# seanrjohnson/protein_gibbs_sampler

Measured on AMD Instinct MI355X. Metric: sampled positions/sec (whole node), ESM-1b L=256 B=256 Gibbs, higher is better.
Workload: dtype bf16; 1 GPU; ESM_sampler ESM-1b (33 layers, d=1280) Gibbs: 256 chains in total, 256 per GPU x L=256 (T=258), P=25 positions per chain per iteration, mask=True top_k=0 temperature=1.0 burnin=inf; bf16 MFMA operands, fp32 accumulate + fp32 residual stream; synthetic weights N(0,0.025), embeddings N(0,0.3), LayerNorm jitter 0.1 (logit std ~10); global_batch=256, seq_len=256, parallelism=chains sharded 1-way (contiguous blocks), 1 RCCL all-gather at the end, n_layers=33

## Files before the change

### include/pgibbs.h

```cpp
#ifndef PGIBBS_H
#define PGIBBS_H

#include <stdint.h>

#ifdef __cplusplus
extern "C" {
#endif

#ifndef PG_API
#if defined(__GNUC__) || defined(__clang__)
#define PG_API __attribute__((visibility("default")))
#else
#define PG_API
#endif
#endif

#define PG_OK 0
#define PG_ERR_INVALID 1
#define PG_ERR_HIP 2
#define PG_ERR_NO_DEVICE 3
#define PG_ERR_WEIGHTS 4
#define PG_ERR_UNSUPPORTED 5
#define PG_ERR_RANGE 6

PG_API const char* pg_version(void);
PG_API const char* pg_last_error(void);
PG_API int pg_device_count(void);

typedef struct pg_pyrandom pg_pyrandom;
PG_API pg_pyrandom* pg_pyrandom_create(void);
PG_API void pg_pyrandom_destroy(pg_pyrandom*);
PG_API int pg_pyrandom_seed(pg_pyrandom*, const uint32_t* key_words, int n_words);
PG_API int pg_pyrandom_setstate(pg_pyrandom*, const uint32_t* mt624, int index);
PG_API int pg_pyrandom_getstate(const pg_pyrandom*, uint32_t* mt624, int* index);
PG_API uint32_t pg_pyrandom_getrandbits32(pg_pyrandom*, int k );
PG_API double pg_pyrandom_random(pg_pyrandom*);
PG_API int pg_pyrandom_sample(pg_pyrandom*, const int32_t* population, int n, int k, int32_t* out);
PG_API int pg_pyrandom_sample_table(pg_pyrandom*, const int32_t* population, int n, int k, int64_t n_rows, int32_t* out);
PG_API int pg_pyrandom_shuffle(pg_pyrandom*, int32_t* x, int n);
PG_API int pg_pyrandom_choices(pg_pyrandom*, int n, int k, int32_t* out);

typedef struct pg_engine pg_engine;

#define PG_ARCH_ESM1B 1
#define PG_ARCH_MSA1B 2
#define PG_ARCH_ESM1 3
#define PG_ARCH_ESM2 4

#define PG_PREC_BF16 0
#define PG_PREC_F16 2
#define PG_PREC_FP32 1

typedef struct {
  int32_t arch;
  int32_t vocab;
  int32_t d_model;
  int32_t n_layers;
  int32_t n_heads;
  int32_t d_ffn;
  int32_t max_positions;
  int32_t pad_idx, mask_idx, cls_idx, eos_idx;
  int32_t token_dropout;
  int32_t max_msa_rows;
  float layer_norm_eps;
} pg_model_config;

typedef struct {
  const char* name;
  const float* data;
  int64_t numel;
} pg_tensor;

PG_API int pg_engine_create(const pg_model_config* cfg, const pg_tensor* tensors, int n_tensors, int device_ordinal,
                     int precision, pg_engine** out);
PG_API int pg_engine_create_embedded(const pg_model_config* cfg, int head_slot, const pg_tensor* tensors, int n_tensors, int device_ordinal,
                              int precision, pg_engine** out);
PG_API void pg_engine_destroy(pg_engine*);
PG_API int pg_engine_set_stream(pg_engine*, void* hip_stream);
PG_API int pg_engine_synchronize(pg_engine*);
PG_API int pg_engine_device(const pg_engine*);
PG_API int pg_engine_set_job_items(pg_engine*, int64_t job_items);
PG_API int pg_engine_get_stat(pg_engine*, const char* name, int64_t* value);

typedef struct {
  int32_t mask;
  int32_t mask_idx;
  int32_t top_k;
  int32_t burnin;
  float temperature;
  int32_t n_valid;
  int32_t valid_idx[32];
  uint64_t rng_seed;
  uint32_t rng_stream;
  uint32_t row_id_base;
  int32_t iter_base;
} pg_sample_params;


PG_API int pg_esm_forward_logits(pg_engine*, const int32_t* tokens, int B, int T, float* logits_out);
PG_API int pg_esm_gibbs_run(pg_engine*, int32_t* tokens_inout, int B, int T, const int32_t* target_idx, int n_iters, int P,
                     const pg_sample_params* params, float* sampled_logits, int32_t* sampled_tokens);
PG_API int pg_esm_gibbs_run_device(pg_engine*, int32_t* d_tokens_inout, int B, int T, const int32_t* d_target_idx,
                            int n_iters, int P, const pg_sample_params* params, float* d_sampled_logits,
                            int32_t* d_sampled_tokens);

PG_API int pg_esm_forward_representations(pg_engine*, const int32_t* tokens, int B, int T, const int32_t* layers, int n_req,
                                          const int32_t* pools, int n_pools, float* per_token_out, float* pooled_out);
PG_API int pg_repr_dbg_rows(int device, const float* x, int64_t M, int d, int d_live, const float* gamma, const float* beta, float eps,
                            const int32_t* tokens, int pad_idx, float* rows_out, int B, int T, const int32_t* pools, int n_pools,
                            float* pooled_out);

PG_API int pg_engine_set_contact_head(pg_engine*, const float* weight, int n_weights, float bias);
PG_API int pg_esm_forward_contacts(pg_engine*, const int32_t* tokens, int B, int T, float* contacts_out, float* logits_out,
                                   const int32_t* attn_layers, int n_attn, float* attn_out);
PG_API int pg_contact_dbg_probs(int device, int precision, const float* qkv, int n_seq, int T, int H, int head_dim, const int32_t* key_tok,
                                int pad_idx, float* probs_out, char* plan, int plan_bytes);
PG_API int pg_contact_dbg_accumulate(int device, const float* P, const int32_t* tokens, int eos_idx, int pad_idx, const float* w, float bias,
                                     int first, int last, float* logits_inout, float* contacts_out, int B, int T, int H);

PG_API int pg_msa_forward_logits(pg_engine*, const int32_t* tokens, int B, int R, int C, float* logits_out);
PG_API int pg_msa_gibbs_run(pg_engine*, int32_t* tokens_inout, int B, int R, int C, const int32_t* target_idx, int n_iters,
                     int P, const pg_sample_params* params, float* sampled_logits, int32_t* sampled_tokens);
PG_API int pg_msa_gibbs_run_device(pg_engine*, int32_t* d_tokens_inout, int B, int R, int C, const int32_t* d_target_idx,
                            int n_iters, int P, const pg_sample_params* params, float* d_sampled_logits,
                            int32_t* d_sampled_tokens);
PG_API int pg_msa_gibbs_single_run(pg_engine*, int32_t* tokens_inout, int R, int C, int mask_row, int target_row,
                            const int32_t* step_idx, const int32_t* step_sample_flag, int n_steps, int P_max,
                            const pg_sample_params* params, float* sampled_logits, int32_t* sampled_tokens);
PG_API int pg_msa_gibbs_single_batch_run(pg_engine*, int32_t* tokens_inout, int B, int R, int C, int mask_row, int target_row,
                                  const int32_t* step_idx, const int32_t* step_sample_flag, int n_steps, int P_max,
                                  const pg_sample_params* params, float* sampled_logits, int32_t* sampled_tokens);

PG_API int pg_esm_forward_logprobs(pg_engine*, const int32_t* tokens, int B, int T, const int32_t* row_of, const int32_t* idx,
                            const int32_t* targets, int n_sel, int P, float* out);
PG_API int pg_msa_forward_logprobs(pg_engine*, const int32_t* tokens, int B, int R, int C, const int32_t* row_of,
                            const int32_t* idx, const int32_t* targets, int n_sel, int P, float* out);
PG_API int pg_logprob_gather_device(void* stream, const float* d_logits, int64_t n_rows, int width, int V, const int32_t* d_idx,
                             const int32_t* d_row_map, const int32_t* d_targets, int64_t n_sel, int P, float* d_out);

#define PG_TABLE_NORM_VOCAB 0
#define PG_TABLE_NORM_COLUMNS 1
PG_API int pg_logprob_table_device(void* stream, const float* d_logits, int64_t n_rows, int width, int V, const int32_t* d_idx,
                            const int32_t* d_row_map, int64_t n_sel, int P, const int32_t* d_cols, int n_cols, int norm,
                            float* d_out , float* d_entropy );
PG_API int pg_esm_forward_logprob_table(pg_engine*, const int32_t* tokens, int B, int T, const int32_t* row_of, const int32_t* idx,
                                 int n_sel, int P, const int32_t* cols, int n_cols, int norm, float* out, float* entropy_or_null);
PG_API int pg_msa_forward_logprob_table(pg_engine*, const int32_t* tokens, int B, int R, int C, const int32_t* row_of,
                                 const int32_t* idx, int n_sel, int P, const int32_t* cols, int n_cols, int norm, float* out,
                                 float* entropy_or_null);

PG_API int pg_mask_scatter_device(void* stream, int32_t* d_tokens, int64_t n_rows, int width, const int32_t* d_idx,
                           const int32_t* d_row_map, int64_t n_sel, int P, int mask_idx);
PG_API int pg_sample_writeback_device(void* stream, int32_t* d_tokens, int64_t n_rows, int width, const float* d_logits,
                               int V, const int32_t* d_idx, const int32_t* d_row_map, int64_t n_sel, int P,
                               const pg_sample_params* params, int iteration, int32_t* d_sampled_tokens);

typedef struct {
  const float* bias;
  int64_t bias_rows;
  int width;
  int n_valid;
  const float* temperatures;
  int n_temperatures;
  float top_p;
} pg_draw_guide;
PG_API int pg_engine_set_draw_guide(pg_engine*, const pg_draw_guide* guide_or_null);
PG_API int pg_sample_writeback_guided_device(void* stream, int32_t* d_tokens, int64_t n_rows, int width, const float* d_logits, int V,
                                      const int32_t* d_idx, const int32_t* d_row_map, int64_t n_sel, int P,
                                      const pg_sample_params* params, int iteration, int32_t* d_sampled_tokens, const float* d_bias,
                                      int64_t bias_rows, const float* d_temperatures, int n_temperatures, float top_p);

#define PG_COMM_ID_BYTES 128
typedef struct pg_comm pg_comm;
PG_API int pg_comm_unique_id(void* id_out);
PG_API int pg_comm_create(int rank, int world, const void* unique_id, int device_ordinal, pg_comm** out);
PG_API void pg_comm_destroy(pg_comm*);
PG_API int pg_comm_rank(const pg_comm*);
PG_API int pg_comm_world(const pg_comm*);
PG_API int pg_gather_tokens(pg_comm*, void* hip_stream, const int32_t* d_local, int64_t rows, int width, const int64_t* counts,
                     int32_t* d_out);
typedef int (*pg_allgather_fn)(void* ctx, const void* send, void* recv, size_t n_int32);
PG_API int pg_dbg_gather_tokens_host(int rank, int world, const int32_t* local, int64_t rows, int width, const int64_t* counts,
                              int force_padded, pg_allgather_fn allgather, void* ctx, int32_t* out);
PG_API int pg_dbg_gather_plan(int rank, int world, int64_t rows, int width, const int64_t* counts, int force_padded, int64_t* out7,
                       int64_t* out_off_bytes);

PG_API int pg_prof_enable(pg_engine*, int on);
PG_API int pg_prof_reset(pg_engine*);
PG_API int pg_prof_get(pg_engine*, const char* kernel_class, double* total_ms, int64_t* launches);
PG_API int pg_prof_get_kernels(pg_engine*, const char* kernel_class, char* buf, int buf_bytes);

PG_API int pg_dbg_gemm(int device, int precision, const float* x, const float* w, const float* bias, float* out, int M, int N,
                int K, int epi);
PG_API int pg_dbg_gemm_v(int device, int precision, const float* x, const float* w, const float* bias, float* out, int M, int N, int K, int epi,
                  int variant, int have_ws, int m_live, char* plan, int plan_bytes);
PG_API int pg_dbg_gemm_ln(int device, int precision, const float* x, const float* x_pad, const float* gamma, const float* beta, float eps,
                   const float* w, const float* bias, float* out, int out_rows, int M, int N, int K, int gelu, int nb, char* plan,
                   int plan_bytes);
PG_API int pg_dbg_gemm_bench(int device, int M, int N, int K, int epi, int variant, int iters, double* avg_ms);
PG_API int pg_dbg_gemm_plan(int M, int N, int K, int epi, int variant, int have_ws, int m_live, int n_cu, char* buf, int buf_bytes);
PG_API int pg_dbg_attention_plan(int kind, int precision, int64_t n_seq_or_B, int T_or_C, int R, int H, int head_dim, int has_pad, int has_bias,
                          int row_step, int order_bh, int n_cu, char* buf, int buf_bytes);
PG_API int pg_dbg_qkv_attention_bench(int device, int B, int T, int H, int iters, double* ms, double* max_diff);
PG_API int pg_dbg_layernorm(int device, const float* x, const float* gamma, const float* beta, float* y, int M, int d,
                     float eps);
PG_API int pg_dbg_layernorm_operand(int device, int precision, const float* x, const float* gamma, const float* beta, float* y, int M,
                             int d, float eps);
PG_API int pg_dbg_attention(int device, int precision, const float* qkv, float* ctx, int B, int T, int H);
PG_API int pg_dbg_rope(int device, int precision, float* qkv_inout, int B, int T, int H);
PG_API int pg_dbg_attention_hd(int device, int precision, const float* qkv, float* ctx, int B, int T, int H, int head_dim,
                        const int32_t* key_tok, int pad_idx);
PG_API int pg_dbg_rope_hd(int device, int precision, float* qkv_inout, int B, int T, int H, int head_dim);
PG_API int pg_dbg_attention_kv(int device, int precision, const float* qkv, float* ctx, int B, int T, int H, int head_dim,
                        const int32_t* key_tok, int pad_idx, const float* bias_k, const float* bias_v, char* plan, int plan_bytes);

PG_API int pg_dbg_msa_attention(int device, int which, const float* qkv, float* ctx, int B, int R, int C, int H, float scale);
PG_API int pg_dbg_msa_attention_tok(int device, int which, const float* qkv, float* ctx, int B, int R, int C, int H, float scale,
                             const int32_t* tok, int pad_idx, char* plan, int plan_bytes);


PG_API int pg_dbg_embed(int device, int precision, const int32_t* tokens, int n_seq, int T, const float* embed, int V, int d, const float* pos,
                 int pos_rows, const float* msa_pos, int rows_per_msa, const float* gamma, const float* beta, const float* gamma2,
                 const float* beta2, int pad_idx, int mask_idx, int token_dropout, float eps, float embed_scale, float* x, uint16_t* h2);
PG_API int pg_dbg_layernorm_rows(int device, int precision, const float* x, const float* gamma, const float* beta, uint16_t* h_inout,
                          int64_t h_rows, int M, int d, float eps, int form, int colmajor_R, int colmajor_C, int* kernel);
PG_API int pg_dbg_gather_ln(int device, int precision, const float* x, int64_t x_rows, const int32_t* idx, const int32_t* row_map, int64_t n_map,
                     int P, int width, const float* gamma, const float* beta, uint16_t* h_inout, int64_t h_rows, int64_t n_sel, int d,
                     float eps, int split);
PG_API int pg_dbg_gather_rows(int device, const void* src, int64_t src_rows, void* dst_inout, int64_t dst_rows, const int32_t* idx, int n_iters,
                       int iter, const int32_t* row_map, int64_t n_map, int P, int width, int64_t n_sel, int row_bytes);
PG_API int pg_dbg_split_rows(int device, const float* x, uint16_t* h_inout, int64_t h_rows, int rows, int K, float scale, int form,
                      float* gelu_out);
PG_API int pg_dbg_lm_tail(int device, const float* g, const float* gamma, const float* beta, const float* embed, const float* out_bias,
                   float* logits, int64_t n, int d, int V, float eps, int* small_kernel);

PG_API int pg_dbg_sample(int device, int32_t* tokens_inout, int64_t n_rows, int width, const float* logits, int V, int compact, const int32_t* idx,
                  int n_tables, const int32_t* row_map, int64_t n_sel, int P, const pg_sample_params* params, int first_iter, int n_steps,
                  int device_iter, int mask_idx, int permit_out_of_range, int32_t* sampled_out, int32_t* masked_tokens_out,
                  unsigned* nonfinite_out);
PG_API int pg_guided_dbg_sample(int device, int32_t* tokens_inout, int64_t n_rows, int width, const float* logits, int V, int compact,
                         const int32_t* idx, int n_tables, const int32_t* row_map, int64_t n_sel, int P, const pg_sample_params* params,
                         int first_iter, int n_steps, int device_iter, int mask_idx, int permit_out_of_range, int32_t* sampled_out,
                         int32_t* masked_tokens_out, unsigned* nonfinite_out, const pg_draw_guide* guide);
PG_API int pg_guided_sizeof_draw_guide(void);

PG_API int pg_embedded_embed_rows(int device, int precision, const int32_t* tokens, int n_seq, int T, const float* embed, int V, int d,
                           const float* pos, int pos_rows, const float* msa_pos, int rows_per_msa, const float* gamma, const float* beta,
                           const float* gamma2, const float* beta2, int pad_idx, int mask_idx, int token_dropout, float eps, float embed_scale,
                           float* x, uint16_t* h2, int d_live);
PG_API int pg_embedded_layernorm_rows(int device, int precision, const float* x, const float* gamma, const float* beta, uint16_t* h_inout,
                               int64_t h_rows, int M, int d, float eps, int form, int colmajor_R, int colmajor_C, int* kernel, int d_live);
PG_API int pg_embedded_gather_ln(int device, int precision, const float* x, int64_t x_rows, const int32_t* idx, const int32_t* row_map, int64_t n_map,
                          int P, int width, const float* gamma, const float* beta, uint16_t* h_inout, int64_t h_rows, int64_t n_sel, int d,
                          float eps, int split, int d_live);
PG_API int pg_embedded_lm_tail(int device, const float* g, const float* gamma, const float* beta, const float* embed, const float* out_bias,
                        float* logits, int64_t n, int d, int V, float eps, int* small_kernel, int d_live);
PG_API int pg_embedded_image(const char* name, const float* src, int64_t numel, int n_heads, int head_width, int head_slot, int d_ffn, int vocab,
                      float* image, int64_t image_numel);
PG_API int pg_embedded_rope_table(int rows, int head_width, int head_slot, float* table);

#ifdef __cplusplus
}
#endif
#endif
```

### protein_gibbs_sampler_amd/_lib.py

```python
import ctypes
import math
import os
import sys
from ctypes import (POINTER, Structure, c_char_p, c_double, c_float, c_int, c_int32, c_int64, c_uint32, c_uint64,
                    c_void_p)

_HERE = os.path.dirname(os.path.abspath(__file__))
LIB_PATH = os.environ.get("PGIBBS_LIB_PATH") or os.path.join(_HERE, "lib", "libpgibbs.so")

PG_OK = 0
PG_ERR_INVALID, PG_ERR_HIP, PG_ERR_NO_DEVICE, PG_ERR_WEIGHTS, PG_ERR_UNSUPPORTED, PG_ERR_RANGE = 1, 2, 3, 4, 5, 6
PG_ARCH_ESM1B, PG_ARCH_MSA1B, PG_ARCH_ESM1, PG_ARCH_ESM2 = 1, 2, 3, 4
PG_COMM_ID_BYTES = 128
PG_PREC_BF16, PG_PREC_FP32, PG_PREC_F16 = 0, 1, 2
PG_TABLE_NORM_VOCAB, PG_TABLE_NORM_COLUMNS = 0, 1
TABLE_NORMS = {"vocab": PG_TABLE_NORM_VOCAB, "columns": PG_TABLE_NORM_COLUMNS}
INT32_MAX = 2**31 - 1


class PgError(RuntimeError):
    def __init__(self, code, msg):
        super().__init__("pgibbs error %d: %s" % (code, msg))
        self.code = code
        self.msg = msg


class ModelConfig(Structure):
    _fields_ = [("arch", c_int32), ("vocab", c_int32), ("d_model", c_int32), ("n_layers", c_int32), ("n_heads", c_int32),
                ("d_ffn", c_int32), ("max_positions", c_int32), ("pad_idx", c_int32), ("mask_idx", c_int32),
                ("cls_idx", c_int32), ("eos_idx", c_int32), ("token_dropout", c_int32), ("max_msa_rows", c_int32),
                ("layer_norm_eps", c_float)]


class Tensor(Structure):
    _fields_ = [("name", c_char_p), ("data", POINTER(c_float)), ("numel", c_int64)]


class SampleParams(Structure):
    _fields_ = [("mask", c_int32), ("mask_idx", c_int32), ("top_k", c_int32), ("burnin", c_int32),
                ("temperature", c_float), ("n_valid", c_int32), ("valid_idx", c_int32 * 32), ("rng_seed", c_uint64),
                ("rng_stream", c_uint32), ("row_id_base", c_uint32), ("iter_base", c_int32)]


class DrawGuideStruct(Structure):
    _fields_ = [("bias", POINTER(c_float)), ("bias_rows", c_int64), ("width", c_int), ("n_valid", c_int),
                ("temperatures", POINTER(c_float)), ("n_temperatures", c_int), ("top_p", c_float)]


class EngineHandle(c_void_p):

    @classmethod
    def from_param(cls, value):
        return c_void_p.from_param(value)


_lib = None

_P32 = POINTER(c_int32)
_PF = POINTER(c_float)
_PU32 = POINTER(c_uint32)
SIGNATURES = [
    ("pg_version", c_char_p, []),
    ("pg_last_error", c_char_p, []),
    ("pg_device_count", c_int, []),
    ("pg_pyrandom_create", c_void_p, []),
    ("pg_pyrandom_destroy", None, [c_void_p]),
    ("pg_pyrandom_seed", c_int, [c_void_p, _PU32, c_int]),
    ("pg_pyrandom_setstate", c_int, [c_void_p, _PU32, c_int]),
    ("pg_pyrandom_getstate", c_int, [c_void_p, _PU32, POINTER(c_int)]),
    ("pg_pyrandom_getrandbits32", c_uint32, [c_void_p, c_int]),
    ("pg_pyrandom_random", c_double, [c_void_p]),
    ("pg_pyrandom_sample", c_int, [c_void_p, _P32, c_int, c_int, _P32]),
    ("pg_pyrandom_sample_table", c_int, [c_void_p, _P32, c_int, c_int, c_int64, _P32]),
    ("pg_pyrandom_shuffle", c_int, [c_void_p, _P32, c_int]),
    ("pg_pyrandom_choices", c_int, [c_void_p, c_int, c_int, _P32]),
    ("pg_engine_create", c_int, [POINTER(ModelConfig), POINTER(Tensor), c_int, c_int, c_int, POINTER(c_void_p)]),
    ("pg_engine_create_embedded", c_int, [POINTER(ModelConfig), c_int, POINTER(Tensor), c_int, c_int, c_int, POINTER(c_void_p)]),
    ("pg_engine_destroy", None, [c_void_p]),
    ("pg_engine_set_stream", c_int, [c_void_p, c_void_p]),
    ("pg_engine_synchronize", c_int, [c_void_p]),
    ("pg_engine_device", c_int, [c_void_p]),
    ("pg_engine_set_job_items", c_int, [c_void_p, c_int64]),
    ("pg_engine_get_stat", c_int, [c_void_p, c_char_p, POINTER(c_int64)]),
    ("pg_esm_forward_logits", c_int, [c_void_p, c_void_p, c_int, c_int, c_void_p]),
    ("pg_esm_gibbs_run", c_int, [c_void_p, c_void_p, c_int, c_int, c_void_p, c_int, c_int, POINTER(SampleParams), c_void_p,
                                 c_void_p]),
    ("pg_esm_gibbs_run_device", c_int, [c_void_p, c_void_p, c_int, c_int, c_void_p, c_int, c_int, POINTER(SampleParams),
                                        c_void_p, c_void_p]),
    ("pg_msa_forward_logits", c_int, [c_void_p, c_void_p, c_int, c_int, c_int, c_void_p]),
    ("pg_msa_gibbs_run", c_int, [c_void_p, c_void_p, c_int, c_int, c_int, c_void_p, c_int, c_int, POINTER(SampleParams),
                                 c_void_p, c_void_p]),
    ("pg_msa_gibbs_run_device", c_int, [c_void_p, c_void_p, c_int, c_int, c_int, c_void_p, c_int, c_int, POINTER(SampleParams),
                                        c_void_p, c_void_p]),
    ("pg_msa_gibbs_single_run", c_int, [c_void_p, c_void_p, c_int, c_int, c_int, c_int, c_void_p, c_void_p, c_int, c_int,
                                        POINTER(SampleParams), c_void_p, c_void_p]),
    ("pg_msa_gibbs_single_batch_run", c_int, [c_void_p, c_void_p, c_int, c_int, c_int, c_int, c_int, c_void_p, c_void_p, c_int,
                                              c_int, POINTER(SampleParams), c_void_p, c_void_p]),
    ("pg_esm_forward_logprobs", c_int, [c_void_p, c_void_p, c_int, c_int, c_void_p, c_void_p, c_void_p, c_int, c_int, c_void_p]),
    ("pg_msa_forward_logprobs", c_int, [c_void_p, c_void_p, c_int, c_int, c_int, c_void_p, c_void_p, c_void_p, c_int, c_int,
                                        c_void_p]),
    ("pg_logprob_gather_device", c_int, [c_void_p, c_void_p, c_int64, c_int, c_int, c_void_p, c_void_p, c_void_p, c_int64, c_int,
                                         c_void_p]),
    ("pg_logprob_table_device", c_int, [c_void_p, c_void_p, c_int64, c_int, c_int, c_void_p, c_void_p, c_int64, c_int, c_void_p, c_int,
                                        c_int, c_void_p, c_void_p]),
    ("pg_esm_forward_logprob_table", c_int, [c_void_p, c_void_p, c_int, c_int, c_void_p, c_void_p, c_int, c_int, c_void_p, c_int, c_int,
                                             c_void_p, c_void_p]),
    ("pg_msa_forward_logprob_table", c_int, [c_void_p, c_void_p, c_int, c_int, c_int, c_void_p, c_void_p, c_int, c_int, c_void_p, c_int,
                                             c_int, c_void_p, c_void_p]),
    ("pg_mask_scatter_device", c_int, [c_void_p, c_void_p, c_int64, c_int, c_void_p, c_void_p, c_int64, c_int, c_int]),
    ("pg_sample_writeback_device", c_int, [c_void_p, c_void_p, c_int64, c_int, c_void_p, c_int, c_void_p, c_void_p, c_int64,
                                           c_int, POINTER(SampleParams), c_int, c_void_p]),
    ("pg_engine_set_draw_guide", c_int, [c_void_p, POINTER(DrawGuideStruct)]),
    ("pg_sample_writeback_guided_device", c_int, [c_void_p, c_void_p, c_int64, c_int, c_void_p, c_int, c_void_p, c_void_p, c_int64,
                                                  c_int, POINTER(SampleParams), c_int, c_void_p, c_void_p, c_int64, c_void_p, c_int,
                                                  c_float]),
    ("pg_guided_dbg_sample", c_int, [c_int, c_void_p, c_int64, c_int, c_void_p, c_int, c_int, c_void_p, c_int, c_void_p, c_int64, c_int,
                                     POINTER(SampleParams), c_int, c_int, c_int, c_int, c_int, c_void_p, c_void_p, c_void_p,
                                     POINTER(DrawGuideStruct)]),
    ("pg_guided_sizeof_draw_guide", c_int, []),
    ("pg_esm_forward_representations", c_int, [EngineHandle, c_void_p, c_int, c_int, c_void_p, c_int, c_void_p, c_int, c_void_p, c_void_p]),
    ("pg_repr_dbg_rows", c_int, [c_int, c_void_p, c_int64, c_int, c_int, c_void_p, c_void_p, c_float, c_void_p, c_int, c_void_p, c_int,
                                 c_int, c_void_p, c_int, c_void_p]),
    ("pg_engine_set_contact_head", c_int, [EngineHandle, c_void_p, c_int, c_float]),
    ("pg_esm_forward_contacts", c_int, [EngineHandle, c_void_p, c_int, c_int, c_void_p, c_void_p, c_void_p, c_int, c_void_p]),
    ("pg_contact_dbg_probs", c_int, [c_int, c_int, c_void_p, c_int, c_int, c_int, c_int, c_void_p, c_int, c_void_p, c_char_p, c_int]),
    ("pg_contact_dbg_accumulate", c_int, [c_int, c_void_p, c_void_p, c_int, c_int, c_void_p, c_float, c_int, c_int, c_void_p, c_void_p,
                                          c_int, c_int, c_int]),
    ("pg_comm_unique_id", c_int, [c_void_p]),
    ("pg_comm_create", c_int, [c_int, c_int, c_void_p, c_int, POINTER(c_void_p)]),
    ("pg_comm_destroy", None, [c_void_p]),
    ("pg_comm_rank", c_int, [c_void_p]),
    ("pg_comm_world", c_int, [c_void_p]),
    ("pg_gather_tokens", c_int, [c_void_p, c_void_p, c_void_p, c_int64, c_int, POINTER(c_int64), c_void_p]),
    ("pg_dbg_gather_tokens_host", c_int, [c_int, c_int, c_void_p, c_int64, c_int, POINTER(c_int64), c_int, c_void_p, c_void_p, c_void_p]),
    ("pg_dbg_gather_plan", c_int, [c_int, c_int, c_int64, c_int, POINTER(c_int64), c_int, POINTER(c_int64), POINTER(c_int64)]),
    ("pg_prof_enable", c_int, [c_void_p, c_int]),
    ("pg_prof_reset", c_int, [c_void_p]),
    ("pg_prof_get", c_int, [c_void_p, c_char_p, POINTER(c_double), POINTER(c_int64)]),
    ("pg_prof_get_kernels", c_int, [c_void_p, c_char_p, c_char_p, c_int]),
    ("pg_dbg_gemm", c_int, [c_int, c_int, c_void_p, c_void_p, c_void_p, c_void_p, c_int, c_int, c_int, c_int]),
    ("pg_dbg_gemm_v", c_int, [c_int, c_int, c_void_p, c_void_p, c_void_p, c_void_p, c_int, c_int, c_int, c_int, c_int, c_int, c_int,
                              c_char_p, c_int]),
    ("pg_dbg_gemm_ln", c_int, [c_int, c_int, c_void_p, c_void_p, c_void_p, c_void_p, c_float, c_void_p, c_void_p, c_void_p, c_int, c_int,
                               c_int, c_int, c_int, c_int, c_char_p, c_int]),
    ("pg_dbg_gemm_bench", c_int, [c_int, c_int, c_int, c_int, c_int, c_int, c_int, POINTER(c_double)]),
    ("pg_dbg_gemm_plan", c_int, [c_int, c_int, c_int, c_int, c_int, c_int, c_int, c_int, c_char_p, c_int]),
    ("pg_dbg_attention_plan", c_int, [c_int, c_int, c_int64, c_int, c_int, c_int, c_int, c_int, c_int, c_int, c_int, c_int, c_char_p, c_int]),
    ("pg_dbg_qkv_attention_bench", c_int, [c_int, c_int, c_int, c_int, c_int, POINTER(c_double), POINTER(c_double)]),
    ("pg_dbg_layernorm", c_int, [c_int, c_void_p, c_void_p, c_void_p, c_void_p, c_int, c_int, c_float]),
    ("pg_dbg_layernorm_operand", c_int, [c_int, c_int, c_void_p, c_void_p, c_void_p, c_void_p, c_int, c_int, c_float]),
    ("pg_dbg_attention", c_int, [c_int, c_int, c_void_p, c_void_p, c_int, c_int, c_int]),
    ("pg_dbg_rope", c_int, [c_int, c_int, c_void_p, c_int, c_int, c_int]),
    ("pg_dbg_attention_hd", c_int, [c_int, c_int, c_void_p, c_void_p, c_int, c_int, c_int, c_int, c_void_p, c_int]),
    ("pg_dbg_rope_hd", c_int, [c_int, c_int, c_void_p, c_int, c_int, c_int, c_int]),
    ("pg_dbg_attention_kv", c_int, [c_int, c_int, c_void_p, c_void_p, c_int, c_int, c_int, c_int, c_void_p, c_int, c_void_p, c_void_p,
                                    c_char_p, c_int]),
    ("pg_dbg_msa_attention", c_int, [c_int, c_int, c_void_p, c_void_p, c_int, c_int, c_int, c_int, c_float]),
    ("pg_dbg_msa_attention_tok", c_int, [c_int, c_int, c_void_p, c_void_p, c_int, c_int, c_int, c_int, c_float, c_void_p, c_int,
                                         c_char_p, c_int]),
    ("pg_dbg_embed", c_int, [c_int, c_int, c_void_p, c_int, c_int, c_void_p, c_int, c_int, c_void_p, c_int, c_void_p, c_int, c_void_p,
                             c_void_p, c_void_p, c_void_p, c_int, c_int, c_int, c_float, c_float, c_void_p, c_void_p]),
    ("pg_dbg_layernorm_rows", c_int, [c_int, c_int, c_void_p, c_void_p, c_void_p, c_void_p, c_int64, c_int, c_int, c_float, c_int, c_int,
                                      c_int, POINTER(c_int)]),
    ("pg_dbg_gather_ln", c_int, [c_int, c_int, c_void_p, c_int64, c_void_p, c_void_p, c_int64, c_int, c_int, c_void_p, c_void_p, c_void_p,
                                 c_int64, c_int64, c_int, c_float, c_int]),
    ("pg_dbg_gather_rows", c_int, [c_int, c_void_p, c_int64, c_void_p, c_int64, c_void_p, c_int, c_int, c_void_p, c_int64, c_int, c_int,
                                   c_int64, c_int]),
    ("pg_dbg_split_rows", c_int, [c_int, c_void_p, c_void_p, c_int64, c_int, c_int, c_float, c_int, c_void_p]),
    ("pg_dbg_lm_tail", c_int, [c_int, c_void_p, c_void_p, c_void_p, c_void_p, c_void_p, c_void_p, c_int64, c_int, c_int, c_float,
                               POINTER(c_int)]),
    ("pg_dbg_sample", c_int, [c_int, c_void_p, c_int64, c_int, c_void_p, c_int, c_int, c_void_p, c_int, c_void_p, c_int64, c_int,
                              POINTER(SampleParams), c_int, c_int, c_int, c_int, c_int, c_void_p, c_void_p, c_void_p]),
    ("pg_embedded_embed_rows", c_int, [c_int, c_int, c_void_p, c_int, c_int, c_void_p, c_int, c_int, c_void_p, c_int, c_void_p, c_int, c_void_p,
                                  c_void_p, c_void_p, c_void_p, c_int, c_int, c_int, c_float, c_float, c_void_p, c_void_p, c_int]),
    ("pg_embedded_layernorm_rows", c_int, [c_int, c_int, c_void_p, c_void_p, c_void_p, c_void_p, c_int64, c_int, c_int, c_float, c_int, c_int,
                                           c_int, POINTER(c_int), c_int]),
    ("pg_embedded_gather_ln", c_int, [c_int, c_int, c_void_p, c_int64, c_void_p, c_void_p, c_int64, c_int, c_int, c_void_p, c_void_p, c_void_p,
                                      c_int64, c_int64, c_int, c_float, c_int, c_int]),
    ("pg_embedded_lm_tail", c_int, [c_int, c_void_p, c_void_p, c_void_p, c_void_p, c_void_p, c_void_p, c_int64, c_int, c_int, c_float,
                                    POINTER(c_int), c_int]),
    ("pg_embedded_image", c_int, [c_char_p, c_void_p, c_int64, c_int, c_int, c_int, c_int, c_int, c_void_p, c_int64]),
    ("pg_embedded_rope_table", c_int, [c_int, c_int, c_int, c_void_p]),
]


def lib():
    global _lib
    if _lib is not None:
        return _lib
    if not os.path.exists(LIB_PATH):
        raise ImportError(
            "protein_gibbs_sampler_amd: the HIP library %s is missing. Build it with "
            "`python -c 'import __graft_entry__ as g; g.build()'` (or `make -C protein_gibbs_sampler_amd/csrc`). "
            "There is no CPU fallback." % LIB_PATH)
    if os.environ.get("PGIBBS_HIP_RUNTIME", "auto") != "system":
        try:
            import torch
        except ImportError:
            pass
    handle = ctypes.CDLL(LIB_PATH, mode=ctypes.RTLD_GLOBAL)
    for name, restype, argtypes in SIGNATURES:
        fn = getattr(handle, name)
        fn.restype = restype
        fn.argtypes = argtypes
    _lib = handle
    return _lib


def check(rc):
    if rc != PG_OK:
        msg = lib().pg_last_error()
        raise PgError(rc, msg.decode() if msg else "")


def ptr(arr):
    return arr.ctypes.data_as(c_void_p)


def make_sample_params(mask, mask_idx, top_k, burnin, temperature, valid_idx, rng_seed, rng_stream=0, row_id_base=0,
                       iter_base=0):
    p = SampleParams()
    p.mask = 1 if mask else 0
    p.mask_idx = int(mask_idx)
    p.top_k = int(max(min(top_k, INT32_MAX), -INT32_MAX))
    p.burnin = INT32_MAX if burnin == float("inf") or burnin > INT32_MAX else int(max(math.ceil(burnin), -INT32_MAX))
    p.temperature = float("nan") if temperature is None else float(temperature)
    if not 1 <= len(valid_idx) <= 32:
        raise ValueError("valid_idx must have 1..32 entries")
    p.n_valid = len(valid_idx)
    for i, v in enumerate(valid_idx):
        p.valid_idx[i] = int(v)
    p.rng_seed = int(rng_seed) & (2**64 - 1)
    p.rng_stream = int(rng_stream) & 0xFFFFFFFF
    p.row_id_base = int(row_id_base) & 0xFFFFFFFF
    p.iter_base = int(iter_base)
    return p


def make_draw_guide(bias=None, temperatures=None, top_p=None):
    import numpy as np
    g = DrawGuideStruct()
    keep = []
    if bias is not None:
        b = np.ascontiguousarray(bias, dtype=np.float32)
        if b.ndim != 3:
            raise ValueError("a draw guide's bias table is [bias_rows, width, n_valid]")
        keep.append(b)
        g.bias = b.ctypes.data_as(POINTER(c_float))
        g.bias_rows, g.width, g.n_valid = b.shape
    if temperatures is not None:
        t = np.ascontiguousarray(temperatures, dtype=np.float32).reshape(-1)
        keep.append(t)
        g.temperatures = t.ctypes.data_as(POINTER(c_float))
        g.n_temperatures = len(t)
    g.top_p = float("nan") if top_p is None else float(top_p)
    return g, keep
```

### protein_gibbs_sampler_amd/csrc/api_dbg.hip

```cpp
#include <math.h>
#include <string.h>

#include <algorithm>
#include <vector>

#include "engine.h"
#include "gemm_epilogue.h"
#include "ln_row.h"

using namespace pg;

namespace {
struct Dbg {
  int prev = -1;
  bool bad = false;
  std::vector<void*> bufs;
  Dbg() { (void)hipGetDevice(&prev); }
  ~Dbg() {
    for (void* p : bufs) (void)hipFree(p);
    if (prev >= 0) (void)hipSetDevice(prev);
  }
  int open(int device) {
    int n = 0;
    if (hipGetDeviceCount(&n) != hipSuccess || n == 0) return fail(PG_ERR_NO_DEVICE, "no HIP device visible");
// ... 49 lines not shown
  PG_HIP(hipDeviceSynchronize());
  std::vector<bf16_t> h((size_t)M * 3 * d);
  PG_HIP(hipMemcpy(h.data(), c3, h.size() * 2, hipMemcpyDeviceToHost));
  for (int64_t r = 0; r < M; ++r)
    for (int c = 0; c < d; ++c) {
      const size_t g = (size_t)r * 3 * d + split_lo_offset(c);
      const bf16_t lo = h[g], hi = h[g + kSplitHi], hi2 = h[g + kSplitDup];
      if (hi != hi2) return fail(PG_ERR_HIP, "split operand row: the two hi copies differ");
      dst[(size_t)r * d + c] = bf16_to_f32(hi) + bf16_to_f32(lo);
    }
  return PG_OK;
}
std::vector<float> lcg_uniform(size_t n, uint32_t seed) {
  std::vector<float> h(n);
  for (auto& v : h) {
    seed = seed * 1664525u + 1013904223u;
    v = (seed >> 8) * (1.0f / 8388608.0f) - 1.0f;
  }
  return h;
}
struct EventPair {
  hipEvent_t a = nullptr, b = nullptr;
  ~EventPair() {
    if (a) (void)hipEventDestroy(a);
    if (b) (void)hipEventDestroy(b);
  }
};
template <typename Launch>
int time_launches(Launch&& launch, int iters, double* avg_ms) {
  EventPair ev;
  for (hipEvent_t* e : {&ev.a, &ev.b}) PG_HIP(hipEventCreate(e));
  int rc;
  for (int i = 0; i < 2; ++i)
    if ((rc = launch())) return rc;
  PG_HIP(hipEventRecord(ev.a, nullptr));
  for (int i = 0; i < iters; ++i)
    if ((rc = launch())) return rc;
  PG_HIP(hipEventRecord(ev.b, nullptr));
  PG_HIP(hipEventSynchronize(ev.b));
  float ms = 0;
  PG_HIP(hipEventElapsedTime(&ms, ev.a, ev.b));
  *avg_ms = ms / iters;
  return PG_OK;
}
void dbg_noted_text(char* plan, int plan_bytes) {
  if (plan && plan_bytes > 0) snprintf(plan, (size_t)plan_bytes, "%s", noted_kernels().c_str());
}

template <typename Launch>
int dbg_attention_run(Dbg& s, int precision, bool strict, const float* qkv, float* ctx, int64_t M, int d, const int32_t* tok, char* plan,
                      int plan_bytes, Launch&& launch) {
  const float* dq = s.up(qkv, (size_t)M * 3 * d);
  const int32_t* dtok = s.up(tok, (size_t)M);
  bf16_t* bq = strict ? nullptr : s.alloc<bf16_t>((size_t)M * 3 * d);
  bf16_t* out = s.alloc<bf16_t>((size_t)M * d * (strict ? 3 : 1));
  float* wide = strict ? nullptr : s.alloc<float>((size_t)M * d);
  int rc = s.check();
  if (rc) return rc;
  clear_noted_kernels();
  if (!strict && (rc = to16(precision, dq, bq, M * 3 * d))) return rc;
  if ((rc = launch(dq, bq, out, dtok))) return rc;
  dbg_noted_text(plan, plan_bytes);
  return strict ? split3_rows_to_host(out, ctx, M, d) : down16(s, precision, out, wide, ctx, M * d);
}
}

extern "C" {

int pg_dbg_gemm(int device, int precision, const float* x, const float* w, const float* bias, float* out, int M, int N,
                int K, int epi) {
  return pg_dbg_gemm_v(device, precision, x, w, bias, out, M, N, K, epi, -1, -1, M, nullptr, 0);
}

int pg_dbg_gemm_v(int device, int precision, const float* x, const float* w, const float* bias, float* out, int M, int N, int K, int epi,
                  int variant, int have_ws, int m_live, char* plan, int plan_bytes) {
  if (plan && plan_bytes > 0) plan[0] = 0;
  int rc = dbg_precision("pg_dbg_gemm", precision, true);
  if (rc) return rc;
  if (!x || !w || !bias || !out || M < 1 || N % 64 || K % 64 || (plan && plan_bytes < 1)) return fail(PG_ERR_INVALID, "pg_dbg_gemm: bad argument");
  if (have_ws < -1 || have_ws > 1 || m_live < 0 || m_live > M) return fail(PG_ERR_INVALID, "pg_dbg_gemm_v: have_ws is -1, 0 or 1 and m_live 0 ... M");
  const bool whole = variant == 1 || variant == 2 || variant == 6 || variant == 7 || variant == 8 || variant == 20 || variant == 80;
  if (variant != -1 && !whole) return fail(PG_ERR_INVALID, "pg_dbg_gemm_v: variant must be -1, 1, 2, 6, 7, 8, 20 or 80");
  const bool strict = precision == PG_PREC_FP32;
  if (strict && variant != -1) return fail(PG_ERR_UNSUPPORTED, "strict mode: launch_gemm_split3 has no variant (-1 only)");
  if (strict && epi == 5 && N % 256) return fail(PG_ERR_INVALID, "pg_dbg_gemm: the fused GELU-and-split epilogue needs N a multiple of 256");
  if (strict && epi != 0 && epi != 2 && epi != 5)
    return fail(PG_ERR_UNSUPPORTED, "strict mode: plain (0), residual (2) and fused GELU-split (5) epilogues only");
  Dbg d;
  if ((rc = d.open(device))) return rc;
  const int Mp = round_up(M, kRowPad), ks = strict ? 3 : 1;
  const int M16 = M <= 256 ? round_up(M, 16) : Mp;
  const bool out16 = !strict && (epi == 3 || epi == 4);
  float* dx = d.alloc<float>((size_t)Mp * K);
  d.put(dx, x, (size_t)M * K);
  const float* dw = d.up(w, (size_t)N * K);
  const float* db = d.up(bias, (size_t)N);
  float* dout = d.alloc<float>((size_t)Mp * N);
  if (epi == 2) d.put(dout, out, (size_t)M * N);
  bf16_t* bx = d.alloc<bf16_t>((size_t)Mp * K * ks);
  bf16_t* bw = d.alloc<bf16_t>((size_t)N * K * ks);
  bf16_t* o16 = strict && epi == 5 ? d.alloc<bf16_t>((size_t)Mp * 3 * N) : out16 ? d.alloc<bf16_t>((size_t)Mp * N) : nullptr;
  const bool offer = have_ws < 0 ? epi == 2 : have_ws == 1;
  const size_t ws_bytes = !strict && offer ? OPS(gemm_splitk_ws_bytes, Mp, N, K) : 0;
  float* ws = ws_bytes && ws_bytes <= ((size_t)1 << 30) ? (float*)d.alloc<char>(ws_bytes) : nullptr;
  if ((rc = d.check())) return rc;
  if (strict) {
    if ((rc = launch_split3_bf16(nullptr, dx, bx, Mp, K, 1.f, false, false))) return rc;
    if ((rc = launch_split3_bf16(nullptr, dw, bw, N, K, 1.f, false, true))) return rc;
    clear_noted_kernels();
    if (epi == 5) {
      if ((rc = launch_gemm_split3(nullptr, bx, bw, db, o16, Mp, N, K, 3 * N, EPI_SPLIT3_GELU))) return rc;
      dbg_noted_text(plan, plan_bytes);
      return split3_rows_to_host(o16, out, M, N);
    }
    if ((rc = launch_gemm_split3(nullptr, bx, bw, db, dout, Mp, N, K, N, epi == 2 ? EPI_F32_RESID : EPI_F32))) return rc;
    dbg_noted_text(plan, plan_bytes);
    return d.down(out, dout, (size_t)M * N);
  }
  if ((rc = to16(precision, dx, bx, (int64_t)Mp * K))) return rc;
  if ((rc = to16(precision, dw, bw, (int64_t)N * K))) return rc;
  clear_noted_kernels();
  void* o = out16 ? (void*)o16 : (void*)dout;
  const int e = out16 ? (epi == 4 ? EPI_BF16_GELU : EPI_BF16) : (epi == 2 ? EPI_F32_RESID : (epi ? EPI_F32_GELU : EPI_F32));
  rc = variant < 0 ? OPS(launch_gemm_bf16, nullptr, bx, bw, db, o, M16, N, K, K, K, N, e, ws, ws ? ws_bytes : 0, m_live)
                   : OPS(launch_gemm_bf16_variant, nullptr, bx, bw, db, o, M16, N, K, K, K, N, e, variant, ws, ws ? ws_bytes : 0, m_live);
  if (rc) return rc;
  dbg_noted_text(plan, plan_bytes);
  return out16 ? down16(d, precision, o16, dout, out, (int64_t)M * N) : d.down(out, dout, (size_t)M * N);
}

int pg_dbg_gemm_ln(int device, int precision, const float* x, const float* x_pad, const float* gamma, const float* beta, float eps,
                   const float* w, const float* bias, float* out, int out_rows, int M, int N, int K, int gelu, int nb, char* plan,
                   int plan_bytes) {
  if (plan && plan_bytes > 0) plan[0] = 0;
  int rc = dbg_precision("pg_dbg_gemm_ln", precision, false);
  if (rc) return rc;
  if (!x || !gamma || !beta || !w || !bias || !out || (plan && plan_bytes < 1)) return fail(PG_ERR_INVALID, "pg_dbg_gemm_ln: bad argument");
  if (M < 1 || M > 32) return fail(PG_ERR_INVALID, "pg_dbg_gemm_ln: M must be in 1 ... 32");
  if (N < 16 || N % 16 || N > 65536) return fail(PG_ERR_INVALID, "pg_dbg_gemm_ln: N must be a multiple of 16, at most 65536");
  if (K < 256 || K % 256) return fail(PG_ERR_INVALID, "pg_dbg_gemm_ln: K must be a multiple of 256");
  if (K / 256 > 5) return fail(PG_ERR_INVALID, "pg_dbg_gemm_ln: K / 256 must be in 1 ... 5");
  if (gelu < 0 || gelu > 1 || nb < 0 || nb > 2) return fail(PG_ERR_INVALID, "pg_dbg_gemm_ln: gelu is 0 or 1 and nb 0, 1 or 2");
  if (nb == 2 && N % 32) return fail(PG_ERR_INVALID, "pg_dbg_gemm_ln: two feature blocks per workgroup need N a multiple of 32");
  if (!(eps >= 0.f)) return fail(PG_ERR_INVALID, "pg_dbg_gemm_ln: eps must not be negative");
  const int Mi = round_up(M, 16);
  if (out_rows < Mi || out_rows > 4096) return fail(PG_ERR_INVALID, "pg_dbg_gemm_ln: out_rows must be in Mi ... 4096");
  if (!OPS(gemm_ln_skinny_ok, Mi, N, K)) return fail(PG_ERR_INVALID, "pg_dbg_gemm_ln: the kernel is switched off (PGIBBS_LN_SKINNY=0)");
  Dbg d;
  if ((rc = d.open(device))) return rc;
  float* dx = d.alloc<float>((size_t)Mi * K);
  d.put(dx, x, (size_t)M * K);
  if (x_pad) d.put(dx + (size_t)M * K, x_pad, (size_t)(Mi - M) * K);
  const float* dg = d.up(gamma, (size_t)K);
  const float* dbt = d.up(beta, (size_t)K);
  const float* dw = d.up(w, (size_t)N * K);
  const float* db = d.up(bias, (size_t)N);
  float* dout = d.up(out, (size_t)out_rows * N);
  bf16_t* bw = d.alloc<bf16_t>((size_t)N * K);
  bf16_t* o16 = d.alloc<bf16_t>((size_t)out_rows * N);
  if ((rc = d.check())) return rc;
  if ((rc = to16(precision, dw, bw, (int64_t)N * K))) return rc;
  if ((rc = to16(precision, dout, o16, (int64_t)out_rows * N))) return rc;
  clear_noted_kernels();
  if ((rc = OPS(launch_gemm_ln_skinny, nullptr, dx, K, dg, dbt, eps, bw, db, o16, Mi, N, K, K, N, gelu ? EPI_BF16_GELU : EPI_BF16, nb))) return rc;
  dbg_noted_text(plan, plan_bytes);
  return down16(d, precision, o16, dout, out, (int64_t)out_rows * N);
}

int pg_dbg_gemm_bench(int device, int M, int N, int K, int epi, int variant, int iters, double* avg_ms) {
  if (!avg_ms || M % 16 || (M > 256 && M % 64) || N % 64 || K % 64 || iters < 1) return fail(PG_ERR_INVALID, "pg_dbg_gemm_bench: bad argument");
  if (variant == 90 && (K % 96 || (epi != EPI_F32 && epi != EPI_F32_RESID))) return fail(PG_ERR_INVALID, "variant 90: K = 3 x depth, fp32 epilogues");
  Dbg d;
  int rc = d.open(device);
  if (rc) return rc;
  const std::vector<float> h = lcg_uniform((size_t)(M > N ? M : N) * K, 12345u);
  const float* f = d.up(h.data(), h.size());
  bf16_t* bx = d.alloc<bf16_t>((size_t)round_up(M, kRowPad) * K);
  bf16_t* bw = d.alloc<bf16_t>((size_t)N * K);
  const float* db = d.alloc<float>((size_t)N);
  void* dout = d.alloc<float>((size_t)round_up(M, kRowPad) * N);
  const size_t ws_bytes = (epi == EPI_F32_RESID && M <= 8192) ? gemm_splitk_ws_bytes(M, N, K) : 0;
  float* ws = ws_bytes ? (float*)d.alloc<char>(ws_bytes) : nullptr;
  if ((rc = d.check())) return rc;
  if ((rc = to16(PG_PREC_BF16, f, bx, (int64_t)M * K))) return rc;
  if ((rc = to16(PG_PREC_BF16, f, bw, (int64_t)N * K, 0.05f))) return rc;
  return time_launches([&] {
    if (variant == 90) return launch_gemm_split3_w16(nullptr, bx, bw, db, dout, M, N, K / 3, N, epi);
    return launch_gemm_bf16_variant(nullptr, bx, bw, db, dout, M, N, K, K, K, N, epi, variant, ws, ws ? ws_bytes : 0);
  }, iters, avg_ms);
}

int pg_dbg_gemm_plan(int M, int N, int K, int epi, int variant, int have_ws, int m_live, int n_cu, char* buf, int buf_bytes) {
  if (!buf || buf_bytes < 2 || M < 1 || N < 1 || K < 1 || n_cu < 1) return fail(PG_ERR_INVALID, "pg_dbg_gemm_plan: bad argument");
  std::string text;
  gemm_plan_text(M, N, K, epi, variant, have_ws != 0, m_live, n_cu, &text);
  snprintf(buf, (size_t)buf_bytes, "%s", text.c_str());
  return PG_OK;
}

int pg_dbg_attention_plan(int kind, int precision, int64_t n_seq_or_B, int T_or_C, int R, int H, int head_dim, int has_pad, int has_bias,
                          int row_step, int order_bh, int n_cu, char* buf, int buf_bytes) {
  const int rc = dbg_precision("pg_dbg_attention_plan", precision, true);
  if (rc) return rc;
  if (!buf || buf_bytes < 2 || (kind != 0 && kind != 1) || n_seq_or_B < 1 || H < 1 || n_cu < 1 || (kind == 1 && (R < 1 || n_seq_or_B > 0x7fffffff)))
    return fail(PG_ERR_INVALID, "pg_dbg_attention_plan: bad argument");
  const bool strict = precision == PG_PREC_FP32;
  std::string text;
  if (kind == 0 && strict) attention_f32_plan_text(n_seq_or_B, T_or_C, H, head_dim, has_pad != 0, has_bias != 0, &text);
  else if (kind == 0) attention_plan_text(n_seq_or_B, T_or_C, H, head_dim, has_pad != 0, has_bias != 0, row_step, n_cu, &text);
  else if (strict) msa_row_f32_plan_text((int)n_seq_or_B, R, T_or_C, H, &text);
  else msa_row_plan_text((int)n_seq_or_B, R, T_or_C, H, order_bh, &text);
  snprintf(buf, (size_t)buf_bytes, "%s", text.c_str());
  return PG_OK;
}

int pg_dbg_qkv_attention_bench(int device, int B, int T, int H, int iters, double* ms, double* max_diff) {
  if (!ms || B < 1 || H < 1 || iters < 1 || !(T == 32 || T == 64 || T == 128 || T == 256))
    return fail(PG_ERR_INVALID, "pg_dbg_qkv_attention_bench: T must be 32, 64, 128 or 256");
  Dbg s;
  int rc = s.open(device);
  if (rc) return rc;
  const int d = H * 64;
  const int64_t M = (int64_t)B * T, Mp = round_up64(M, kRowPad);
  const std::vector<float> h = lcg_uniform((size_t)std::max<int64_t>(Mp, 3 * d) * d, 777u);
  const float* fx = s.up(h.data(), (size_t)Mp * d);
  const float* fw = s.up(h.data(), (size_t)3 * d * d);
  const float* db = s.up(h.data(), (size_t)3 * d);
  bf16_t* bx = s.alloc<bf16_t>((size_t)Mp * d);
  bf16_t* bw = s.alloc<bf16_t>((size_t)3 * d * d);
  bf16_t* bwh = s.alloc<bf16_t>((size_t)3 * d * d);
  float* dbh = s.alloc<float>((size_t)3 * d);
  bf16_t* qkv = s.alloc<bf16_t>((size_t)Mp * 3 * d);
  bf16_t* c1 = s.alloc<bf16_t>((size_t)Mp * d);
  bf16_t* c2 = s.alloc<bf16_t>((size_t)Mp * d);
  if ((rc = s.check())) return rc;
  if ((rc = to16(PG_PREC_BF16, fx, bx, Mp * d))) return rc;
  if ((rc = to16(PG_PREC_BF16, fw, bw, (int64_t)3 * d * d, 0.03f))) return rc;
  if ((rc = launch_headmajor_qkv(nullptr, bw, db, bwh, dbh, H, d))) return rc;
  auto fused = [&] { return launch_gemm_colattn(nullptr, bx, bwh, dbh, c1, B, T, 1, H, d, d); };
  auto proj = [&] { return launch_gemm_bf16(nullptr, bx, bw, db, qkv, (int)Mp, 3 * d, d, d, d, 3 * d, EPI_BF16); };
  auto attn = [&] { return launch_attention_bf16(nullptr, qkv, c2, B, T, H, 3 * d, d, d, 2 * d); };
  if ((rc = time_launches(fused, iters, ms + 0)) || (rc = time_launches(proj, iters, ms + 1)) || (rc = time_launches(attn, iters, ms + 2)))
    return rc;
  if (max_diff) {
    std::vector<bf16_t> a((size_t)M * d), b((size_t)M * d);
    if ((rc = s.down(a.data(), c1, a.size())) || (rc = s.down(b.data(), c2, b.size()))) return rc;
    double worst = 0;
    for (size_t i = 0; i < a.size(); ++i) worst = std::max(worst, (double)fabsf(bf16_to_f32(a[i]) - bf16_to_f32(b[i])));
    *max_diff = worst;
  }
  return PG_OK;
}

int pg_dbg_layernorm(int device, const float* x, const float* gamma, const float* beta, float* y, int M, int d, float eps) {
  if (!x || !gamma || !beta || !y || M < 1 || d < 4) return fail(PG_ERR_INVALID, "pg_dbg_layernorm: bad argument");
  Dbg s;
  int rc = s.open(device);
  if (rc) return rc;
  const float* dx = s.up(x, (size_t)M * d);
  const float* dg = s.up(gamma, (size_t)d);
  const float* dbt = s.up(beta, (size_t)d);
  float* dy = s.alloc<float>((size_t)M * d);
  if ((rc = s.check())) return rc;
  if ((rc = launch_layernorm_f32(nullptr, dx, dg, dbt, dy, M, d, eps))) return rc;
  return s.down(y, dy, (size_t)M * d);
}

int pg_dbg_attention(int device, int precision, const float* qkv, float* ctx, int B, int T, int H) {
  return pg_dbg_attention_hd(device, precision, qkv, ctx, B, T, H, 64, nullptr, -1);
}

int pg_dbg_attention_hd(int device, int precision, const float* qkv, float* ctx, int B, int T, int H, int head_dim,
                        const int32_t* key_tok, int pad_idx) {
  return pg_dbg_attention_kv(device, precision, qkv, ctx, B, T, H, head_dim, key_tok, pad_idx, nullptr, nullptr, nullptr, 0);
}

int pg_dbg_attention_kv(int device, int precision, const float* qkv, float* ctx, int B, int T, int H, int head_dim,
                        const int32_t* key_tok, int pad_idx, const float* bias_k, const float* bias_v, char* plan, int plan_bytes) {
  if (plan && plan_bytes > 0) plan[0] = 0;
  int rc = dbg_precision("pg_dbg_attention_kv", precision, true);
  if (rc) return rc;
  if (!qkv || !ctx || B < 1 || T < 1 || H < 1 || (plan && plan_bytes < 1)) return fail(PG_ERR_INVALID, "pg_dbg_attention: bad argument");
  if (!head_width(head_dim)) return fail(PG_ERR_INVALID, "pg_dbg_attention_hd: head_dim must be " + head_widths_text(false));
  if (!bias_k != !bias_v) return fail(PG_ERR_INVALID, "pg_dbg_attention_kv: bias_k and bias_v come together or not at all");
  const std::string head_err = attention_head_error(head_dim, bias_k != nullptr);
  if (!head_err.empty()) return fail(PG_ERR_INVALID, head_err);
  if ((double)B * T * 3 * H * head_dim > 2147483647.0) return fail(PG_ERR_INVALID, "pg_dbg_attention: more than 2^31 - 1 qkv values");
  Dbg s;
  if ((rc = s.open(device))) return rc;
  const int d = H * head_dim;
  const bool strict = precision == PG_PREC_FP32;
  float* bias32 = bias_k ? s.alloc<float>((size_t)2 * d) : nullptr;
  if (bias_k) s.put(bias32, bias_k, (size_t)d), s.put(bias32 + d, bias_v, (size_t)d);
  bf16_t* bias16 = bias_k && !strict ? s.alloc<bf16_t>((size_t)2 * d) : nullptr;
  return dbg_attention_run(s, precision, strict, qkv, ctx, (int64_t)B * T, d, key_tok, plan, plan_bytes,
                           [&](const float* dq, const bf16_t* bq, bf16_t* out, const int32_t* dtok) {
    const SeqLayout chain = {1, T, 0, 1};
    if (strict) return launch_attention_f32(nullptr, dq, out, d, B, T, H, 3 * d, 3 * d, d, 2 * d, chain, dtok, pad_idx, bias32, head_dim);
    const int rc16 = bias_k ? to16(precision, bias32, bias16, 2 * d) : PG_OK;
    return rc16 ? rc16 : OPS(launch_attention_bf16, nullptr, bq, out, B, T, H, 3 * d, d, d, 2 * d, dtok, pad_idx, bias16, head_dim);
  });
}

int pg_dbg_layernorm_operand(int device, int precision, const float* x, const float* gamma, const float* beta, float* y, int M, int d,
                             float eps) {
  int rc = dbg_precision("pg_dbg_layernorm_operand", precision, true);
  if (rc) return rc;
  if (!x || !gamma || !beta || !y || M < 1 || d < 32 || d % 32) return fail(PG_ERR_INVALID, "pg_dbg_layernorm_operand: bad argument");
  Dbg s;
  if ((rc = s.open(device))) return rc;
  const bool split = precision == PG_PREC_FP32;
  const float* dx = s.up(x, (size_t)M * d);
  const float* dg = s.up(gamma, (size_t)d);
  const float* dbt = s.up(beta, (size_t)d);
  float* dy = s.alloc<float>((size_t)M * d);
  bf16_t* h = s.alloc<bf16_t>((size_t)M * d * (split ? 3 : 1));
  if ((rc = s.check())) return rc;
  if ((rc = OPS(launch_layernorm_bf16, nullptr, dx, dg, dbt, h, M, d, eps, split, 0, 0, true))) return rc;
  return split ? split3_rows_to_host(h, y, M, d) : down16(s, precision, h, dy, y, (int64_t)M * d);
}

int pg_dbg_rope(int device, int precision, float* qkv, int B, int T, int H) {
  return pg_dbg_rope_hd(device, precision, qkv, B, T, H, 64);
}

int pg_dbg_rope_hd(int device, int precision, float* qkv, int B, int T, int H, int head_dim) {
  int rc = dbg_precision("pg_dbg_rope_hd", precision, true);
  if (rc) return rc;
  const HeadWidth* w = head_width(head_dim);
  if (!w) return fail(PG_ERR_INVALID, "pg_dbg_rope_hd: head_dim must be " + head_widths_text(false));
  if (!qkv || B < 1 || T < 1 || H < 1 || H > w->max_heads) return fail(PG_ERR_INVALID, "pg_dbg_rope: bad argument");
  Dbg s;
  if ((rc = s.open(device))) return rc;
  const int d = H * head_dim;
  const int64_t M = (int64_t)B * T, n = M * 3 * d;
  const std::vector<float> tab = rope_table(T, head_dim);
  float* dq = s.up(qkv, (size_t)n);
  const float* dtab = s.up(tab.data(), tab.size());
  bf16_t* bq = precision == PG_PREC_FP32 ? nullptr : s.alloc<bf16_t>((size_t)n);
  if ((rc = s.check())) return rc;
  if (precision == PG_PREC_FP32) {
    if ((rc = launch_rope(nullptr, dq, true, dtab, T, M, T, H, 3 * d, head_dim))) return rc;
    return s.down(qkv, dq, (size_t)n);
  }
  if ((rc = to16(precision, dq, bq, n))) return rc;
  if ((rc = OPS(launch_rope, nullptr, bq, false, dtab, T, M, T, H, 3 * d, head_dim))) return rc;
  return down16(s, precision, bq, dq, qkv, n);
}

int pg_dbg_msa_attention(int device, int which, const float* qkv, float* ctx, int B, int R, int C, int H, float scale) {
  return pg_dbg_msa_attention_tok(device, which, qkv, ctx, B, R, C, H, scale, nullptr, -1, nullptr, 0);
}

int pg_dbg_msa_attention_tok(int device, int which, const float* qkv, float* ctx, int B, int R, int C, int H, float scale,
                             const int32_t* tok, int pad_idx, char* plan, int plan_bytes) {
  if (plan && plan_bytes > 0) plan[0] = 0;
  if (!qkv || !ctx || B < 1 || R < 1 || C < 1 || H < 1 || (plan && plan_bytes < 1)) return fail(PG_ERR_INVALID, "pg_dbg_msa_attention: bad argument");
  if (which < 0 || which > 5) return fail(PG_ERR_INVALID, "pg_dbg_msa_attention: which must be 0 ... 5");
  if ((double)B * R * C * 3 * H * 64 > 2147483647.0) return fail(PG_ERR_INVALID, "pg_dbg_msa_attention: more than 2^31 - 1 qkv values");
  if (tok && which == 4)
    return fail(PG_ERR_UNSUPPORTED, "fp16 precision mode: alignments wider than 576 columns take the split-bf16 row attention, "
                                    "which exists for bf16 operands only -- use precision bf16 or fp32");
  if ((which == 2 || (which == 0 && tok)) && (double)B * H * C * msa_row_scores_ld(C) > 1073741823.0)
    return fail(PG_ERR_INVALID, "pg_dbg_msa_attention: the fp32 score maps of this shape exceed 4 GiB");
  const int precision = (which == 4 || which == 5) ? PG_PREC_F16 : PG_PREC_BF16;
  if (which == 4 || which == 5) which -= 4;
  Dbg s;
  int rc = s.open(device);
  if (rc) return rc;
  const int d = H * 64;
  const int64_t M = (int64_t)B * R * C;
  const bool strict = which == 2 || which == 3;
  const bool ragged = which == 0 && tok;
  float* wide = ragged ? s.alloc<float>((size_t)M * 3 * d) : nullptr;
  float* sc = which == 2 || ragged ? s.alloc<float>((size_t)B * H * C * msa_row_scores_ld(C)) : nullptr;
  const size_t pbytes = (size_t)B * H * 16 * C * 576 * 4 + (size_t)B * H * (C / 16 + 9) * 18 * 1024;
  float* part = which == 0 && !tok && pbytes <= ((size_t)1 << 30) ? (float*)s.alloc<char>(pbytes) : nullptr;
  return dbg_attention_run(s, precision, strict, qkv, ctx, M, d, tok, plan, plan_bytes,
                           [&](const float* dq, const bf16_t* bq, bf16_t* out, const int32_t* dtok) {
    const SeqLayout col = {C, R * C, 1, C};
    if (which == 2) return launch_msa_row_attention_f32(nullptr, dq, sc, out, d, B, R, C, H, 3 * d, 3 * d, d, 2 * d, scale, dtok, pad_idx);
    if (which == 3) return launch_attention_f32(nullptr, dq, out, d, (int64_t)B * C, R, H, 3 * d, 3 * d, d, 2 * d, col, dtok, pad_idx);
    if (ragged) {
      const int rcw = launch_bf16_to_f32(nullptr, bq, wide, M * 3 * d);
      return rcw ? rcw : launch_msa_row_attention_f32(nullptr, wide, sc, out, 0, B, R, C, H, 3 * d, d, d, 2 * d, scale, dtok, pad_idx);
    }
    if (which == 0) return OPS(launch_msa_row_attention_bf16, nullptr, bq, out, B, R, C, H, 3 * d, d, d, 2 * d, scale, part, part ? pbytes : 0, 0);
    return OPS(launch_attention_seq_bf16, nullptr, bq, out, (int64_t)B * C, R, H, 3 * d, d, d, 2 * d, col, dtok, pad_idx);
  });
}

extern "C++" {
namespace {
int dbg_row_width(const char* who, int d, int d_live) {
  if (!row_d_ok(d)) return
    fail(PG_ERR_INVALID, std::string(who) + ": d must be a multiple of 4 and <= 2560, or a multiple of 512 up to 5120");
  if (!row_live_ok(d, d_live)) return fail(PG_ERR_INVALID, std::string(who) + ": the live width must be a multiple of 4, at most d");
  return PG_OK;
}
int64_t dbg_gather_src(const char* who, int64_t r, int32_t pos, bool zero_fill, const int32_t* row_map, int64_t n_map, int P, int width,
                       int64_t src_rows) {
  if (pos < 0 || (pos & 0x3fffffff) >= width) {
    if (zero_fill) return -1;
    pos = 0;
  }
  pos &= 0x3fffffff;
  const int64_t s = r / P;
  if (row_map && s >= n_map) { fail(PG_ERR_INVALID, std::string(who) + ": row_map is shorter than the selected rows need"); return -2; }
  const int64_t row = (row_map ? (int64_t)row_map[s] : s) * width + pos;
  if (row < 0 || row >= src_rows) {
    fail(PG_ERR_INVALID, std::string(who) + ": selected row " + std::to_string(r) + " reads source row " + std::to_string(row) + " of " + std::to_string(src_rows));
    return -2;
  }
  return row;
}
const char* const kCopyFailed = "hipMalloc / copy failed";
}
}

static int dbg_embed_rows(const char* who, int device, int precision, const int32_t* tokens, int n_seq, int T, const float* embed, int V, int d,
                           const float* pos, int pos_rows, const float* msa_pos, int rows_per_msa, const float* gamma, const float* beta,
                           const float* gamma2, const float* beta2, int pad_idx, int mask_idx, int token_dropout, float eps, float embed_scale,
                           float* x, uint16_t* h2, int d_live) {
  int rc = dbg_precision(who, precision, false);
  if (rc) return rc;
  if (!tokens || !embed || !x || n_seq < 1 || T < 1 || V < 1 || (pos && pos_rows < 1) || rows_per_msa < 0 || (rows_per_msa > 0 && !msa_pos) ||
      !gamma != !beta || !gamma2 != !beta2 || !gamma2 != !h2)
    return fail(PG_ERR_INVALID, std::string(who) + ": bad argument");
  if ((rc = dbg_row_width(who, d, d_live))) return rc;
  if (d_live != d && gamma) return fail(PG_ERR_INVALID, std::string(who) + ": emb_layer_norm_before has no live-width form");
  const int64_t n_tok = (int64_t)n_seq * T;
  for (int64_t sq = 0; sq < n_seq; ++sq) {
    int n_before = 0;
    for (int t = 0; t < T; ++t) {
      const int32_t tok = tokens[sq * T + t];
      if (tok < 0 || tok >= V)
        return fail(PG_ERR_INVALID, std::string(who) + ": token " + std::to_string(tok) + " is outside the embedding table of " + std::to_string(V) + " rows");
      n_before += tok != pad_idx;
      const int p = tok == pad_idx ? pad_idx : n_before + pad_idx;
      if (pos && (p < 0 || p >= pos_rows))
        return fail(PG_ERR_INVALID, std::string(who) + ": position row " + std::to_string(p) + " is outside the position table of " + std::to_string(pos_rows) + " rows");
    }
  }
  Dbg s;
  if ((rc = s.open(device))) return rc;
  const int32_t* dtok = s.up(tokens, (size_t)n_tok);
  const float* de = s.up(embed, (size_t)V * d);
  const float* dp = s.up(pos, (size_t)pos_rows * d);
  const float* dm = rows_per_msa > 0 ? s.up(msa_pos, (size_t)rows_per_msa * d) : nullptr;
  const float* dg = s.up(gamma, (size_t)d);
  const float* db = s.up(beta, (size_t)d);
  const float* dg2 = s.up(gamma2, (size_t)d);
  const float* db2 = s.up(beta2, (size_t)d);
  float* dx = s.alloc<float>((size_t)n_tok * d);
  bf16_t* dh = h2 ? s.up((const bf16_t*)h2, (size_t)n_tok * d) : nullptr;
  if ((rc = s.check(kCopyFailed))) return rc;
  if ((rc = OPS(launch_embed_ln, nullptr, dtok, de, dp, dm, dg, db, dx, n_tok, T, d, pad_idx, mask_idx, token_dropout, rows_per_msa, eps, dg2,
                db2, dh, embed_scale, d_live)))
    return rc;
  if ((rc = s.down(x, dx, (size_t)n_tok * d))) return rc;
  return h2 ? s.down(h2, dh, (size_t)n_tok * d) : PG_OK;
}

int pg_dbg_embed(int device, int precision, const int32_t* tokens, int n_seq, int T, const float* embed, int V, int d, const float* pos,
                 int pos_rows, const float* msa_pos, int rows_per_msa, const float* gamma, const float* beta, const float* gamma2,
                 const float* beta2, int pad_idx, int mask_idx, int token_dropout, float eps, float embed_scale, float* x, uint16_t* h2) {
  return dbg_embed_rows("pg_dbg_embed", device, precision, tokens, n_seq, T, embed, V, d, pos, pos_rows, msa_pos, rows_per_msa, gamma, beta, gamma2, beta2,
                                pad_idx, mask_idx, token_dropout, eps, embed_scale, x, h2, d);
}

int pg_embedded_embed_rows(int device, int precision, const int32_t* tokens, int n_seq, int T, const float* embed, int V, int d,
                           const float* pos, int pos_rows, const float* msa_pos, int rows_per_msa, const float* gamma, const float* beta,
                           const float* gamma2, const float* beta2, int pad_idx, int mask_idx, int token_dropout, float eps, float embed_scale,
                           float* x, uint16_t* h2, int d_live) {
  return dbg_embed_rows("pg_embedded_embed_rows", device, precision, tokens, n_seq, T, embed, V, d, pos, pos_rows, msa_pos, rows_per_msa, gamma, beta, gamma2, beta2, pad_idx, mask_idx, token_dropout, eps, embed_scale, x, h2, d_live);
}

static int dbg_layernorm_rows(const char* who, int device, int precision, const float* x, const float* gamma, const float* beta, uint16_t* h_inout,
                               int64_t h_rows, int M, int d, float eps, int form, int colmajor_R, int colmajor_C, int* kernel, int d_live) {
  int rc = dbg_precision(who, precision, false);
  if (rc) return rc;
  if (!x || !gamma || !beta || !h_inout || M < 1 || h_rows < M || form < 0 || form > 2 || colmajor_R < 0 || (colmajor_R > 0 && colmajor_C < 1))
    return fail(PG_ERR_INVALID, std::string(who) + ": bad argument");
  if (form && (precision != PG_PREC_BF16 || d % 32))
    return fail(PG_ERR_INVALID, std::string(who) + ": split rows are bf16 pairs in groups of 32 columns");
  if (row_d_ok(d) && !row_live_ok(d, d_live)) return fail(PG_ERR_INVALID, std::string(who) + ": the live width must be a multiple of 4, at most d");
  if ((rc = OPS(layernorm_bf16_check, M, d, form != 0, colmajor_R, colmajor_C, d_live))) return rc;
  Dbg s;
  if ((rc = s.open(device))) return rc;
  const size_t h_n = (size_t)h_rows * d * (form ? 3 : 1);
  const float* dx = s.up(x, (size_t)M * d);
  const float* dg = s.up(gamma, (size_t)d);
  const float* db = s.up(beta, (size_t)d);
  bf16_t* dh = s.up(h_inout, h_n);
  if ((rc = s.check(kCopyFailed))) return rc;
  unsigned stride_grid = 0;
  if (kernel) *kernel = OPS(layernorm_bf16_choice, M, d, colmajor_R, &stride_grid, d_live);
  if ((rc = OPS(launch_layernorm_bf16, nullptr, dx, dg, db, dh, M, d, eps, form != 0, colmajor_R, colmajor_C, form != 2, d_live))) return rc;
  return s.down(h_inout, dh, h_n);
}

int pg_dbg_layernorm_rows(int device, int precision, const float* x, const float* gamma, const float* beta, uint16_t* h_inout,
                          int64_t h_rows, int M, int d, float eps, int form, int colmajor_R, int colmajor_C, int* kernel) {
  return dbg_layernorm_rows("pg_dbg_layernorm_rows", device, precision, x, gamma, beta, h_inout, h_rows, M, d, eps, form, colmajor_R, colmajor_C, kernel, d);
}

int pg_embedded_layernorm_rows(int device, int precision, const float* x, const float* gamma, const float* beta, uint16_t* h_inout,
                               int64_t h_rows, int M, int d, float eps, int form, int colmajor_R, int colmajor_C, int* kernel, int d_live) {
  return dbg_layernorm_rows("pg_embedded_layernorm_rows", device, precision, x, gamma, beta, h_inout, h_rows, M, d, eps, form, colmajor_R, colmajor_C, kernel, d_live);
}

static int dbg_gather_ln_rows(const char* who, int device, int precision, const float* x, int64_t x_rows, const int32_t* idx, const int32_t* row_map, int64_t n_map,
                          int P, int width, const float* gamma, const float* beta, uint16_t* h_inout, int64_t h_rows, int64_t n_sel, int d,
                          float eps, int split, int d_live) {
  int rc = dbg_precision(who, precision, false);
  if (rc) return rc;
  if (!x || !gamma || !beta || !h_inout || x_rows < 1 || n_sel < 1 || h_rows < n_sel || P < 1 || width < 1 || (row_map && n_map < 1) ||
      split < 0 || split > 1)
    return fail(PG_ERR_INVALID, std::string(who) + ": bad argument");
  if ((rc = dbg_row_width(who, d, d_live))) return rc;
  if (split && (precision != PG_PREC_BF16 || d % 32))
    return fail(PG_ERR_INVALID, std::string(who) + ": split rows are bf16 pairs in groups of 32 columns");
  if (!idx) {
    if (n_sel > x_rows) return fail(PG_ERR_INVALID, std::string(who) + ": more selected rows than source rows");
  } else {
    for (int64_t r = 0; r < n_sel; ++r)
      if (dbg_gather_src(who, r, idx[r], true, row_map, n_map, P, width, x_rows) == -2) return PG_ERR_INVALID;
  }
  Dbg s;
  if ((rc = s.open(device))) return rc;
  const size_t h_n = (size_t)h_rows * d * (split ? 3 : 1);
  const float* dx = s.up(x, (size_t)x_rows * d);
  const int32_t* di = s.up(idx, (size_t)n_sel);
  const int32_t* dm = s.up(row_map, (size_t)n_map);
  const float* dg = s.up(gamma, (size_t)d);
  const float* db = s.up(beta, (size_t)d);
  bf16_t* dh = s.up(h_inout, h_n);
  if ((rc = s.check(kCopyFailed))) return rc;
  if ((rc = OPS(launch_gather_ln_bf16, nullptr, dx, di, dm, P, width, dg, db, dh, n_sel, d, eps, split != 0, d_live))) return rc;
  return s.down(h_inout, dh, h_n);
}

int pg_dbg_gather_ln(int device, int precision, const float* x, int64_t x_rows, const int32_t* idx, const int32_t* row_map, int64_t n_map,
                     int P, int width, const float* gamma, const float* beta, uint16_t* h_inout, int64_t h_rows, int64_t n_sel, int d,
                     float eps, int split) {
  return dbg_gather_ln_rows("pg_dbg_gather_ln", device, precision, x, x_rows, idx, row_map, n_map, P, width, gamma, beta, h_inout, h_rows, n_sel, d, eps, split, d);
}

int pg_embedded_gather_ln(int device, int precision, const float* x, int64_t x_rows, const int32_t* idx, const int32_t* row_map, int64_t n_map,
                          int P, int width, const float* gamma, const float* beta, uint16_t* h_inout, int64_t h_rows, int64_t n_sel, int d,
                          float eps, int split, int d_live) {
  return dbg_gather_ln_rows("pg_embedded_gather_ln", device, precision, x, x_rows, idx, row_map, n_map, P, width, gamma, beta, h_inout, h_rows, n_sel, d, eps, split, d_live);
}

int pg_dbg_gather_rows(int device, const void* src, int64_t src_rows, void* dst_inout, int64_t dst_rows, const int32_t* idx, int n_iters,
                       int iter, const int32_t* row_map, int64_t n_map, int P, int width, int64_t n_sel, int row_bytes) {
  if (!src || !dst_inout || !idx || src_rows < 1 || n_sel < 1 || dst_rows < n_sel || P < 1 || width < 1 || (row_map && n_map < 1) ||
      n_iters < 0 || (n_iters > 0 && (iter < 0 || iter >= n_iters)) || row_bytes < 16)
    return fail(PG_ERR_INVALID, "pg_dbg_gather_rows: bad argument");
  if (row_bytes % 16) return fail(PG_ERR_INVALID, "pg_dbg_gather_rows: rows must be multiples of 16 bytes");
  const int32_t* now = idx + (n_iters > 0 ? (size_t)iter * n_sel : 0);
  for (int64_t r = 0; r < n_sel; ++r)
    if (dbg_gather_src("pg_dbg_gather_rows", r, now[r], false, row_map, n_map, P, width, src_rows) == -2) return PG_ERR_INVALID;
  Dbg s;
  int rc = s.open(device);
  if (rc) return rc;
  const char* ds = s.up((const char*)src, (size_t)src_rows * row_bytes);
  char* dd = s.up((const char*)dst_inout, (size_t)dst_rows * row_bytes);
  const int32_t* di = s.up(idx, (size_t)(n_iters > 0 ? n_iters : 1) * n_sel);
  const int32_t* dm = s.up(row_map, (size_t)n_map);
  const int32_t it32 = iter;
  const int32_t* dit = n_iters > 0 ? s.up(&it32, 1) : nullptr;
  if ((rc = s.check(kCopyFailed))) return rc;
  if ((rc = launch_gather_rows(nullptr, ds, dd, di, dm, P, width, n_sel, row_bytes, dit))) return rc;
  return s.down((char*)dst_inout, dd, (size_t)dst_rows * row_bytes);
}

int pg_dbg_split_rows(int device, const float* x, uint16_t* h_inout, int64_t h_rows, int rows, int K, float scale, int form, float* gelu_out) {
  if (!x || !h_inout || rows < 1 || h_rows < rows || K < 1) return fail(PG_ERR_INVALID, "pg_dbg_split_rows: bad argument");
  if (K % kSplitCols) return fail(PG_ERR_INVALID, "pg_dbg_split_rows: K must be a multiple of 32");
  if (form < 0 || form > 3) return fail(PG_ERR_INVALID, "pg_dbg_split_rows: form is weight (1) + through GELU (2)");
  if (form == 3) return fail(PG_ERR_INVALID, "pg_dbg_split_rows: GELU on a weight operand");
  if (form == 2 && scale != 1.0f) return fail(PG_ERR_INVALID, "pg_dbg_split_rows: the GELU form takes scale 1");
  if (form == 2 && !gelu_out) return fail(PG_ERR_INVALID, "pg_dbg_split_rows: the GELU form returns gelu_out");
  Dbg s;
  int rc = s.open(device);
  if (rc) return rc;
  const size_t h_n = (size_t)h_rows * 3 * K;
  float* dx = s.up(x, (size_t)rows * K);
  bf16_t* dh = s.up(h_inout, h_n);
  if ((rc = s.check(kCopyFailed))) return rc;
  if ((rc = launch_split3_bf16(nullptr, dx, dh, rows, K, scale, form == 2, form == 1))) return rc;
  if ((rc = s.down(h_inout, dh, h_n))) return rc;
  if (form != 2) return PG_OK;
  if ((rc = launch_gelu_f32(nullptr, dx, (int64_t)rows * K))) return rc;
  return s.down(gelu_out, dx, (size_t)rows * K);
}

static int dbg_lm_tail_rows(const char* who, int device, const float* g, const float* gamma, const float* beta, const float* embed, const float* out_bias,
                        float* logits, int64_t n, int d, int V, float eps, int* small_kernel, int d_live) {
  if (!g || !embed || !out_bias || !logits || n < 1 || !gamma != !beta) return fail(PG_ERR_INVALID, std::string(who) + ": bad argument");
  if (V < 1 || V > 64) return fail(PG_ERR_INVALID, std::string(who) + ": vocab must be in 1..64");
  int rc = dbg_row_width(who, d, d_live);
  if (rc) return rc;
  Dbg s;
  if ((rc = s.open(device))) return rc;
// ... 212 lines not shown
```

### protein_gibbs_sampler_amd/csrc/attention.hip

```cpp
#include <stdlib.h>

#include "attn_frag.h"

PG_OPS_BEGIN


#ifdef PG_ATT_PROF
__device__ unsigned long long* pg_att_prof;
#define PG_T(slot, i)                                                                                              \
  do {                                                                                                             \
    if ((slot) < 8 && (threadIdx.x & 63) == 0)                                                                     \
      pg_att_prof[(((size_t)blockIdx.x * 4 + (threadIdx.x >> 6)) * 8 + (slot)) * 8 + (i)] = __builtin_readcyclecounter(); \
  } while (0)
#else
#define PG_T(slot, i)
#endif

constexpr int attention_occupancy(int maxkb, int hd, bool pad = false) {
  return hd == 128 ? (maxkb <= 8 || (maxkb == 10 && !pad) ? 2 : 1) : hd == 64 ? (maxkb <= 18 ? 2 : 1) : 2;
}
constexpr int attention_resident16(int kb) {
  return kb <= 6 ? 8 : kb <= 8 ? 7 : kb <= 10 ? 6 : kb <= 14 ? 5 : kb <= 22 ? 4 : kb <= 34 ? 3 : 2;
}
constexpr int attention_resident(int kb, int hd) {
  return hd == 16 ? attention_resident16(kb) : hd == 128 ? (kb <= 4 ? 4 : (kb <= 6 ? 3 : (kb <= 10 ? 2 : 1))) : hd == 64 ? (kb <= 20 ? 2 : 1) : (kb <= 20 ? 4 : (kb <= 26 ? 3 : 2));
}
template <int MAXKB, bool PADMASK, bool BIASKV = false, bool SPLIT = false, int HD = 64>
__global__ __launch_bounds__(256, attention_occupancy(MAXKB, HD, PADMASK)) void attention_kernel(const bf16_t* __restrict__ qkv, bf16_t* __restrict__ ctx, int T,
                                                       int H, int ld_qkv_, int ld_ctx_, int k_off, int v_off,
                                                       SeqLayout sl, const int32_t* __restrict__ key_tok, int pad_idx,
                                                       const bf16_t* __restrict__ bias_kv, int split_from = 0, int split = 1) {
  constexpr int ROW = HD * 2, NKK = score_steps(HD), NDB = HD / 16;
  typedef kfrag_t<HD> kf_t;
  __shared__ __attribute__((aligned(16))) char smem[2 * MAXKB * 16 * ROW + (PADMASK ? MAXKB * 16 : 0)];
  char* Ks = smem;
  char* Vs = smem + MAXKB * 16 * ROW;
  char* padf = smem + 2 * MAXKB * 16 * ROW;

  const int tid = threadIdx.x, lane = tid & 63, wave = tid >> 6;
  PG_T(7, 0);
  int pair = blockIdx.x, qb_first = wave, qb_step = 4;
  if (SPLIT && (int)blockIdx.x >= split_from) {
    const int u = blockIdx.x - split_from;
    pair = split_from + u / split;
    qb_first = u % split + split * wave;
    qb_step = 4 * split;
  }
  const int seq = pair / H, h = pair % H;
  const size_t row0 = (size_t)(seq / sl.inner_count) * sl.outer_rows + (size_t)(seq % sl.inner_count) * sl.inner_rows;
  const size_t ld_qkv = (size_t)ld_qkv_ * sl.row_step, ld_ctx = (size_t)ld_ctx_ * sl.row_step;
  const bf16_t* base = qkv + row0 * ld_qkv_ + h * HD;
  const int Tk = T + (BIASKV ? 1 : 0);
  constexpr int nkc = MAXKB / 2;

  stage_kv<MAXKB * 16, 256, BIASKV, HD>(Ks, Vs, tid, base, ld_qkv, k_off, v_off, 0, T, bias_kv + h * HD, bias_kv + (H + h) * HD);
  if (PADMASK) {
    for (int key = tid; key < MAXKB * 16; key += 256)
      padf[key] = (key < T && key_tok[row0 + (size_t)key * sl.row_step] == pad_idx) ? 1 : 0;
  }
  PG_T(7, 1);
  __syncthreads();
  PG_T(7, 2);

  const int fr = lane & 15, fq = lane >> 4;
  const int nqb = (T + 15) >> 4;
  kf_t qf[NKK], qn[NKK];
  auto load_q = [&](int qb, kf_t (&dst)[NKK]) {
    int qrow = qb * 16 + fr;
    if (qrow >= T) qrow = T - 1;
#pragma unroll
    for (int kk = 0; kk < NKK; ++kk) dst[kk] = q_frag<HD>(base + (size_t)qrow * ld_qkv, kk, fq);
  };
  if (qb_first < nqb) load_q(qb_first, qf);
  for (int qb = qb_first; qb < nqb; qb += qb_step) {
    if (qb + qb_step < nqb) load_q(qb + qb_step, qn);
    PG_T(qb >> 2, 0);

    f32x4 st[MAXKB];
    {
      constexpr int CH = HD == 128 ? 2 : (MAXKB % 6 == 0) ? 6 : (MAXKB % 4 == 0 ? 4 : 2);
      kf_t kbuf[2][CH][NKK];
      auto load_chunk = [&](int ch, kf_t (&dst)[CH][NKK]) {
#pragma unroll
        for (int u = 0; u < CH; ++u) {
#if defined(PG_ATT_PROF) && PG_ATT_ABL == 1
          const int krow = (ch * CH + (u > 0 ? 0 : u)) * 16 + fr;
          if (u > 0) { for (int kk = 0; kk < NKK; ++kk) dst[u][kk] = dst[0][kk]; continue; }
#else
          const int krow = (ch * CH + u) * 16 + fr;
#endif
#pragma unroll
          for (int kk = 0; kk < NKK; ++kk) dst[u][kk] = k_frag<HD>(Ks, krow, kk, fq);
        }
      };
      load_chunk(0, kbuf[0]);
#pragma unroll
      for (int ch = 0; ch < MAXKB / CH; ++ch) {
        if (ch + 1 < MAXKB / CH) load_chunk(ch + 1, kbuf[(ch + 1) & 1]);
        __builtin_amdgcn_sched_barrier(0);
#pragma unroll
        for (int u = 0; u < CH; ++u)
          st[ch * CH + u] = score_mfma(kbuf[ch & 1][u][0], qf[0], (f32x4){0.f, 0.f, 0.f, 0.f});
        if constexpr (NKK == 2) {
#pragma unroll
          for (int u = 0; u < CH; ++u)
            st[ch * CH + u] = score_mfma(kbuf[ch & 1][u][1], qf[1], st[ch * CH + u]);
        }
        if constexpr (NKK == 4) {
#pragma unroll
          for (int kk = 1; kk < 4; ++kk)
#pragma unroll
            for (int u = 0; u < CH; ++u)
              st[ch * CH + u] = score_mfma(kbuf[ch & 1][u][kk], qf[kk], st[ch * CH + u]);
        }
        __builtin_amdgcn_sched_barrier(0);
      }
    }
    PG_T(qb >> 2, 1);
    int tl = Tk - fq * 4;
    asm volatile("" : "+v"(tl));
#pragma unroll
    for (int kb = MAXKB > 6 ? MAXKB - 6 : 0; kb < MAXKB; ++kb)
      if ((kb + 1) * 16 > Tk) st[kb] = mask_tail(st[kb], kb, tl);
    float mx = lane_max(st);
    if (PADMASK) {
      const float fill = sl.row_step == 1 ? -3.0e38f : -10000.0f;
      mx = -3.0e38f;
#pragma unroll
      for (int kb = 0; kb < MAXKB; ++kb) {
        st[kb] = mask_pad(st[kb], *(const uint32_t*)(padf + kb * 16 + fq * 4), fill);
#pragma unroll
        for (int r = 0; r < 4; ++r) mx = fmaxf(mx, st[kb][r]);
      }
    }
    const float inv = softmax_exact(st, mx);
    PG_T(qb >> 2, 2);

    f32x4 o[NDB];
#pragma unroll
    for (int db = 0; db < NDB; ++db) o[db] = (f32x4){0.f, 0.f, 0.f, 0.f};
    {
      VtFrag vbuf[3][NDB];
      auto load_v = [&](int c, VtFrag (&dst)[NDB]) {
#pragma unroll
        for (int db = 0; db < NDB; ++db) {
#if defined(PG_ATT_PROF) && PG_ATT_ABL == 2
          if (db > 0) { dst[db] = dst[0]; continue; }
#endif
#pragma unroll
          for (int hh = 0; hh < 2; ++hh) dst[db].h[hh] = vt_half<HD>(Vs, (2 * c + hh) * 16, db, fr, fq);
        }
      };
      load_v(0, vbuf[0]);
      if (nkc > 1) load_v(1, vbuf[1]);
#pragma unroll
      for (int c = 0; c < nkc; ++c) {
        if (c + 2 < nkc) load_v(c + 2, vbuf[(c + 2) % 3]);
        const bf16x8 pf = p_frag(st[2 * c], st[2 * c + 1]);
        __builtin_amdgcn_sched_barrier(0);
#pragma unroll
        for (int db = 0; db < NDB; ++db) o[db] = mfma_op16(vbuf[c % 3][db].v, pf, o[db]);
        __builtin_amdgcn_sched_barrier(0);
      }
    }
    PG_T(qb >> 2, 3);
    const int q = qb * 16 + fr;
    if (q < T) store_ctx(o, inv, ctx + row0 * ld_ctx_ + (size_t)q * ld_ctx + h * HD + fq * 4);
    qf[0] = qn[0];
    if constexpr (NKK == 2) qf[1] = qn[1];
    if constexpr (NKK == 4) { qf[1] = qn[1]; qf[2] = qn[2]; qf[3] = qn[3]; }
    PG_T(qb >> 2, 4);
  }
  PG_T(7, 3);
}

template <int MAXKB, int OCC, bool PADMASK, bool BIASKV, int HD = 64>
__global__ __launch_bounds__(256, OCC) void attention_long_kernel(const bf16_t* __restrict__ qkv, bf16_t* __restrict__ ctx, int T,
                                                               int H, int ld_qkv_, int ld_ctx_, int k_off, int v_off,
                                                               SeqLayout sl, int n_qchunk, const int32_t* __restrict__ key_tok_,
                                                               int pad_idx, const bf16_t* __restrict__ bias_kv_) {
  const int32_t* __restrict__ key_tok = PADMASK ? key_tok_ : nullptr;
  const bf16_t* __restrict__ bias_kv = BIASKV ? bias_kv_ : nullptr;
  constexpr int tpad = MAXKB * 16, nkc = MAXKB / 2;
  constexpr int ROW = HD * 2, NKK = score_steps(HD), NDB = HD / 16;
  typedef kfrag_t<HD> kf_t;
  __shared__ __attribute__((aligned(16))) char smem[2 * tpad * ROW + (PADMASK ? tpad : 0)];
  char* Ks = smem;
  char* Vs = smem + tpad * ROW;
  char* padf = smem + 2 * tpad * ROW;
  const int tid = threadIdx.x, lane = tid & 63, wave = tid >> 6;
  const int qc = blockIdx.x % n_qchunk, sh = blockIdx.x / n_qchunk;
  const int seq = sh / H, h = sh % H;
  const size_t row0 = (size_t)(seq / sl.inner_count) * sl.outer_rows + (size_t)(seq % sl.inner_count) * sl.inner_rows;
  const size_t ld_qkv = (size_t)ld_qkv_ * sl.row_step, ld_ctx = (size_t)ld_ctx_ * sl.row_step;
  const bf16_t* base = qkv + row0 * ld_qkv_ + h * HD;
  const int fr = lane & 15, fq = lane >> 4;
  const int q0 = qc * 64 + wave * 16;
  const bool active = q0 < T;
  kf_t qf[NKK];
  {
    int qrow = q0 + fr;
    if (qrow >= T) qrow = T - 1;
#pragma unroll
    for (int kk = 0; kk < NKK; ++kk) qf[kk] = q_frag<HD>(base + (size_t)qrow * ld_qkv, kk, fq);
  }
  f32x4 o[NDB];
#pragma unroll
  for (int db = 0; db < NDB; ++db) o[db] = (f32x4){0.f, 0.f, 0.f, 0.f};
  float m = -3.0e38f, l = 0.f;
  constexpr float LOG2E = 1.44269504088896341f;
  const int Tk = T + (bias_kv ? 1 : 0);

  for (int k0 = 0; k0 < Tk; k0 += tpad) {
    __syncthreads();
    stage_kv<tpad, 256, BIASKV, HD>(Ks, Vs, tid, base, ld_qkv, k_off, v_off, k0, T, bias_kv + h * HD, bias_kv + (H + h) * HD);
    if (PADMASK) {
      for (int key = tid; key < tpad; key += 256)
        padf[key] = (k0 + key < T && key_tok[row0 + (size_t)(k0 + key) * sl.row_step] == pad_idx) ? 1 : 0;
    }
    __syncthreads();
    if (!active) continue;
    f32x4 st[MAXKB];
#pragma unroll
    for (int kb = 0; kb < MAXKB; ++kb) {
      st[kb] = (f32x4){0.f, 0.f, 0.f, 0.f};
#pragma unroll
      for (int kk = 0; kk < NKK; ++kk) st[kb] = score_mfma(k_frag<HD>(Ks, kb * 16 + fr, kk, fq), qf[kk], st[kb]);
    }
    const int tl = Tk - k0 - fq * 4;
#pragma unroll
    for (int kb = 0; kb < MAXKB; ++kb) st[kb] = mask_tail(st[kb], kb, tl);
    float tmax = lane_max(st);
    if (PADMASK) {
      const float fill = sl.row_step == 1 ? -3.0e38f : -10000.0f;
      tmax = -3.0e38f;
#pragma unroll
      for (int kb = 0; kb < MAXKB; ++kb) {
        st[kb] = mask_pad(st[kb], *(const uint32_t*)(padf + kb * 16 + fq * 4), fill);
#pragma unroll
        for (int r = 0; r < 4; ++r) tmax = fmaxf(tmax, st[kb][r]);
      }
    }
    const float mn = fmaxf(m, rows4_max(tmax));
    const float alpha = __builtin_amdgcn_exp2f((m - mn) * LOG2E);
    const float mneg = -mn * LOG2E;
    float psum = 0.f;
#pragma unroll
    for (int kb = 0; kb < MAXKB; ++kb)
#pragma unroll
      for (int r = 0; r < 4; ++r) {
        const float e = __builtin_amdgcn_exp2f(fmaf(st[kb][r], LOG2E, mneg));
        st[kb][r] = e;
        psum += e;
      }
    psum = rows4_sum(psum);
    l = l * alpha + psum;
    m = mn;
#pragma unroll
    for (int db = 0; db < NDB; ++db) {
      o[db][0] *= alpha; o[db][1] *= alpha; o[db][2] *= alpha; o[db][3] *= alpha;
    }
#pragma unroll
    for (int c = 0; c < nkc; ++c) {
      const bf16x8 pf = p_frag(st[2 * c], st[2 * c + 1]);
#pragma unroll
      for (int db = 0; db < NDB; ++db) {
        VtFrag vf;
#pragma unroll
        for (int hh = 0; hh < 2; ++hh) vf.h[hh] = vt_half<HD>(Vs, (2 * c + hh) * 16, db, fr, fq);
        o[db] = mfma_op16(vf.v, pf, o[db]);
      }
    }
  }
  const int q = q0 + fr;
  if (active && q < T) store_ctx(o, 1.0f / l, ctx + row0 * ld_ctx_ + (size_t)q * ld_ctx + h * HD + fq * 4);
}

struct AttentionPlan {
  std::string error;
  bool whole = true;
  int kb = 0, hd = 64;
  bool pad = false, bias = false;
  int split_from = 0, split = 1;
  unsigned grid = 0;
  int n_qchunk = 0;
};

static AttentionPlan plan_attention(int64_t n_seq, int T, int H, int head_dim, bool has_pad, bool has_bias, int row_step, int n_cu) {
  AttentionPlan p;
  p.hd = head_dim, p.pad = has_pad, p.bias = has_bias;
  auto refuse = [&](const char* why) { p.error = why; return p; };
  p.error = attention_head_error(head_dim, has_bias);
  if (!p.error.empty() || n_seq == 0) return p;
  const int64_t pairs = n_seq * H;
  if (pairs > 0x7fffffff) return refuse("attention: too many sequences");
  if (T <= 0) return refuse("attention: empty sequence");
  p.kb = attention_rung(T + (has_bias ? 1 : 0), !has_bias, attention_max_keys(head_dim));
  p.whole = p.kb != 0;
  if (!p.whole) {
    p.n_qchunk = (T + 63) / 64;
    if (pairs * p.n_qchunk > 0x7fffffff) return refuse("attention: too many sequences");
    p.grid = (unsigned)(pairs * p.n_qchunk);
    return p;
  }
  p.grid = (unsigned)pairs;
  static const int split_on = env_int("PGIBBS_ATTN_SPLIT", 1);
  if (split_on && !has_pad && !has_bias && row_step == 1 && T >= 64) {
    const long slots = (long)n_cu * attention_resident(p.kb, head_dim);
    const long rem = pairs % slots;
    const int nqb = (T + 15) / 16;
    int sp = rem ? (int)(slots / rem) : 1;
    if (sp > 4) sp = 4;
    if (sp > nqb / 4) sp = nqb / 4;
    if (sp >= 2) {
      p.split = sp;
      p.split_from = (int)(pairs - rem);
      p.grid = (unsigned)(p.split_from + rem * sp);
    }
  }
  return p;
}

static std::string plan_text(const AttentionPlan& p) {
  if (!p.error.empty()) return "error: " + p.error;
  if (!p.grid) return "nothing";
  std::string t = (p.whole ? "whole kb" + std::to_string(p.kb) : std::string(p.hd == 128 ? "long t128" : "long t288")) + " hd" + std::to_string(p.hd);
  if (p.pad) t += " pad";
  if (p.bias) t += " bias";
  if (p.split > 1) return t + " split" + std::to_string(p.split) + " " + std::to_string(p.split_from) + "+" + std::to_string(p.grid - p.split_from) + "wg";
  return t + " " + std::to_string(p.grid) + "wg";
}
void attention_plan_text(int64_t n_seq, int T, int H, int head_dim, bool has_pad, bool has_bias, int row_step, int n_cu, std::string* text) {
  *text = plan_text(plan_attention(n_seq, T, H, head_dim, has_pad, has_bias, row_step, n_cu));
}

template <int KB, int HD, class... Args>
static void launch_rung(bool pad, bool bias, bool split, dim3 grid, hipStream_t s, Args... args) {
  auto go = [&](auto* kernel) { hipLaunchKernelGGL(kernel, grid, dim3(256), 0, s, args...); };
  if constexpr (coarse_rung(KB) && HD == 64) {
    if (bias && pad) return go(attention_kernel<KB, true, true, false, HD>);
    if (bias) return go(attention_kernel<KB, false, true, false, HD>);
  }
  if constexpr (KB * 16 <= attention_max_keys(HD)) {
    if (pad) go(attention_kernel<KB, true, false, false, HD>);
    else if (split) go(attention_kernel<KB, false, false, true, HD>);
    else go(attention_kernel<KB, false, false, false, HD>);
  }
}
template <int HD, class... Args>
static void launch_long(bool pad, bool bias, dim3 grid, hipStream_t s, Args... args) {
  auto go = [&](auto* kernel) { hipLaunchKernelGGL(kernel, grid, dim3(256), 0, s, args...); };
  if constexpr (HD == 64) {
    if (bias && pad) return go(attention_long_kernel<18, 2, true, true, HD>);
    if (bias) return go(attention_long_kernel<18, 2, false, true, HD>);
  }
  constexpr int KB = HD == 128 ? 8 : 18;
  if (pad) go(attention_long_kernel<KB, 2, true, false, HD>);
  else go(attention_long_kernel<KB, 2, false, false, HD>);
}

int launch_attention_seq_bf16(hipStream_t s, const bf16_t* qkv, bf16_t* ctx, int64_t n_seq, int T, int H, int ld_qkv,
                              int ld_ctx, int k_off, int v_off, SeqLayout sl, const int32_t* key_tok, int pad_idx,
                              const bf16_t* bias_kv, int head_dim) {
  const AttentionPlan p = plan_attention(n_seq, T, H, head_dim, key_tok != nullptr, bias_kv != nullptr, sl.row_step, device_cu_count());
  if (!p.error.empty()) return fail(1, p.error);
  if (!p.grid) return 0;
  note_kernel(plan_text(p).c_str());
  auto launch = [&](auto hd) {
    constexpr int HD = decltype(hd)::value;
    if (!p.whole)
      return launch_long<HD>(p.pad, p.bias, dim3(p.grid), s, qkv, ctx, T, H, ld_qkv, ld_ctx, k_off, v_off, sl, p.n_qchunk, key_tok,
                             pad_idx, bias_kv);
    visit_rung(p.kb, [&](auto kb) {
      launch_rung<decltype(kb)::value, HD>(p.pad, p.bias, p.split > 1, dim3(p.grid), s, qkv, ctx, T, H, ld_qkv, ld_ctx, k_off, v_off,
                                           sl, key_tok, pad_idx, bias_kv, p.split_from, p.split);
    });
  };
  visit_head_width(head_dim, launch);
  PG_HIP(hipGetLastError());
  return 0;
}

int launch_attention_bf16(hipStream_t s, const bf16_t* qkv, bf16_t* ctx, int B, int T, int H, int ld_qkv, int ld_ctx,
                          int k_off, int v_off, const int32_t* key_tok, int pad_idx, const bf16_t* bias_kv, int head_dim) {
  SeqLayout sl = {1, T, 0, 1};
  return launch_attention_seq_bf16(s, qkv, ctx, B, T, H, ld_qkv, ld_ctx, k_off, v_off, sl, key_tok, pad_idx, bias_kv, head_dim);
}

PG_OPS_END
```

### protein_gibbs_sampler_amd/csrc/engine.h

```cpp
#pragma once
#include <map>
#include <string>
#include <vector>

#include "kernels.h"

namespace pg {

#define OPS(fn, ...) (precision == PG_PREC_F16 ? opf16::fn(__VA_ARGS__) : opbf16::fn(__VA_ARGS__))

struct DevBuf {
  void* p = nullptr;
  size_t bytes = 0;
  int ensure(size_t need, hipStream_t s);
  void release();
  template <typename T> T* as() const { return (T*)p; }
};

struct Prof {
  struct Rec { int cls; hipEvent_t a, b; std::string kernels; };
  bool on = false;
  std::vector<Rec> recs;
  std::vector<hipEvent_t> pool;
  size_t used = 0;
  hipEvent_t get();
  void reset();
  void destroy();
};

enum ProfClass { PC_NONE = -1, PC_GEMM = 0, PC_ATTN, PC_LN, PC_EMBED, PC_HEAD, PC_SAMPLE, PC_GEMM_QKV, PC_GEMM_OUT, PC_GEMM_FC1, PC_GEMM_FC2,
                 PC_ROPE ,
                 PC_REPR_ROWS, PC_REPR_POOL ,
                 PC_ATTN_PROBS, PC_CONTACT , PC_COUNT };

struct DenseW {
  bf16_t* w = nullptr;
  float* b = nullptr;
  int N = 0, K = 0;
};
struct LnW { float* g = nullptr; float* b = nullptr; };

struct FfnW { LnW ln; DenseW fc1, fc2; };

struct EsmLayer {
  LnW ln1;
  DenseW qkv, out;
  FfnW ffn;
  bf16_t* bias_kv16 = nullptr;
  float* bias_kv32 = nullptr;
};
struct MsaLayer {
  LnW ln_row, ln_col;
  DenseW row_qkv, row_out, col_qkv, col_out;
  FfnW ffn;
  DenseW col_qkv_hm;
};

struct GraphKey {
  int32_t mask = 0, mask_idx = 0;
  const void *tok = nullptr, *idx = nullptr;
  int64_t B = 0, T = 0, P = 0;
  hipStream_t stream = nullptr;
  uint64_t epoch_pad = 0;
  int64_t job_items = 0;
  bool guided = false;
  bool operator==(const GraphKey& o) const {
    return mask == o.mask && mask_idx == o.mask_idx && tok == o.tok && idx == o.idx && B == o.B && T == o.T && P == o.P &&
           stream == o.stream && epoch_pad == o.epoch_pad && job_items == o.job_items && guided == o.guided;
  }
  void reset() { *this = GraphKey(); }
};

struct ReprTap {
  std::vector<int> layers;
  const int32_t* d_tok = nullptr;
  int B = 0, T = 0;
  const int32_t* d_pools = nullptr;
  int n_pools = 0;
  float* rows = nullptr;
  float* pooled = nullptr;
  size_t next = 0;
  bool wants_inner(int n_layers) const {
    for (int l : layers)
      if (l >= 1 && l < n_layers) return true;
    return false;
  }
};

struct ContactTap {
  const int32_t* d_tok = nullptr;
  int B = 0, T = 0;
  bool fold = false;
  float* logits = nullptr;
  float* contacts = nullptr;
  std::vector<int> attn_layers;
  float* attn_out = nullptr;
  size_t next_attn = 0;
  int folded = 0;
};

struct Engine {
  pg_model_config cfg;
  int device = 0;
  int precision = 0;
  hipStream_t own_stream = nullptr, stream = nullptr;
  bool strict() const { return precision == PG_PREC_FP32; }
  bool esm1() const { return cfg.arch == PG_ARCH_ESM1; }
  bool esm2() const { return cfg.arch == PG_ARCH_ESM2; }
  bool esm_family() const { return cfg.arch == PG_ARCH_ESM1B || cfg.arch == PG_ARCH_ESM1 || cfg.arch == PG_ARCH_ESM2; }

  ~Engine();
  int init(const pg_model_config* c, const pg_tensor* tensors, int n_tensors, int device_ordinal, int precision, int live_head = 0);
  int init_embedded(const pg_model_config* c, int head_slot, const pg_tensor* tensors, int n_tensors, int device_ordinal, int precision);

  std::vector<void*> owned;
  float *embed = nullptr, *pos = nullptr, *msa_pos = nullptr, *embed_out = nullptr;
  float embed_scale() const { return cfg.arch == PG_ARCH_ESM1 ? sqrtf((float)cfg.d_model) : 1.0f; }
  LnW ln_before, ln_after, head_ln;
  DenseW head_dense;
  float* head_bias = nullptr;
  std::vector<EsmLayer> esm_layers;
  std::vector<MsaLayer> msa_layers;
  int d_live = 0;
  bool embedded() const { return d_live != cfg.d_model; }
  int head_dim = 64;
  float* rope_tab = nullptr;
  int rope_rows = 0;
  PgChainLayerW* chain_layers = nullptr;

  DevBuf x, h, qkv, ctx, ffn, sel_h, sel_g, logits, d_tokens, d_idx, d_samp_tok, d_samp_logits, d_rowmap, scratch;
  DevBuf x_sel, ctx_sel, h_sel, ffn_sel;
  DevBuf tmp_idx, tmp_out;
  DevBuf splitk;
  DevBuf ffn_f32, scores;
  DevBuf chain_sync, chain_part;
  DevBuf repr_rows, repr_pooled, repr_ranges;
  int size_activations(int64_t Mp);
  float* splitk_ws(int rows, int n, int K, int64_t batch_rows);

  ReprTap* tap = nullptr;
  int tap_layer(int l);
  ContactTap* ctap = nullptr;
  int tap_attention(int l, const void* qkv_rows);
  float* contact_w = nullptr;
  float contact_bias = 0.f;
  int set_contact_head(const float* weight, int n_weights, float bias);
  DevBuf contact_P, contact_sums, contact_logits, contact_probs, contact_attn;

  bool esm_pad_in_batch = false;
  int64_t job_items = 0;
  int64_t order_items = 0;
  int64_t job_batch(int64_t B) const { return order_items > 0 ? order_items : (job_items > B ? job_items : B); }
  int64_t batch_rows_for(int64_t B, int64_t rows_per_item) const { return job_batch(B) * rows_per_item; }
  int64_t batch_rows = 0;
  int sel_gemm_rows(int64_t n_sel, int64_t Np) const;

  unsigned* chain_err = nullptr;
  int chain_check();
  bool chain_disabled = false, chain_retry = false;
  struct ChainCall {
    int32_t* d_tok; int B, T; const int32_t* d_idx; int n_iters, P; pg_sample_params sp; float* lg; int32_t* st; size_t snap_off;
  };
  std::vector<ChainCall> chain_log;
  bool chain_replay_ok = false;
  DevBuf chain_snap;
  static constexpr size_t kChainSnapBytes = 128, kChainLogMax = 64;
  bool chain_may_run(int B, int T) const;
  int chain_log_call(int32_t* d_tok, int B, int T, const int32_t* d_idx, int n_iters, int P, const pg_sample_params* sp, float* lg,
                     int32_t* st);
  unsigned* range_err = nullptr;
  int range_check();
  int finish_check() { int rc = chain_check(); return rc ? rc : range_check(); }

  DrawGuideDev guide;
  float *guide_bias_dev = nullptr, *guide_temps_dev = nullptr;
  int set_draw_guide(const pg_draw_guide* g);
  const DrawGuideDev* draw_guide() const { return guide.active() ? &guide : nullptr; }

  DevBuf d_iter;
  hipGraphExec_t graph_exec = nullptr;
  GraphKey graph_key;
  int64_t stat_graph_captures = 0, stat_graph_replays = 0;

  int dense3(const bf16_t* x3, const DenseW& W, float* out, int Mp, bool accumulate);
  int dense3_gelu(const bf16_t* x3, const DenseW& W, int Mp, const DenseW* next = nullptr);
  bool dense3_wants_dup(const DenseW& W, int Mp, bool gelu = false) const;
  template <typename Attn> int strict_attention(const LnW& ln, const DenseW& qkv_w, const DenseW& out_w, int Mi, int64_t M, Attn&& attn);
  int ffn_strict(const FfnW& F, int Mi, int64_t M);

  Prof prof;
  template <typename F> int timed(int cls, F&& f);
  int embed_rows(const int32_t* d_tok, int64_t M, int T, int rows_per_msa, const LnW* first_ln);
  int dense(int cls, const bf16_t* a, const DenseW& W, void* out, int rows, int epi, int m_live = 0, bool splitk = false);
  int dense_ln(const float* x, const LnW& ln, const DenseW& W, bf16_t* out, int rows, int epi);
  int layer_norm(const float* x, const LnW& ln, bf16_t* h, int64_t M, bool dup = true, int colmajor_R = 0, int colmajor_C = 0);
  int resid_gemm_ln(int cls, const bf16_t* a, const DenseW& W, float* x, int rows, int64_t M_real, const LnW& ln, bf16_t* h,
                    bool splitk = false, int colmajor_R = 0, int colmajor_C = 0);
  int rope(void* qkv_rows, int64_t M, int T);
  int ffn_block(const DenseW& out, const FfnW& F, const LnW* next_ln, int Mi, int64_t M, bool folded = false);
  bool prune_last(int64_t n_draws, int64_t token_rows) const;
  int pruned_tail(const DenseW& out, const FfnW& F, const int32_t* sel_idx, const int32_t* sel_row_map, int P, int width, int64_t n_sel,
                  const int32_t* d_iter, int Ni, bool ln_in_gemm);
  enum ChainRan { CHAIN_NOT_RUN, CHAIN_TO_LAST_ATTENTION, CHAIN_WHOLE_FORWARD };
  int chain_forward(int B, int T, int Mi, bool stop_at_last_attention, ChainRan* ran);
  int esm_trunk(const int32_t* d_tok, int B, int T, const int32_t* sel_idx, int P, int64_t n_sel, const int32_t* d_iter);
  int msa_trunk(const int32_t* d_tok, int B, int R, int C, const int32_t* sel_idx, const int32_t* sel_row_map, int P, int64_t n_sel);
  int trunk(const int32_t* d_tok, int B, int R, int C, const int32_t* sel_idx = nullptr, const int32_t* sel_row_map = nullptr, int P = 0,
            int64_t n_sel = 0, const int32_t* d_iter = nullptr);
  int head(const int32_t* d_idx, const int32_t* d_row_map, int P, int width, int64_t n_sel, float* d_logits,
           const float* x_src = nullptr);

  int check_call(bool msa, int B, int R, int C, int count0 = 0, int count1 = 0, int row0 = 0, int row1 = 0) const;
  struct GuideRowShift {
    DrawGuideDev& g;
    const float* bias;
    GuideRowShift(Engine& e, int64_t row0, int C) : g(e.guide), bias(e.guide.bias) {
      if (g.bias && g.bias_rows > 1) g.bias += (size_t)row0 * C * g.n_valid;
    }
    ~GuideRowShift() { g.bias = bias; }
  };
  int masked_logits(int32_t* d_tok, int B, int R, int C, const int32_t* idx, const int32_t* mask_map, const int32_t* sel_map,
                    int64_t n_rows, int P, bool mask, int mask_idx, float* lg, const int32_t* dit = nullptr);
  int esm_gibbs_device(int32_t* d_tok, int B, int T, const int32_t* d_idx, int n_iters, int P, const pg_sample_params* sp,
                       float* d_samp_logits, int32_t* d_samp_tok);
  int msa_gibbs_device(int32_t* d_tok, int B, int R, int C, const int32_t* d_idx, int n_iters, int P,
                       const pg_sample_params* sp, float* d_samp_logits, int32_t* d_samp_tok);
  int msa_single_device(int32_t* d_tok, int B, int R, int C, int mask_row, int target_row, const int32_t* d_step_idx,
                        const int32_t* step_sample_flag_host, int n_steps, int P_max, const pg_sample_params* sp,
                        float* d_samp_logits, int32_t* d_samp_tok);
};

template <typename Tb, typename Tt, typename Copy>
int template_block_rows(Tb* block, Tt* table, int n_steps, int B, int b0, int nb, size_t row, Copy&& copy) {
  for (int s = 0; s < n_steps && row > 0; ++s)
    if (int rc = copy(block + (size_t)s * nb * row, table + ((size_t)s * B + b0) * row, (size_t)nb * row)) return rc;
  return PG_OK;
}

std::vector<float> rope_table(int rows, int hd = 64, int live = 0);
struct EmbedShape { int n_heads, width, slot, d_ffn, vocab; };
bool embedded_image(const std::string& name, const EmbedShape& es, const float* src, int64_t* rows, int64_t* cols, std::vector<float>* image);
int embedded_check(const pg_model_config* c, int head_slot);

struct TensorMap {
  std::map<std::string, const pg_tensor*> m;
  const float* get(const std::string& name, int64_t numel, std::string& err) const;
};

}

struct pg_engine {
  pg::Engine e;
};
```

### protein_gibbs_sampler_amd/csrc/engine.hip

```cpp
#include <algorithm>

#include "engine.h"

#include <math.h>
#include <stdlib.h>
#include <string.h>

#include "gemm_epilogue.h"
#include "ln_row.h"

namespace pg {

static thread_local std::string g_last_error;
void set_error(const std::string& msg) { g_last_error = msg; }
int fail(int code, const std::string& msg) {
  g_last_error = msg;
  return code;
}
const char* last_error_cstr() { return g_last_error.c_str(); }

static thread_local std::string g_noted;
void note_kernel(const char* label, long tiles, int splits) {
  if (g_noted.size() > 512) return;
  if (!g_noted.empty()) g_noted += " + ";
// ... 277 lines not shown
  device = device_ordinal;
  PG_HIP(hipStreamCreateWithFlags(&own_stream, hipStreamNonBlocking));
  stream = own_stream;

  std::vector<std::vector<float>> images;
  std::vector<pg_tensor> run_tensors;
  if (live_head) {
    const EmbedShape es = {cfg.n_heads, live_head, head_dim, cfg.d_ffn, cfg.vocab};
    images.resize(n_tensors);
    for (int i = 0; i < n_tensors; ++i) {
      int64_t r = 0, cc = 0;
      if (!tensors[i].name || !embedded_image(tensors[i].name, es, nullptr, &r, &cc, nullptr)) continue;
      if (tensors[i].numel != r * cc)
        return fail(PG_ERR_WEIGHTS, std::string("tensor '") + tensors[i].name + "' has " + std::to_string(tensors[i].numel) + " elements, expected " + std::to_string(r * cc));
      embedded_image(tensors[i].name, es, tensors[i].data, &r, &cc, &images[i]);
      run_tensors.push_back({tensors[i].name, images[i].data(), (int64_t)images[i].size()});
    }
    tensors = run_tensors.data();
    n_tensors = (int)run_tensors.size();
  }
  TensorMap tm;
  for (int i = 0; i < n_tensors; ++i)
    if (tensors[i].name) tm.m[tensors[i].name] = &tensors[i];
  Uploader up{this, &tm, prec, ""};
  const int d = cfg.d_model, f = cfg.d_ffn, V = cfg.vocab;
  const float qs = live_head ? (float)pow((double)live_head, -0.5) : hw->q_scale;
  bool ok = true;
  ok = ok && (embed = up.f32("embed_tokens.weight", (int64_t)V * d));
  if (!esm2()) ok = ok && (pos = up.f32("embed_positions.weight", (int64_t)(cfg.max_positions + cfg.pad_idx + 1) * d));
  if (esm1()) {
    ok = ok && (embed_out = up.f32("embed_out.weight", (int64_t)V * d));
    ok = ok && (head_bias = up.f32("embed_out.bias", V));
  } else {
    if (!esm2()) ok = ok && up.ln(ln_before, "emb_layer_norm_before", d);
    ok = ok && up.ln(ln_after, "emb_layer_norm_after", d);
    ok = ok && up.dense(head_dense, {"lm_head.dense"}, {1.0f}, d, d);
    ok = ok && up.ln(head_ln, "lm_head.layer_norm", d);
    ok = ok && (head_bias = up.f32("lm_head.bias", V));
  }
  if (ok && cfg.arch != PG_ARCH_MSA1B) {
    esm_layers.resize(cfg.n_layers);
    for (int i = 0; ok && i < cfg.n_layers; ++i) {
      const std::string p = "layers." + std::to_string(i) + ".";
      EsmLayer& L = esm_layers[i];
      ok = ok && up.ln(L.ln1, p + "self_attn_layer_norm", d);
      ok = ok && up.dense(L.qkv, {p + "self_attn.q_proj", p + "self_attn.k_proj", p + "self_attn.v_proj"}, {qs, 1.f, 1.f}, d, d);
      ok = ok && up.dense(L.out, {p + "self_attn.out_proj"}, {1.f}, d, d);
      ok = ok && up.ln(L.ffn.ln, p + "final_layer_norm", d);
      ok = ok && up.dense(L.ffn.fc1, {p + "fc1"}, {1.f}, f, d);
      ok = ok && up.dense(L.ffn.fc2, {p + "fc2"}, {1.f}, d, f);
      if (ok && esm1()) ok = up.bias_kv(L, p + "self_attn.bias_k", p + "self_attn.bias_v", d);
    }
  } else if (ok) {
    ok = ok && (msa_pos = up.f32("msa_position_embedding", (int64_t)cfg.max_msa_rows * d));
    msa_layers.resize(cfg.n_layers);
    for (int i = 0; ok && i < cfg.n_layers; ++i) {
      const std::string p = "layers." + std::to_string(i) + ".";
      MsaLayer& L = msa_layers[i];
      const std::string r = p + "row_self_attention.", cpre = p + "column_self_attention.", ff = p + "feed_forward_layer.";
      ok = ok && up.ln(L.ln_row, r + "layer_norm", d);
      ok = ok && up.dense(L.row_qkv, {r + "layer.q_proj", r + "layer.k_proj", r + "layer.v_proj"}, {1.f, 1.f, 1.f}, d, d);
      ok = ok && up.dense(L.row_out, {r + "layer.out_proj"}, {1.f}, d, d);
      ok = ok && up.ln(L.ln_col, cpre + "layer_norm", d);
      ok = ok && up.dense(L.col_qkv, {cpre + "layer.q_proj", cpre + "layer.k_proj", cpre + "layer.v_proj"}, {qs, 1.f, 1.f}, d, d);
      if (ok && !strict()) ok = up.headmajor(L.col_qkv_hm, L.col_qkv, cfg.n_heads);
      ok = ok && up.dense(L.col_out, {cpre + "layer.out_proj"}, {1.f}, d, d);
      ok = ok && up.ln(L.ffn.ln, ff + "layer_norm", d);
      ok = ok && up.dense(L.ffn.fc1, {ff + "layer.fc1"}, {1.f}, f, d);
      ok = ok && up.dense(L.ffn.fc2, {ff + "layer.fc2"}, {1.f}, d, f);
    }
  }
  if (!ok) return fail(PG_ERR_WEIGHTS, up.err.empty() ? std::string("weight upload failed") : up.err);
  if (esm2()) {
    if (cfg.max_positions < 1) return fail(PG_ERR_INVALID, "max_positions must be positive");
    rope_rows = cfg.max_positions + 2;
    const std::vector<float> tab = rope_table(rope_rows, head_dim, live_head);
    void* dt = nullptr;
    PG_HIP(hipMalloc(&dt, tab.size() * 4));
    owned.push_back(dt);
    PG_HIP(hipMemcpy(dt, tab.data(), tab.size() * 4, hipMemcpyHostToDevice));
    rope_tab = (float*)dt;
  }
  if (cfg.arch == PG_ARCH_ESM1B && !strict() && OPS(chain_trunk_ok, 32, d, f, cfg.n_heads)) {
    std::vector<PgChainLayerW> tab(cfg.n_layers);
    for (int i = 0; i < cfg.n_layers; ++i) {
      const EsmLayer& L = esm_layers[i];
      tab[i] = {L.ln1.g, L.ln1.b, L.qkv.w, L.qkv.b, L.out.w, L.out.b, L.ffn.ln.g, L.ffn.ln.b, L.ffn.fc1.w, L.ffn.fc1.b, L.ffn.fc2.w, L.ffn.fc2.b};
    }
    void* dt = nullptr;
    PG_HIP(hipMalloc(&dt, tab.size() * sizeof(PgChainLayerW)));
    owned.push_back(dt);
    PG_HIP(hipMemcpy(dt, tab.data(), tab.size() * sizeof(PgChainLayerW), hipMemcpyHostToDevice));
    chain_layers = (PgChainLayerW*)dt;
    PG_HIP(hipHostMalloc((void**)&chain_err, sizeof(unsigned), hipHostMallocMapped));
    *chain_err = 0;
  }
  PG_HIP(hipHostMalloc((void**)&range_err, sizeof(unsigned), hipHostMallocMapped));
  *range_err = 0;
  PG_HIP(hipStreamSynchronize(stream));
  return PG_OK;
}

int Engine::range_check() {
  if (!range_err || !*range_err) return PG_OK;
  *range_err = 0;
  return fail(PG_ERR_RANGE, precision == PG_PREC_F16
                                ? "non-finite logits: a 16-bit tensor of the forward left the fp16 range (+-65504) -- run this model with "
                                  "precision bf16 (or fp32); the results of this call are invalid"
                                : "non-finite logits (NaN / inf in the weights or an overflow in the forward); the results of this call are invalid");
}

bool Engine::chain_may_run(int B, int T) const {
  if (!(chain_layers && chain_err && !chain_disabled && !esm_pad_in_batch && T >= 1 && T <= 32 && (int64_t)B * T <= 32)) return false;
  const int64_t M = (int64_t)B * T;
  const int Mi = round_up((int)M, 16);
  const int d = cfg.d_model, f = cfg.d_ffn;
  if (batch_rows_for(B, T) > 2048 && Mi < 64) return false;
  return gemm_ln_skinny_ok(Mi, 3 * d, d) && gemm_ln_skinny_ok(Mi, f, d) && OPS(chain_trunk_ok, Mi, d, f, cfg.n_heads);
}

int Engine::chain_log_call(int32_t* d_tok, int B, int T, const int32_t* d_idx_, int n_iters, int P, const pg_sample_params* sp,
                           float* lg, int32_t* st) {
  int rc;
  if (chain_log.size() >= kChainLogMax) {
    PG_HIP(hipStreamSynchronize(stream));
    if ((rc = chain_check()) && !chain_replay_ok) return rc;
    chain_retry = false;
    if (chain_disabled) return PG_OK;
  }
  if ((rc = chain_snap.ensure(kChainSnapBytes * kChainLogMax, stream))) return rc;
  const size_t off = chain_log.size() * kChainSnapBytes;
  PG_HIP(hipMemcpyAsync((char*)chain_snap.p + off, d_tok, (size_t)B * T * 4, hipMemcpyDeviceToDevice, stream));
  chain_log.push_back({d_tok, B, T, d_idx_, n_iters, P, *sp, lg, st, off});
  return PG_OK;
}

int Engine::chain_check() {
  chain_replay_ok = false;
  if (!chain_err || !*chain_err) { chain_log.clear(); return PG_OK; }
  *chain_err = 0;
  if (range_err) *range_err = 0;
  if (chain_sync.p) (void)hipMemsetAsync(chain_sync.p, 0, chain_sync.bytes, stream);
  if (graph_exec) { (void)hipGraphExecDestroy(graph_exec); graph_exec = nullptr; graph_key.reset(); }
  if (!chain_disabled)
    fprintf(stderr, "pgibbs: a device-wide barrier of the persistent single-chain trunk timed out (another persistent grid on this GPU?); "
                    "this engine uses the per-layer launches from now on\n");
  chain_disabled = true;
  chain_retry = true;
  if (!chain_log.empty()) {
    std::vector<ChainCall> log;
    log.swap(chain_log);
    std::vector<int32_t*> seen;
    for (const ChainCall& c : log) {
      if (std::find(seen.begin(), seen.end(), c.d_tok) == seen.end()) {
        seen.push_back(c.d_tok);
        PG_HIP(hipMemcpyAsync(c.d_tok, (char*)chain_snap.p + c.snap_off, (size_t)c.B * c.T * 4, hipMemcpyDeviceToDevice, stream));
      }
      int rc = esm_gibbs_device(c.d_tok, c.B, c.T, c.d_idx, c.n_iters, c.P, &c.sp, c.lg, c.st);
      if (rc) return rc;
    }
    PG_HIP(hipStreamSynchronize(stream));
    chain_replay_ok = true;
    return fail(PG_ERR_HIP, "single-chain trunk: a device-wide barrier timed out; the device-pointer calls since the last "
                            "synchronisation were run again on the per-layer launches (their results are valid)");
  }
  return fail(PG_ERR_HIP, "single-chain trunk: a device-wide barrier timed out (is another persistent kernel sharing this GPU? "
                          "PGIBBS_CHAIN_TRUNK=0 selects the per-layer launches); the results of this call are invalid");
}

int Engine::dense(int cls, const bf16_t* a, const DenseW& W, void* out, int rows, int epi, int m_live, bool use_splitk) {
  float* ws = use_splitk ? splitk_ws(rows, W.N, W.K, batch_rows) : nullptr;
  const size_t ws_bytes = use_splitk ? splitk.bytes : 0;
  return timed(cls, [&] { return OPS(launch_gemm_bf16, stream, a, W.w, W.b, out, rows, W.N, W.K, W.K, W.K, W.N, epi, ws, ws_bytes, m_live); });
}

int Engine::dense_ln(const float* x, const LnW& ln, const DenseW& W, bf16_t* out, int rows, int epi) {
  return timed(PC_GEMM, [&] { return OPS(launch_gemm_ln_skinny, stream, x, W.K, ln.g, ln.b, cfg.layer_norm_eps, W.w, W.b, out, rows, W.N, W.K, W.K, W.N, epi); });
}

int Engine::layer_norm(const float* x, const LnW& ln, bf16_t* h, int64_t M, bool dup, int colmajor_R, int colmajor_C) {
  return timed(PC_LN, [&] { return OPS(launch_layernorm_bf16, stream, x, ln.g, ln.b, h, M, cfg.d_model, cfg.layer_norm_eps, strict(), colmajor_R, colmajor_C, dup, d_live); });
}

int Engine::embed_rows(const int32_t* d_tok, int64_t M, int T, int rows_per_msa, const LnW* first_ln) {
  return timed(PC_EMBED, [&] {
    return OPS(launch_embed_ln, stream, d_tok, embed, pos, msa_pos, ln_before.g, ln_before.b, x.as<float>(), M, T, cfg.d_model, cfg.pad_idx,
                           cfg.mask_idx, rows_per_msa ? 0 : cfg.token_dropout, rows_per_msa, cfg.layer_norm_eps, first_ln ? first_ln->g : nullptr,
                           first_ln ? first_ln->b : nullptr, first_ln ? h.as<bf16_t>() : nullptr, embed_scale(), d_live);
  });
}

int Engine::dense3(const bf16_t* x3, const DenseW& W, float* out, int Mp, bool accumulate) {
  return timed(PC_GEMM, [&] { return launch_gemm_split3(stream, x3, W.w, W.b, out, Mp, W.N, W.K, W.N, accumulate ? EPI_F32_RESID : EPI_F32); });
}

int Engine::sel_gemm_rows(int64_t n_sel, int64_t Np) const {
  if (n_sel > 256) return (int)Np;
  const int r = round_up((int)n_sel, 16);
  return (batch_rows > 2048 && r < 64) ? 64 : r;
}

bool Engine::dense3_wants_dup(const DenseW& W, int Mp, bool gelu) const {
  static const int nodup = env_int("PGIBBS_SPLIT3_NODUP", 1);
  if (!nodup) return true;
  if (gelu && W.N % 256 == 0 && Mp % 256 == 0) return false;
  return !gemm_split3_fused(Mp, W.N, W.K, EPI_F32);
}

int Engine::dense3_gelu(const bf16_t* x3, const DenseW& W, int Mp, const DenseW* next) {
  if (W.N % 256 == 0 && Mp % 256 == 0) {
    const int epi = next && !dense3_wants_dup(*next, Mp) ? EPI_SPLIT2_GELU : EPI_SPLIT3_GELU;
    return timed(PC_GEMM, [&] { return launch_gemm_split3(stream, x3, W.w, W.b, ffn.as<bf16_t>(), Mp, W.N, W.K, 3 * W.N, epi); });
  }
  int rc = ffn_f32.ensure((size_t)Mp * W.N * 4, stream);
  if (rc || (rc = dense3(x3, W, ffn_f32.as<float>(), Mp, false))) return rc;
  return timed(PC_LN, [&] { return launch_split3_bf16(stream, ffn_f32.as<float>(), ffn.as<bf16_t>(), Mp, W.N, 1.f, true, false); });
}

float* Engine::splitk_ws(int rows, int n, int K, int64_t batch_rows) {
  if (rows > 2048 || batch_rows > 2048) return nullptr;
  const size_t need = OPS(gemm_splitk_ws_bytes, rows, n, K);
  if (splitk.bytes < need && splitk.ensure(need, stream)) return nullptr;
  return splitk.as<float>();
}

std::vector<float> rope_table(int rows, int hd, int live) {
  const int half = hd / 2, lhalf = live > 0 ? live / 2 : half;
  std::vector<float> tab((size_t)rows * hd);
  for (int i = 0; i < half; ++i) {
    if (i >= lhalf) {
      for (int t = 0; t < rows; ++t) tab[(size_t)t * hd + i] = 1.0f, tab[(size_t)t * hd + half + i] = 0.0f;
      continue;
    }
    const float inv_freq = 1.0f / (float)pow(10000.0, (double)((float)(2 * i) / (float)(2 * lhalf)));
    for (int t = 0; t < rows; ++t) {
      const float ang = (float)t * inv_freq;
      tab[(size_t)t * hd + i] = (float)cos((double)ang);
      tab[(size_t)t * hd + half + i] = (float)sin((double)ang);
    }
  }
  return tab;
}

int Engine::rope(void* qkv_rows, int64_t M, int T) {
  if (!esm2()) return PG_OK;
  return timed(PC_ROPE, [&] { return OPS(launch_rope, stream, qkv_rows, strict(), rope_tab, rope_rows, M, T, cfg.n_heads, 3 * cfg.d_model, head_dim); });
}

int Engine::size_activations(int64_t Mp) {
  if (Mp > 0x7fffffff / 4) return fail(PG_ERR_INVALID, "too many tokens in one call");
  const size_t d = cfg.d_model, f = cfg.d_ffn;
  const size_t w = strict() ? 3 : 1;
  int rc;
  if ((rc = x.ensure((size_t)Mp * d * 4, stream))) return rc;
  if ((rc = h.ensure((size_t)Mp * w * d * 2, stream))) return rc;
  if ((rc = qkv.ensure((size_t)Mp * 3 * d * (strict() ? 4 : 2), stream))) return rc;
  if ((rc = ctx.ensure((size_t)Mp * w * d * 2, stream))) return rc;
  return ffn.ensure((size_t)Mp * w * f * 2, stream);
}

int Engine::ffn_strict(const FfnW& F, int Mi, int64_t M) {
  float* X = x.as<float>();
  bf16_t* H3 = h.as<bf16_t>();
  int rc;
  if ((rc = layer_norm(X, F.ln, H3, M, dense3_wants_dup(F.fc1, Mi, true)))) return rc;
  if ((rc = dense3_gelu(H3, F.fc1, Mi, &F.fc2))) return rc;
  return dense3(ffn.as<bf16_t>(), F.fc2, X, Mi, true);
}

template <typename Attn>
int Engine::strict_attention(const LnW& ln, const DenseW& qkv_w, const DenseW& out_w, int Mi, int64_t M, Attn&& attn) {
  float* X = x.as<float>();
  bf16_t* H3 = h.as<bf16_t>();
  int rc;
  if ((rc = layer_norm(X, ln, H3, M, dense3_wants_dup(qkv_w, Mi)))) return rc;
  if ((rc = dense3(H3, qkv_w, qkv.as<float>(), Mi, false))) return rc;
  if ((rc = attn(dense3_wants_dup(out_w, Mi) ? cfg.d_model : -cfg.d_model))) return rc;
  return dense3(ctx.as<bf16_t>(), out_w, X, Mi, true);
}

int Engine::ffn_block(const DenseW& out, const FfnW& F, const LnW* next_ln, int Mi, int64_t M, bool folded) {
  float* X = x.as<float>();
  bf16_t* Hh = h.as<bf16_t>();
  bf16_t* CTX = ctx.as<bf16_t>();
  bf16_t* FFN = ffn.as<bf16_t>();
  int rc;
  if (folded) {
    if ((rc = dense(PC_GEMM, CTX, out, X, Mi, EPI_F32_RESID))) return rc;
    if ((rc = dense_ln(X, F.ln, F.fc1, FFN, Mi, EPI_BF16_GELU))) return rc;
    return dense(PC_GEMM, FFN, F.fc2, X, Mi, EPI_F32_RESID, (int)M, true);
  }
  if ((rc = resid_gemm_ln(PC_GEMM_OUT, CTX, out, X, Mi, M, F.ln, Hh))) return rc;
  if ((rc = dense(PC_GEMM_FC1, Hh, F.fc1, FFN, Mi, EPI_BF16_GELU, (int)M))) return rc;
  if (next_ln) return resid_gemm_ln(PC_GEMM_FC2, FFN, F.fc2, X, Mi, M, *next_ln, Hh, true);
  return dense(PC_GEMM_FC2, FFN, F.fc2, X, Mi, EPI_F32_RESID, (int)M, true);
}

bool Engine::prune_last(int64_t n_draws, int64_t token_rows) const {
  static const int prune = env_int("PGIBBS_PRUNE_LAST", 1);
  return prune && !strict() && n_draws > 0 && 2 * n_draws < token_rows;
}

int Engine::pruned_tail(const DenseW& out, const FfnW& F, const int32_t* sel_idx, const int32_t* sel_row_map, int P, int width,
                        int64_t n_sel, const int32_t* d_iter_, int Ni, bool ln_in_gemm) {
  const int d = cfg.d_model, f = cfg.d_ffn;
  const int64_t Np = round_up64(n_sel, kRowPad);
  int rc;
  if ((rc = x_sel.ensure((size_t)Np * d * 4, stream)) || (rc = ctx_sel.ensure((size_t)Np * d * 2, stream)) ||
      (rc = h_sel.ensure((size_t)Np * d * 2, stream)) || (rc = ffn_sel.ensure((size_t)Np * f * 2, stream))) return rc;
  float* XS = x_sel.as<float>();
  bf16_t* HS = h_sel.as<bf16_t>();
  bf16_t* FS = ffn_sel.as<bf16_t>();
  rc = timed(PC_HEAD, [&] {
    int r2 = launch_gather_rows(stream, x.as<float>(), XS, sel_idx, sel_row_map, P, width, n_sel, d * 4, d_iter_);
    if (r2) return r2;
    return launch_gather_rows(stream, ctx.as<bf16_t>(), ctx_sel.as<bf16_t>(), sel_idx, sel_row_map, P, width, n_sel, d * 2, d_iter_);
  });
  if (rc) return rc;
  if ((rc = dense(PC_GEMM, ctx_sel.as<bf16_t>(), out, XS, Ni, EPI_F32_RESID))) return rc;
  if (ln_in_gemm && gemm_ln_skinny_ok(Ni, f, d)) {
    if ((rc = dense_ln(XS, F.ln, F.fc1, FS, Ni, EPI_BF16_GELU))) return rc;
  } else {
    if ((rc = layer_norm(XS, F.ln, HS, n_sel))) return rc;
    if ((rc = dense(PC_GEMM, HS, F.fc1, FS, Ni, EPI_BF16_GELU))) return rc;
  }
  return dense(PC_GEMM, FS, F.fc2, XS, Ni, EPI_F32_RESID, 0, true);
}

int Engine::trunk(const int32_t* d_tok, int B, int R, int C, const int32_t* sel_idx, const int32_t* sel_row_map, int P, int64_t n_sel,
                  const int32_t* d_iter_) {
  return cfg.arch == PG_ARCH_MSA1B ? msa_trunk(d_tok, B, R, C, sel_idx, sel_row_map, P, n_sel) : esm_trunk(d_tok, B, C, sel_idx, P, n_sel, d_iter_);
}

int Engine::tap_layer(int l) {
  if (!tap || tap->next >= tap->layers.size() || tap->layers[tap->next] != l) return PG_OK;
  const size_t i = tap->next++;
  const int64_t M = (int64_t)tap->B * tap->T;
  const bool ln = l == cfg.n_layers && !esm1();
  float* rows = tap->rows + i * (size_t)M * d_live;
  int rc = timed(PC_REPR_ROWS, [&] {
    return launch_repr_rows(stream, x.as<float>(), ln ? ln_after.g : nullptr, ln ? ln_after.b : nullptr, tap->d_tok, cfg.pad_idx, rows, M,
                            cfg.d_model, d_live, cfg.layer_norm_eps);
  });
  if (rc || !tap->pooled) return rc;
  float* means = tap->pooled + i * (size_t)tap->n_pools * tap->B * d_live;
  return timed(PC_REPR_POOL, [&] { return launch_repr_pool(stream, rows, tap->d_pools, means, tap->n_pools, tap->B, tap->T, d_live); });
}

int Engine::tap_attention(int l, const void* qkv_rows) {
  if (!ctap) return PG_OK;
  ContactTap& t = *ctap;
  const int d = cfg.d_model, H = cfg.n_heads;
  const size_t map = (size_t)t.B * H * t.T * t.T;
  float* Pl = contact_P.as<float>();
  if (t.next_attn < t.attn_layers.size() && t.attn_layers[t.next_attn] == l) Pl = t.attn_out + map * t.next_attn++;
  const SeqLayout chain = {1, t.T, 0, 1};
  const int32_t* key_tok = esm_pad_in_batch ? t.d_tok : nullptr;
  int rc = timed(PC_ATTN_PROBS, [&] {
    if (strict()) return launch_attn_probs_f32(stream, (const float*)qkv_rows, Pl, t.B, t.T, H, 3 * d, d, chain, key_tok, cfg.pad_idx, head_dim);
    return OPS(launch_attn_probs, stream, (const bf16_t*)qkv_rows, Pl, t.B, t.T, H, 3 * d, d, chain, key_tok, cfg.pad_idx, head_dim);
  });
  ++t.folded;
  if (rc || !t.fold) return rc;
  return timed(PC_CONTACT, [&] {
    return launch_contact_accumulate(stream, Pl, t.d_tok, cfg.eos_idx, cfg.pad_idx, contact_w + (size_t)l * H, contact_bias, l == 0,
                                     l == cfg.n_layers - 1, contact_sums.as<float>(), t.logits, t.contacts, t.B, t.T, H);
  });
}

int Engine::set_contact_head(const float* weight, int n_weights, float bias) {
  if (contact_w) {
    PG_HIP(hipStreamSynchronize(stream));
    PG_HIP(hipFree(contact_w));
    contact_w = nullptr;
  }
  if (!weight) return PG_OK;
  PG_HIP(hipMalloc((void**)&contact_w, (size_t)n_weights * 4));
  PG_HIP(hipMemcpy(contact_w, weight, (size_t)n_weights * 4, hipMemcpyHostToDevice));
  contact_bias = bias;
  return PG_OK;
}

int Engine::esm_trunk(const int32_t* d_tok, int B, int T, const int32_t* sel_idx, int P, int64_t n_sel, const int32_t* d_iter_) {
  const int d = cfg.d_model, f = cfg.d_ffn;
  const int64_t M = (int64_t)B * T;
  const int64_t Mp = round_up64(M, kRowPad);
  int rc;
  if ((rc = size_activations(Mp))) return rc;
  batch_rows = batch_rows_for(B, T);
  float* X = x.as<float>();
  if (strict()) {
    float* QKVf = qkv.as<float>();
    const int Mi = (int)Mp;
    if ((rc = embed_rows(d_tok, M, T, 0, nullptr)) || (rc = tap_layer(0))) return rc;
    const SeqLayout chain = {1, T, 0, 1};
    for (int l = 0; l < cfg.n_layers; ++l) {
      const EsmLayer& L = esm_layers[l];
      rc = strict_attention(L.ln1, L.qkv, L.out, Mi, M, [&](int split_d) {
        int r = rope(QKVf, M, T);
        if (r || (r = tap_attention(l, QKVf))) return r;
        return timed(PC_ATTN, [&] { return launch_attention_f32(stream, QKVf, ctx.as<bf16_t>(), split_d, B, T, cfg.n_heads, 3 * d, 3 * d, d, 2 * d, chain, esm_pad_in_batch ? d_tok : nullptr, cfg.pad_idx, L.bias_kv32, head_dim); });
      });
      if (rc || (rc = ffn_strict(L.ffn, Mi, M)) || (rc = tap_layer(l + 1))) return rc;
    }
    return PG_OK;
  }
  bf16_t* Hh = h.as<bf16_t>();
  bf16_t* QKV = qkv.as<bf16_t>();
  bf16_t* CTX = ctx.as<bf16_t>();
  const int Mi = sel_gemm_rows(M, Mp);
  const bool ln_in_gemm = !embedded() && gemm_ln_skinny_ok(Mi, 3 * d, d) && gemm_ln_skinny_ok(Mi, f, d);

  if ((rc = embed_rows(d_tok, M, T, 0, ln_in_gemm ? nullptr : &esm_layers[0].ln1)) || (rc = tap_layer(0))) return rc;
  ChainRan ran = CHAIN_NOT_RUN;
  const bool tap_inside = tap && tap->wants_inner(cfg.n_layers);
  if (ln_in_gemm && !tap_inside && !ctap && (rc = chain_forward(B, T, Mi, sel_idx != nullptr, &ran))) return rc;
  if (ran == CHAIN_WHOLE_FORWARD) return tap_layer(cfg.n_layers);
  const EsmLayer& tail = esm_layers.back();
  auto finish_selected = [&] { return pruned_tail(tail.out, tail.ffn, sel_idx, nullptr, P, T, n_sel, d_iter_, sel_gemm_rows(n_sel, round_up64(n_sel, kRowPad)), ln_in_gemm); };
  if (ran == CHAIN_TO_LAST_ATTENTION) return finish_selected();
  for (int l = 0; l < cfg.n_layers; ++l) {
    const EsmLayer& L = esm_layers[l];
    if ((rc = ln_in_gemm ? dense_ln(X, L.ln1, L.qkv, QKV, Mi, EPI_BF16) : dense(PC_GEMM_QKV, Hh, L.qkv, QKV, Mi, EPI_BF16))) return rc;
    if ((rc = rope(QKV, M, T)) || (rc = tap_attention(l, QKV))) return rc;
    if ((rc = timed(PC_ATTN, [&] { return OPS(launch_attention_bf16, stream, QKV, CTX, B, T, cfg.n_heads, 3 * d, d, d, 2 * d, esm_pad_in_batch ? d_tok : nullptr, cfg.pad_idx, L.bias_kv16, head_dim); }))) return rc;
    const bool last = l == cfg.n_layers - 1;
    if (sel_idx && last) return finish_selected();
    if ((rc = ffn_block(L.out, L.ffn, last ? nullptr : &esm_layers[l + 1].ln1, Mi, M, ln_in_gemm)) || (rc = tap_layer(l + 1))) return rc;
  }
  return PG_OK;
}

int Engine::chain_forward(int B, int T, int Mi, bool stop_at_last_attention, ChainRan* ran) {
  const int d = cfg.d_model, f = cfg.d_ffn;
  if (!(chain_layers && !chain_disabled && !esm_pad_in_batch && T <= 32 && (int64_t)B * T <= Mi && OPS(chain_trunk_ok, Mi, d, f, cfg.n_heads))) return PG_OK;
  int rc;
  if ((rc = chain_sync.ensure(OPS(chain_trunk_sync_bytes), stream)) || (rc = chain_part.ensure(OPS(chain_trunk_part_bytes, Mi, d), stream))) return rc;
  PgChainTrunkArgs ca;
  ca.layers = chain_layers; ca.n_layers = cfg.n_layers; ca.partial_last = stop_at_last_attention ? 1 : 0; ca.B = B; ca.T = T;
  ca.x = x.as<float>(); ca.qkv = qkv.as<bf16_t>(); ca.ctx = ctx.as<bf16_t>(); ca.ffn = ffn.as<bf16_t>();
  ca.part = chain_part.as<float>(); ca.sync = chain_sync.as<unsigned>();
  ca.err = chain_err; ca.eps = cfg.layer_norm_eps;
  rc = timed(PC_GEMM, [&] { return OPS(launch_chain_trunk, stream, ca, Mi, d); });
  if (rc == kChainTrunkUnfit) {
    chain_disabled = true;
    return PG_OK;
  }
  if (rc) return rc;
  static const int fault_at = env_int("PGIBBS_CHAIN_TRUNK_FAULT", 0);
  static int launches = 0;
  if (fault_at > 0 && ++launches == fault_at) *chain_err = 1;
  *ran = stop_at_last_attention ? CHAIN_TO_LAST_ATTENTION : CHAIN_WHOLE_FORWARD;
  return PG_OK;
}

int Engine::resid_gemm_ln(int cls, const bf16_t* a, const DenseW& W, float* x, int M_rows, int64_t M_real, const LnW& ln, bf16_t* h,
                          bool use_splitk, int colmajor_R, int colmajor_C) {
  const int rc = dense(cls, a, W, x, M_rows, EPI_F32_RESID, (int)M_real, use_splitk);
  return rc ? rc : layer_norm(x, ln, h, M_real, true, colmajor_R, colmajor_C);
}

int Engine::head(const int32_t* d_idx_, const int32_t* d_row_map, int P, int width, int64_t n_sel, float* d_logits,
                 const float* x_src) {
  if (!x_src) x_src = x.as<float>();
  const int d = cfg.d_model, V = cfg.vocab;
  const int64_t Np = round_up64(n_sel, kRowPad);
  int rc;
  if (esm1()) {
    const float* rows = x_src;
    if (d_idx_) {
      if ((rc = sel_g.ensure((size_t)Np * d * 4, stream))) return rc;
      if ((rc = launch_gather_rows(stream, x_src, sel_g.as<float>(), d_idx_, d_row_map, P, width, n_sel, d * 4))) return rc;
      rows = sel_g.as<float>();
    }
    return timed(PC_HEAD, [&] { return launch_lm_tail(stream, rows, nullptr, nullptr, embed_out, head_bias, d_logits, n_sel, d, V, cfg.layer_norm_eps); });
  }
  if ((rc = sel_h.ensure((size_t)Np * d * 2, stream))) return rc;
  if ((rc = sel_g.ensure((size_t)Np * d * 4, stream))) return rc;
  const float eps = cfg.layer_norm_eps;
  if (strict()) {
    if ((rc = sel_h.ensure((size_t)Np * 3 * d * 2, stream))) return rc;
    if ((rc = OPS(launch_gather_ln_bf16, stream, x_src, d_idx_, d_row_map, P, width, ln_after.g, ln_after.b,
                                    sel_h.as<bf16_t>(), n_sel, d, eps, true, d_live))) return rc;
    if ((rc = dense3(sel_h.as<bf16_t>(), head_dense, sel_g.as<float>(), (int)Np, false))) return rc;
    if ((rc = launch_gelu_f32(stream, sel_g.as<float>(), Np * d))) return rc;
    return launch_lm_tail(stream, sel_g.as<float>(), head_ln.g, head_ln.b, embed, head_bias, d_logits, n_sel, d, V, eps, d_live);
  }
  return timed(PC_HEAD, [&] {
    int r = OPS(launch_gather_ln_bf16, stream, x_src, d_idx_, d_row_map, P, width, ln_after.g, ln_after.b,
                                  sel_h.as<bf16_t>(), n_sel, d, eps, false, d_live);
    if (r) return r;
    if ((r = dense(PC_NONE, sel_h.as<bf16_t>(), head_dense, sel_g.as<float>(), sel_gemm_rows(n_sel, Np), EPI_F32_GELU))) return r;
    return launch_lm_tail(stream, sel_g.as<float>(), head_ln.g, head_ln.b, embed, head_bias, d_logits, n_sel, d, V, eps, d_live);
  });
}

int Engine::masked_logits(int32_t* d_tok, int B, int R, int C, const int32_t* idx, const int32_t* mask_map, const int32_t* sel_map,
                          int64_t n_rows, int P, bool mask, int mask_idx, float* lg, const int32_t* dit) {
  const int64_t n_draws = n_rows * P;
  int rc;
  if (mask && P > 0)
    if ((rc = timed(PC_SAMPLE, [&] { return launch_mask_scatter(stream, d_tok, C, idx, mask_map, n_rows, P, mask_idx, dit); }))) return rc;
  const bool pruned = prune_last(n_draws, (int64_t)B * R * C);
  if ((rc = trunk(d_tok, B, R, C, pruned ? idx : nullptr, sel_map, P, n_draws, dit))) return rc;
  if (P == 0) return PG_OK;
  return pruned ? head(nullptr, nullptr, 1, 1, n_draws, lg, x_sel.as<float>()) : head(idx, sel_map, P, C, n_draws, lg);
}

int Engine::esm_gibbs_device(int32_t* d_tok, int B, int T, const int32_t* d_idx_, int n_iters, int P,
                             const pg_sample_params* sp, float* d_samp_logits_, int32_t* d_samp_tok_) {
  int rc = check_call(false, B, 1, T, n_iters, P);
  if (rc) return rc;
  if (B == 0 || n_iters == 0) return PG_OK;
  const int V = cfg.vocab;
  const int64_t n_sel_rows = B;
  const int64_t n_draws = (int64_t)B * P;
  if (!d_samp_logits_ && (rc = logits.ensure((size_t)(n_draws > 0 ? n_draws : 1) * V * 4, stream))) return rc;
  static const int use_graph = env_int("PGIBBS_GRAPH", 1);
  const bool pruned = prune_last(n_draws, (int64_t)B * T);

  auto iteration = [&](int it, const int32_t* dit) -> int {
    const int32_t* idx_it = dit ? d_idx_ : d_idx_ + (size_t)it * n_draws;
    float* lg = d_samp_logits_ ? d_samp_logits_ + (size_t)it * n_draws * V : logits.as<float>();
    int r = masked_logits(d_tok, B, 1, T, idx_it, nullptr, nullptr, n_sel_rows, P, sp->mask, sp->mask_idx, lg, dit);
    if (r || P == 0) return r;
    int32_t* st = d_samp_tok_ ? d_samp_tok_ + (size_t)it * n_draws : nullptr;
    return timed(PC_SAMPLE, [&] { return launch_sample_writeback(stream, d_tok, T, lg, V, 1, idx_it, nullptr, n_sel_rows, P, sp, dit ? 0 : it, st, dit, range_err, draw_guide()); });
  };

  const bool graphable = use_graph && pruned && !prof.on && !d_samp_logits_ && !d_samp_tok_ && (int64_t)B * T <= 4096;
  auto epoch_pad = [&] { return g_alloc_epoch * 2 + (esm_pad_in_batch ? 1 : 0); };
  GraphKey key;
  if (graphable) key = {sp->mask, sp->mask_idx, d_tok, d_idx_, B, T, P, stream, epoch_pad(), job_items, draw_guide() != nullptr};
  const bool reuse = graphable && graph_exec && key == graph_key;
  if (!graphable || (!reuse && n_iters < 3)) {
    for (int it = 0; it < n_iters; ++it)
      if ((rc = iteration(it, nullptr))) return rc;
    return PG_OK;
  }
  int first = 0;
  if (!reuse) {
    if ((rc = d_iter.ensure(graph_state_bytes(), stream))) return rc;
    if ((rc = iteration(0, nullptr))) return rc;
    first = 1;
    key.epoch_pad = epoch_pad();
    if (graph_exec) { (void)hipGraphExecDestroy(graph_exec); graph_exec = nullptr; }
    hipGraph_t graph = nullptr;
    PG_HIP(hipStreamBeginCapture(stream, hipStreamCaptureModeThreadLocal));
    rc = iteration(0, d_iter.as<int32_t>());
    if (!rc) rc = launch_iter_counter(stream, d_iter.as<int32_t>(), false, 0);
    hipError_t ce = hipStreamEndCapture(stream, &graph);
    if (rc) { if (graph) (void)hipGraphDestroy(graph); return rc; }
    if (ce != hipSuccess) return fail(PG_ERR_HIP, std::string("hipStreamEndCapture: ") + hipGetErrorString(ce));
    ce = hipGraphInstantiate(&graph_exec, graph, nullptr, nullptr, 0);
    (void)hipGraphDestroy(graph);
    if (ce != hipSuccess) { graph_exec = nullptr; return fail(PG_ERR_HIP, std::string("hipGraphInstantiate: ") + hipGetErrorString(ce)); }
    graph_key = key;
    ++stat_graph_captures;
  }
  if ((rc = launch_graph_state(stream, d_iter.as<int32_t>(), first, sp, draw_guide()))) return rc;
  for (int it = first; it < n_iters; ++it) PG_HIP(hipGraphLaunch(graph_exec, stream));
  stat_graph_replays += n_iters - first;
  return PG_OK;
}

int Engine::msa_trunk(const int32_t* d_tok, int B, int R, int C, const int32_t* sel_idx, const int32_t* sel_row_map, int P,
                      int64_t n_sel) {
  const int d = cfg.d_model, H = cfg.n_heads;
  const int64_t M = (int64_t)B * R * C;
  const int64_t Mp = round_up64(M, kRowPad);
  int rc;
  if ((rc = size_activations(Mp))) return rc;
  batch_rows = batch_rows_for(B, (int64_t)R * C);
  float* X = x.as<float>();
  bf16_t* Hh = h.as<bf16_t>();
  bf16_t* QKV = qkv.as<bf16_t>();
  bf16_t* CTX = ctx.as<bf16_t>();
  const int Mi = (int)Mp;
  const float row_scale = 0.125f / sqrtf((float)R);
  const int32_t* pad_tok = esm_pad_in_batch ? d_tok : nullptr;
  if (pad_tok && precision == PG_PREC_F16)
    return fail(PG_ERR_UNSUPPORTED, "fp16 precision mode: batches with <pad> (ragged MSA lists) take the scores-through-scratch row "
                                    "attention, which exists for bf16 operands only -- use precision bf16 or fp32");
  if (strict()) {
    if ((rc = scores.ensure((size_t)B * H * C * msa_row_scores_ld(C) * 4, stream))) return rc;
    float* QKVf = qkv.as<float>();
    if ((rc = embed_rows(d_tok, M, C, R, nullptr))) return rc;
    const SeqLayout colS = {C, R * C, 1, C};
    for (const MsaLayer& L : msa_layers) {
      rc = strict_attention(L.ln_row, L.row_qkv, L.row_out, Mi, M, [&](int split_d) {
        return timed(PC_ATTN, [&] { return launch_msa_row_attention_f32(stream, QKVf, scores.as<float>(), CTX, split_d, B, R, C, H, 3 * d, 3 * d, d, 2 * d, row_scale, pad_tok, cfg.pad_idx); });
      });
      if (rc) return rc;
      rc = strict_attention(L.ln_col, L.col_qkv, L.col_out, Mi, M, [&](int split_d) {
        return timed(PC_ATTN, [&] { return launch_attention_f32(stream, QKVf, CTX, split_d, (int64_t)B * C, R, H, 3 * d, 3 * d, d, 2 * d, colS, pad_tok, cfg.pad_idx); });
      });
      if (rc || (rc = ffn_strict(L.ffn, Mi, M))) return rc;
    }
    return PG_OK;
  }

  if ((rc = embed_rows(d_tok, M, C, R, &msa_layers[0].ln_row))) return rc;
  const SeqLayout col = {C, R * C, 1, C};
  for (int l = 0; l < cfg.n_layers; ++l) {
    const MsaLayer& L = msa_layers[l];
    if ((rc = dense(PC_GEMM_QKV, Hh, L.row_qkv, QKV, Mi, EPI_BF16))) return rc;
    if (C <= 576 && !pad_tok) {
      float* part = nullptr;
      const size_t need = msa_row_split_scratch_bytes(B, R, C, H, (int)(job_batch(B) * H));
      if (need) {
        if (need > ((size_t)1 << 31)) return fail(PG_ERR_INVALID, "too many MSAs in one call for the row-split attention scratch: use smaller batches");
        if ((rc = scores.ensure(need, stream))) return rc;
        part = scores.as<float>();
      }
      if ((rc = timed(PC_ATTN, [&] { return OPS(launch_msa_row_attention_bf16, stream, QKV, CTX, B, R, C, H, 3 * d, d, d, 2 * d, row_scale, part, part ? scores.bytes : 0, (int)(job_batch(B) * H)); }))) return rc;
    } else {
      if (precision == PG_PREC_F16)
        return fail(PG_ERR_UNSUPPORTED, "fp16 precision mode: alignments wider than 576 columns take the split-bf16 row attention, "
                                        "which exists for bf16 operands only -- use precision bf16 or fp32");
      if ((rc = scratch.ensure((size_t)Mp * 3 * d * 4, stream)) || (rc = scores.ensure((size_t)B * H * C * msa_row_scores_ld(C) * 4, stream))) return rc;
      rc = timed(PC_ATTN, [&] {
        int r2 = launch_bf16_to_f32(stream, QKV, scratch.as<float>(), (int64_t)M * 3 * d);
        if (r2) return r2;
        return launch_msa_row_attention_f32(stream, scratch.as<float>(), scores.as<float>(), CTX, 0, B, R, C, H,
                                            3 * d, d, d, 2 * d, row_scale, pad_tok, cfg.pad_idx);
      });
      if (rc) return rc;
    }
    const bool col_fused = !pad_tok && colattn_ok(R, d, H) && L.col_qkv_hm.w;
    if ((rc = resid_gemm_ln(PC_GEMM_OUT, CTX, L.row_out, X, Mi, M, L.ln_col, Hh, false, col_fused ? R : 0, col_fused ? C : 0))) return rc;
    if (col_fused) {
      if ((rc = timed(PC_GEMM_QKV, [&] { return OPS(launch_gemm_colattn, stream, Hh, L.col_qkv_hm.w, L.col_qkv_hm.b, CTX, B, R, C, H, d, d); }))) return rc;
    } else {
      if ((rc = dense(PC_GEMM_QKV, Hh, L.col_qkv, QKV, Mi, EPI_BF16))) return rc;
      if ((rc = timed(PC_ATTN, [&] { return OPS(launch_attention_seq_bf16, stream, QKV, CTX, (int64_t)B * C, R, H, 3 * d, d, d, 2 * d, col, pad_tok, cfg.pad_idx, nullptr); }))) return rc;
    }
    const bool last = l == cfg.n_layers - 1;
    if (sel_idx && last) return pruned_tail(L.col_out, L.ffn, sel_idx, sel_row_map, P, C, n_sel, nullptr, (int)round_up64(n_sel, kRowPad), false);
    if ((rc = ffn_block(L.col_out, L.ffn, last ? nullptr : &msa_layers[l + 1].ln_row, Mi, M))) return rc;
  }
  return PG_OK;
}

int Engine::set_draw_guide(const pg_draw_guide* g) {
  int rc;
  if (g && (rc = check_draw_guide_tables(g, "pg_engine_set_draw_guide"))) return rc;
  DrawGuideDev next;
  if (g) {
    next.top_p = g->top_p;
    if (g->bias) { next.bias_rows = g->bias_rows; next.width = g->width; next.n_valid = g->n_valid; }
    if (g->temperatures) next.n_temps = g->n_temperatures;
  }
  const bool had = guide_bias_dev || guide_temps_dev;
  if (!had && !(g && (g->bias || g->temperatures))) {
    guide = next;
    return PG_OK;
  }
  PG_HIP(hipStreamSynchronize(stream));
  if (guide_bias_dev) (void)hipFree(guide_bias_dev);
  if (guide_temps_dev) (void)hipFree(guide_temps_dev);
  guide_bias_dev = guide_temps_dev = nullptr;
  guide = DrawGuideDev();
  if (g && g->bias) {
    const size_t bytes = (size_t)g->bias_rows * g->width * g->n_valid * 4;
    PG_HIP(hipMalloc((void**)&guide_bias_dev, bytes));
    PG_HIP(hipMemcpyAsync(guide_bias_dev, g->bias, bytes, hipMemcpyHostToDevice, stream));
    next.bias = guide_bias_dev;
  }
  if (g && g->temperatures) {
    PG_HIP(hipMalloc((void**)&guide_temps_dev, (size_t)g->n_temperatures * 4));
    PG_HIP(hipMemcpyAsync(guide_temps_dev, g->temperatures, (size_t)g->n_temperatures * 4, hipMemcpyHostToDevice, stream));
    next.temps = guide_temps_dev;
  }
  PG_HIP(hipStreamSynchronize(stream));
  guide = next;
  return PG_OK;
}

int Engine::check_call(bool msa, int B, int R, int C, int count0, int count1, int row0, int row1) const {
  if (msa && cfg.arch != PG_ARCH_MSA1B) return fail(PG_ERR_INVALID, "engine was not built for the MSA-1b architecture");
  if (!msa && !esm_family()) return fail(PG_ERR_INVALID, "engine was not built for an ESM-1b / ESM-1 / ESM-2 architecture");
  if (B < 0 || R < 1 || C < 1) return fail(PG_ERR_INVALID, "bad shape");
  if (msa && R > cfg.max_msa_rows) return fail(PG_ERR_INVALID, "MSA has more rows than msa_position_embedding");
  if (C > cfg.max_positions)
    return fail(PG_ERR_INVALID, msa ? "alignment longer than the learned position table" : "sequence longer than the learned position table");
  if (count0 < 0 || count1 < 0) return fail(PG_ERR_INVALID, "bad shape");
  if (row0 < 0 || row0 >= R || row1 < 0 || row1 >= R) return fail(PG_ERR_INVALID, "row index out of range");
  return PG_OK;
}

int Engine::msa_gibbs_device(int32_t* d_tok, int B, int R, int C, const int32_t* d_idx_, int n_iters, int P,
                             const pg_sample_params* sp, float* d_samp_logits_, int32_t* d_samp_tok_) {
  int rc = check_call(true, B, R, C, n_iters, P);
  if (rc) return rc;
  if (B == 0 || n_iters == 0) return PG_OK;
  const int V = cfg.vocab;
  const int64_t n_sel_rows = (int64_t)B * R;
  const int64_t n_draws = n_sel_rows * P;
  if (!d_samp_logits_ && (rc = logits.ensure((size_t)(n_draws > 0 ? n_draws : 1) * V * 4, stream))) return rc;
  for (int it = 0; it < n_iters; ++it) {
    const int32_t* idx_it = d_idx_ + (size_t)it * n_draws;
    float* lg = d_samp_logits_ ? d_samp_logits_ + (size_t)it * n_draws * V : logits.as<float>();
    if ((rc = masked_logits(d_tok, B, R, C, idx_it, nullptr, nullptr, n_sel_rows, P, sp->mask, sp->mask_idx, lg))) return rc;
    if (P == 0) continue;
    int32_t* st = d_samp_tok_ ? d_samp_tok_ + (size_t)it * n_draws : nullptr;
    if ((rc = timed(PC_SAMPLE, [&] { return launch_sample_writeback(stream, d_tok, C, lg, V, 1, idx_it, nullptr, n_sel_rows, P, sp, it, st, nullptr, range_err, draw_guide()); }))) return rc;
  }
  return PG_OK;
}

int Engine::msa_single_device(int32_t* d_tok, int B, int R, int C, int mask_row, int target_row, const int32_t* d_step_idx,
                              const int32_t* step_sample_flag_host, int n_steps, int P_max, const pg_sample_params* sp,
                              float* d_samp_logits_, int32_t* d_samp_tok_) {
  int rc = check_call(true, B, R, C, n_steps, P_max, mask_row, target_row);
  if (rc) return rc;
  if (n_steps == 0 || B == 0) return PG_OK;
  const int V = cfg.vocab;
  if (B > 1 && (int64_t)R * C <= 2048) {
    auto copy = [&](auto* dst, const auto* src, size_t n) -> int {
      PG_HIP(hipMemcpyAsync(dst, src, n * sizeof(*dst), hipMemcpyDeviceToDevice, stream));
      return PG_OK;
    };
    auto to_table = [&](auto* block, auto* table, size_t n) { return copy(table, block, n); };
    const size_t n1 = (size_t)n_steps * (P_max > 0 ? P_max : 1);
    for (int b = 0; b < B; ++b) {
// ... 52 lines not shown
```

### protein_gibbs_sampler_amd/csrc/kernels_ops.inc

```
int launch_gemm_bf16(hipStream_t s, const bf16_t* X, const bf16_t* W, const float* bias, void* out, int M, int N, int K,
                     int ldx, int ldw, int ldo, int epi, float* ws = nullptr, size_t ws_bytes = 0, int m_live = 0);
int gemm_splitk_splits(int K);
size_t gemm_splitk_ws_bytes(int M, int N, int K);
int launch_gemm_bf16_variant(hipStream_t s, const bf16_t* X, const bf16_t* W, const float* bias, void* out, int M, int N,
                             int K, int ldx, int ldw, int ldo, int epi, int variant, float* ws = nullptr, size_t ws_bytes = 0,
                             int m_live = 0);

bool gemm_ln_skinny_ok(int M, int N, int K);
int launch_gemm_ln_skinny(hipStream_t s, const float* X, int ldx, const float* gamma, const float* beta, float eps, const bf16_t* W,
                          const float* bias, void* out, int M, int N, int K, int ldw, int ldo, int epi, int nb_force = 0);
bool chain_trunk_ok(int M, int d_model, int d_ffn, int n_heads);
size_t chain_trunk_sync_bytes();
size_t chain_trunk_part_bytes(int M, int d_model);
int launch_chain_trunk(hipStream_t s, const PgChainTrunkArgs& a, int M, int d_model);
int launch_gemm_big(hipStream_t s, const bf16_t* X, const bf16_t* W, const float* bias, void* out, int M, int N, int K, int ldx,
                    int ldw, int ldo, int epi, int m_live = 0);
void gemm_plan_text(int M, int N, int K, int epi, int variant, bool have_ws, int m_live, int n_cu, std::string* text);
void gemm_big_geometry(int M, int N, int K, int* m_main_panels, int* tail_rows);
int launch_gemm_w16(hipStream_t s, const bf16_t* X, const bf16_t* W, const float* bias, void* out, int M, int N, int K, int ldx,
                    int ldw, int ldo, int epi, int tail_rows = 0);
int launch_gemm_split3(hipStream_t s, const bf16_t* X3, const bf16_t* W3, const float* bias, void* out, int M, int N, int K, int ldo,
                       int epi);
bool gemm_split3_fused(int M, int N, int K, int epi);
int launch_gemm_split3_w16(hipStream_t s, const bf16_t* X3, const bf16_t* W3, const float* bias, void* out, int M, int N, int K,
                           int ldo, int epi);

int launch_attention_bf16(hipStream_t s, const bf16_t* qkv, bf16_t* ctx, int B, int T, int H, int ld_qkv, int ld_ctx,
                          int k_off, int v_off, const int32_t* key_tok = nullptr, int pad_idx = -1, const bf16_t* bias_kv = nullptr,
                          int head_dim = 64);
int launch_attention_seq_bf16(hipStream_t s, const bf16_t* qkv, bf16_t* ctx, int64_t n_seq, int T, int H, int ld_qkv,
                              int ld_ctx, int k_off, int v_off, SeqLayout sl, const int32_t* key_tok = nullptr,
                              int pad_idx = -1, const bf16_t* bias_kv = nullptr, int head_dim = 64);
size_t msa_row_split_scratch_bytes(int B, int R, int C, int H, int order_bh);
void attention_plan_text(int64_t n_seq, int T, int H, int head_dim, bool has_pad, bool has_bias, int row_step, int n_cu, std::string* text);
void attention_f32_plan_text(int64_t n_seq, int T, int H, int head_dim, bool has_pad, bool has_bias, std::string* text);
void msa_row_plan_text(int B, int R, int C, int H, int order_bh, std::string* text);
void msa_row_f32_plan_text(int B, int R, int C, int H, std::string* text);
int launch_attn_probs(hipStream_t s, const bf16_t* qkv, float* P, int64_t n_seq, int T, int H, int ld_qkv, int k_off, SeqLayout sl,
                      const int32_t* key_tok = nullptr, int pad_idx = -1, int head_dim = 64);
int launch_attn_probs_f32(hipStream_t s, const float* qkv, float* P, int64_t n_seq, int T, int H, int ld_qkv, int k_off, SeqLayout sl,
                          const int32_t* key_tok = nullptr, int pad_idx = -1, int head_dim = 64);
void attn_probs_plan_text(int64_t n_seq, int T, int H, int head_dim, bool has_pad, std::string* text);
void attn_probs_f32_plan_text(int64_t n_seq, int T, int H, int head_dim, bool has_pad, std::string* text);
int launch_msa_row_attention_bf16(hipStream_t s, const bf16_t* qkv, bf16_t* ctx, int B, int R, int C, int H, int ld_qkv,
                                  int ld_ctx, int k_off, int v_off, float scale, float* partial = nullptr,
                                  size_t partial_bytes = 0, int order_bh = 0);

int launch_embed_ln(hipStream_t s, const int32_t* tokens, const float* embed, const float* pos, const float* msa_pos,
                    const float* gamma, const float* beta, float* x, int64_t n_tok, int T, int d, int pad_idx,
                    int mask_idx, int token_dropout, int rows_per_msa, float eps,
                    const float* gamma2 = nullptr, const float* beta2 = nullptr, bf16_t* h2 = nullptr,
                    float embed_scale = 1.0f,
                    int d_live = 0);
int launch_rope(hipStream_t s, void* qkv, bool f32, const float* table, int table_rows, int64_t M, int T, int H, int ld,
                int head_dim = 64);
int launch_layernorm_bf16(hipStream_t s, const float* x, const float* gamma, const float* beta, bf16_t* h, int64_t M,
                          int d, float eps, bool split3 = false,
                          int colmajor_R = 0, int colmajor_C = 0,
                          bool split3_dup = true,
                          int d_live = 0);
int layernorm_bf16_check(int64_t M, int d, bool split3, int colmajor_R, int colmajor_C, int d_live = 0);
int layernorm_bf16_choice(int64_t M, int d, int colmajor_R, unsigned* stride_grid, int d_live = 0);
bool colattn_ok(int R, int d_model, int n_heads);
int launch_gemm_colattn(hipStream_t s, const bf16_t* X, const bf16_t* W, const float* bias, bf16_t* ctx, int B, int R, int C, int H,
                        int d, int ld_ctx);
int launch_headmajor_qkv(hipStream_t s, const bf16_t* w, const float* b, bf16_t* w2, float* b2, int H, int K);
int launch_layernorm_f32(hipStream_t s, const float* x, const float* gamma, const float* beta, float* y, int64_t M, int d,
                         float eps, int d_live = 0);
int launch_gather_ln_bf16(hipStream_t s, const float* x, const int32_t* idx, const int32_t* row_map, int P, int width,
                          const float* gamma, const float* beta, bf16_t* h, int64_t n_sel, int d, float eps,
                          bool split3 = false, int d_live = 0);
int launch_split3_bf16(hipStream_t s, const float* src, bf16_t* dst, int64_t rows, int K, float scale, bool gelu, bool weight);
int launch_gelu_f32(hipStream_t s, float* p, int64_t n);
int launch_attention_f32(hipStream_t s, const float* qkv, bf16_t* ctx, int split_d, int64_t n_seq, int T, int H,
                         int ld_qkv, int ld_ctx, int k_off, int v_off, SeqLayout sl, const int32_t* key_tok = nullptr,
                         int pad_idx = -1, const float* bias_kv = nullptr,
                         int head_dim = 64);
static inline int msa_row_scores_ld(int C) { return (C + 3) & ~3; }
int launch_msa_row_attention_f32(hipStream_t s, const float* qkv, float* scores, bf16_t* ctx, int split_d, int B, int R,
                                 int C, int H, int ld_qkv, int ld_ctx, int k_off, int v_off, float scale,
                                 const int32_t* tok = nullptr, int pad_idx = -1);
int launch_gather_rows(hipStream_t s, const void* src, void* dst, const int32_t* idx, const int32_t* row_map, int P, int width,
                       int64_t n_sel, int row_bytes, const int32_t* d_iter = nullptr);
int launch_lm_tail(hipStream_t s, const float* g, const float* gamma, const float* beta, const float* embed,
                   const float* out_bias, float* logits, int64_t n, int d, int V, float eps, int d_live = 0);
bool lm_tail_small(int64_t n, int d);
int launch_f32_to_bf16(hipStream_t s, const float* src, bf16_t* dst, int64_t n, float scale);
int launch_bf16_to_f32(hipStream_t s, const bf16_t* src, float* dst, int64_t n);
int launch_scale_f32(hipStream_t s, float* p, int64_t n, float scale);
```

Before: 72810 sampled positions/s.

## Compute last-layer queries only at sampled positions and skip dead key blocks

In the final ESM-1b layer, the full QKV GEMM now produces only K and V for all rows. The LN'd rows at the sampled positions are gathered, Q is computed just for them, and a new indexed attention kernel yields context only for those queries, which the pruned tail consumes directly. Separately, attention kernels gain a DEADLAST variant that skips score and PV MFMAs for a final 16-key block lying wholly past T (T=258 fits in kb-1 blocks when the rung rounds up). This trims last-layer Q projection and attention work but adds an extra gather and a small GEMM launch. It also relies on there being no RoPE for ESM-1b.

```diff
diff --git a/include/pgibbs.h b/include/pgibbs.h
--- a/include/pgibbs.h
+++ b/include/pgibbs.h
@@ -213,6 +213,11 @@
 PG_API int pg_dbg_rope_hd(int device, int precision, float* qkv_inout, int B, int T, int H, int head_dim);
 PG_API int pg_dbg_attention_kv(int device, int precision, const float* qkv, float* ctx, int B, int T, int H, int head_dim,
                         const int32_t* key_tok, int pad_idx, const float* bias_k, const float* bias_v, char* plan, int plan_bytes);
+PG_API int pg_attn_dbg_blocks(int device, int precision, const float* qkv, float* ctx, int B, int T, int H, int head_dim,
+                            int all_blocks, char* plan, int plan_bytes);
+PG_API int pg_attn_dbg_bench(int device, int precision, int B, int T, int H, int head_dim, int all_blocks, int iters, double* avg_ms);
+PG_API int pg_attn_dbg_indexed(int device, int precision, const float* qkv, const int32_t* idx, float* ctx_sel, int B, int T, int H,
+                             int P, char* plan, int plan_bytes);
 
 PG_API int pg_dbg_msa_attention(int device, int which, const float* qkv, float* ctx, int B, int R, int C, int H, float scale);
 PG_API int pg_dbg_msa_attention_tok(int device, int which, const float* qkv, float* ctx, int B, int R, int C, int H, float scale,
diff --git a/protein_gibbs_sampler_amd/_lib.py b/protein_gibbs_sampler_amd/_lib.py
--- a/protein_gibbs_sampler_amd/_lib.py
+++ b/protein_gibbs_sampler_amd/_lib.py
@@ -126,6 +126,9 @@
     ("pg_contact_dbg_probs", c_int, [c_int, c_int, c_void_p, c_int, c_int, c_int, c_int, c_void_p, c_int, c_void_p, c_char_p, c_int]),
     ("pg_contact_dbg_accumulate", c_int, [c_int, c_void_p, c_void_p, c_int, c_int, c_void_p, c_float, c_int, c_int, c_void_p, c_void_p,
                                           c_int, c_int, c_int]),
+    ("pg_attn_dbg_blocks", c_int, [c_int, c_int, c_void_p, c_void_p, c_int, c_int, c_int, c_int, c_int, c_char_p, c_int]),
+    ("pg_attn_dbg_bench", c_int, [c_int, c_int, c_int, c_int, c_int, c_int, c_int, c_int, POINTER(c_double)]),
+    ("pg_attn_dbg_indexed", c_int, [c_int, c_int, c_void_p, c_void_p, c_void_p, c_int, c_int, c_int, c_int, c_char_p, c_int]),
     ("pg_comm_unique_id", c_int, [c_void_p]),
     ("pg_comm_create", c_int, [c_int, c_int, c_void_p, c_int, POINTER(c_void_p)]),
     ("pg_comm_destroy", None, [c_void_p]),
@@ -200,6 +203,8 @@
             pass
     handle = ctypes.CDLL(LIB_PATH, mode=ctypes.RTLD_GLOBAL)
     for name, restype, argtypes in SIGNATURES:
+        if name.startswith("pg_attn_dbg_") and os.environ.get("PGIBBS_LIB_PATH") and not hasattr(handle, name):
+            continue
         fn = getattr(handle, name)
         fn.restype = restype
         fn.argtypes = argtypes
diff --git a/protein_gibbs_sampler_amd/csrc/api_dbg.hip b/protein_gibbs_sampler_amd/csrc/api_dbg.hip
--- a/protein_gibbs_sampler_amd/csrc/api_dbg.hip
+++ b/protein_gibbs_sampler_amd/csrc/api_dbg.hip
@@ -375,6 +375,81 @@
   });
 }
 
+int pg_attn_dbg_blocks(int device, int precision, const float* qkv, float* ctx, int B, int T, int H, int head_dim, int all_blocks,
+                            char* plan, int plan_bytes) {
+  if (plan && plan_bytes > 0) plan[0] = 0;
+  int rc = dbg_precision("pg_attn_dbg_blocks", precision, false);
+  if (rc) return rc;
+  if (!qkv || !ctx || B < 1 || T < 1 || H < 1 || all_blocks < 0 || all_blocks > 1 || (plan && plan_bytes < 1))
+    return fail(PG_ERR_INVALID, "pg_attn_dbg_blocks: bad argument");
+  if (!head_width(head_dim)) return fail(PG_ERR_INVALID, "pg_attn_dbg_blocks: head_dim must be " + head_widths_text(false));
+  if ((double)B * T * 3 * H * head_dim > 2147483647.0) return fail(PG_ERR_INVALID, "pg_attn_dbg_blocks: more than 2^31 - 1 qkv values");
+  Dbg s;
+  if ((rc = s.open(device))) return rc;
+  const int d = H * head_dim;
+  return dbg_attention_run(s, precision, false, qkv, ctx, (int64_t)B * T, d, nullptr, plan, plan_bytes,
+                           [&](const float*, const bf16_t* bq, bf16_t* out, const int32_t*) {
+    OPS(attention_all_blocks, all_blocks != 0);
+    const int r = OPS(launch_attention_bf16, nullptr, bq, out, B, T, H, 3 * d, d, d, 2 * d, nullptr, -1, nullptr, head_dim);
+    OPS(attention_all_blocks, false);
+    return r;
+  });
+}
+
+int pg_attn_dbg_bench(int device, int precision, int B, int T, int H, int head_dim, int all_blocks, int iters, double* avg_ms) {
+  int rc = dbg_precision("pg_attn_dbg_bench", precision, false);
+  if (rc) return rc;
+  if (!avg_ms || B < 1 || T < 1 || H < 1 || iters < 1 || all_blocks < 0 || all_blocks > 1 || !head_width(head_dim))
+    return fail(PG_ERR_INVALID, "pg_attn_dbg_bench: bad argument");
+  const int d = H * head_dim;
+  const size_t chain = (size_t)T * 3 * d;
+  if ((double)B * chain > 2147483647.0) return fail(PG_ERR_INVALID, "pg_attn_dbg_bench: more than 2^31 - 1 qkv values");
+  Dbg s;
+  if ((rc = s.open(device))) return rc;
+  const std::vector<float> h = lcg_uniform(chain, 4242u);
+  const float* f = s.up(h.data(), chain);
+  bf16_t* bq = s.alloc<bf16_t>((size_t)B * chain);
+  bf16_t* out = s.alloc<bf16_t>((size_t)B * T * d);
+  if ((rc = s.check())) return rc;
+  if ((rc = to16(precision, f, bq, (int64_t)chain))) return rc;
+  for (int b = 1; b < B; ++b) PG_HIP(hipMemcpyAsync(bq + (size_t)b * chain, bq, chain * 2, hipMemcpyDeviceToDevice, nullptr));
+  OPS(attention_all_blocks, all_blocks != 0);
+  rc = time_launches([&] { return OPS(launch_attention_bf16, nullptr, bq, out, B, T, H, 3 * d, d, d, 2 * d, nullptr, -1, nullptr, head_dim); },
+                     iters, avg_ms);
+  OPS(attention_all_blocks, false);
+  return rc;
+}
+
+int pg_attn_dbg_indexed(int device, int precision, const float* qkv, const int32_t* idx, float* ctx_sel, int B, int T, int H, int P,
+                             char* plan, int plan_bytes) {
+  if (plan && plan_bytes > 0) plan[0] = 0;
+  int rc = dbg_precision("pg_attn_dbg_indexed", precision, false);
+  if (rc) return rc;
+  if (!qkv || !idx || !ctx_sel || B < 1 || T < 1 || H < 1 || P < 1 || (plan && plan_bytes < 1))
+    return fail(PG_ERR_INVALID, "pg_attn_dbg_indexed: bad argument");
+  if (!OPS(attention_indexed_ok, T, 64)) return fail(PG_ERR_INVALID, "pg_attn_dbg_indexed: T must be in 1 ... 576");
+  for (int64_t i = 0; i < (int64_t)B * P; ++i)
+    if (idx[i] < 0 || idx[i] >= T) return fail(PG_ERR_INVALID, "pg_attn_dbg_indexed: a position outside 0 ... T - 1");
+  if ((double)B * T * 3 * H * 64 > 2147483647.0) return fail(PG_ERR_INVALID, "pg_attn_dbg_indexed: more than 2^31 - 1 qkv values");
+  Dbg s;
+  if ((rc = s.open(device))) return rc;
+  const int d = H * 64;
+  const int64_t M = (int64_t)B * T, n_sel = (int64_t)B * P;
+  const float* dq = s.up(qkv, (size_t)M * 3 * d);
+  const int32_t* di = s.up(idx, (size_t)n_sel);
+  bf16_t* bq = s.alloc<bf16_t>((size_t)M * 3 * d);
+  bf16_t* qs = s.alloc<bf16_t>((size_t)n_sel * 3 * d);
+  bf16_t* out = s.alloc<bf16_t>((size_t)n_sel * d);
+  float* wide = s.alloc<float>((size_t)n_sel * d);
+  if ((rc = s.check())) return rc;
+  if ((rc = to16(precision, dq, bq, M * 3 * d))) return rc;
+  if ((rc = launch_gather_rows(nullptr, bq, qs, di, nullptr, P, T, n_sel, 3 * d * 2))) return rc;
+  clear_noted_kernels();
+  if ((rc = OPS(launch_attention_indexed_bf16, nullptr, bq, qs, out, B, T, H, P, 3 * d, 3 * d, d, d, 2 * d, 64))) return rc;
+  dbg_noted_text(plan, plan_bytes);
+  return down16(s, precision, out, wide, ctx_sel, n_sel * d);
+}
+
 int pg_dbg_layernorm_operand(int device, int precision, const float* x, const float* gamma, const float* beta, float* y, int M, int d,
                              float eps) {
   int rc = dbg_precision("pg_dbg_layernorm_operand", precision, true);
diff --git a/protein_gibbs_sampler_amd/csrc/attention.hip b/protein_gibbs_sampler_amd/csrc/attention.hip
--- a/protein_gibbs_sampler_amd/csrc/attention.hip
+++ b/protein_gibbs_sampler_amd/csrc/attention.hip
@@ -25,12 +25,15 @@
 constexpr int attention_resident(int kb, int hd) {
   return hd == 16 ? attention_resident16(kb) : hd == 128 ? (kb <= 4 ? 4 : (kb <= 6 ? 3 : (kb <= 10 ? 2 : 1))) : hd == 64 ? (kb <= 20 ? 2 : 1) : (kb <= 20 ? 4 : (kb <= 26 ? 3 : 2));
 }
-template <int MAXKB, bool PADMASK, bool BIASKV = false, bool SPLIT = false, int HD = 64>
+constexpr bool dead_last_built(int hd, int kb) { return !(hd == 32 && kb == 20); }
+template <int MAXKB, bool PADMASK, bool BIASKV = false, bool SPLIT = false, int HD = 64, bool DEADLAST = false>
 __global__ __launch_bounds__(256, attention_occupancy(MAXKB, HD, PADMASK)) void attention_kernel(const bf16_t* __restrict__ qkv, bf16_t* __restrict__ ctx, int T,
                                                        int H, int ld_qkv_, int ld_ctx_, int k_off, int v_off,
                                                        SeqLayout sl, const int32_t* __restrict__ key_tok, int pad_idx,
                                                        const bf16_t* __restrict__ bias_kv, int split_from = 0, int split = 1) {
+  static_assert(!DEADLAST || (!PADMASK && !BIASKV), "DEADLAST: the plain and SPLIT forms");
   constexpr int ROW = HD * 2, NKK = score_steps(HD), NDB = HD / 16;
+  constexpr int NKB = DEADLAST ? MAXKB - 1 : MAXKB;
   typedef kfrag_t<HD> kf_t;
   __shared__ __attribute__((aligned(16))) char smem[2 * MAXKB * 16 * ROW + (PADMASK ? MAXKB * 16 : 0)];
   char* Ks = smem;
@@ -76,7 +79,7 @@
     if (qb + qb_step < nqb) load_q(qb + qb_step, qn);
     PG_T(qb >> 2, 0);
 
-    f32x4 st[MAXKB];
+    f32x4 st[NKB];
     {
       constexpr int CH = HD == 128 ? 2 : (MAXKB % 6 == 0) ? 6 : (MAXKB % 4 == 0 ? 4 : 2);
       kf_t kbuf[2][CH][NKK];
@@ -89,6 +92,7 @@
 #else
           const int krow = (ch * CH + u) * 16 + fr;
 #endif
+          if (DEADLAST && ch * CH + u == MAXKB - 1) continue;
 #pragma unroll
           for (int kk = 0; kk < NKK; ++kk) dst[u][kk] = k_frag<HD>(Ks, krow, kk, fq);
         }
@@ -100,18 +104,18 @@
         __builtin_amdgcn_sched_barrier(0);
 #pragma unroll
         for (int u = 0; u < CH; ++u)
-          st[ch * CH + u] = score_mfma(kbuf[ch & 1][u][0], qf[0], (f32x4){0.f, 0.f, 0.f, 0.f});
+          if (ch * CH + u < NKB) st[ch * CH + u] = score_mfma(kbuf[ch & 1][u][0], qf[0], (f32x4){0.f, 0.f, 0.f, 0.f});
         if constexpr (NKK == 2) {
 #pragma unroll
           for (int u = 0; u < CH; ++u)
-            st[ch * CH + u] = score_mfma(kbuf[ch & 1][u][1], qf[1], st[ch * CH + u]);
+            if (ch * CH + u < NKB) st[ch * CH + u] = score_mfma(kbuf[ch & 1][u][1], qf[1], st[ch * CH + u]);
         }
         if constexpr (NKK == 4) {
 #pragma unroll
           for (int kk = 1; kk < 4; ++kk)
 #pragma unroll
             for (int u = 0; u < CH; ++u)
-              st[ch * CH + u] = score_mfma(kbuf[ch & 1][u][kk], qf[kk], st[ch * CH + u]);
+              if (ch * CH + u < NKB) st[ch * CH + u] = score_mfma(kbuf[ch & 1][u][kk], qf[kk], st[ch * CH + u]);
         }
         __builtin_amdgcn_sched_barrier(0);
       }
@@ -120,14 +124,14 @@
     int tl = Tk - fq * 4;
     asm volatile("" : "+v"(tl));
 #pragma unroll
-    for (int kb = MAXKB > 6 ? MAXKB - 6 : 0; kb < MAXKB; ++kb)
+    for (int kb = MAXKB > 6 ? MAXKB - 6 : 0; kb < NKB; ++kb)
       if ((kb + 1) * 16 > Tk) st[kb] = mask_tail(st[kb], kb, tl);
     float mx = lane_max(st);
     if (PADMASK) {
       const float fill = sl.row_step == 1 ? -3.0e38f : -10000.0f;
       mx = -3.0e38f;
 #pragma unroll
-      for (int kb = 0; kb < MAXKB; ++kb) {
+      for (int kb = 0; kb < NKB; ++kb) {
         st[kb] = mask_pad(st[kb], *(const uint32_t*)(padf + kb * 16 + fq * 4), fill);
 #pragma unroll
         for (int r = 0; r < 4; ++r) mx = fmaxf(mx, st[kb][r]);
@@ -148,7 +152,8 @@
           if (db > 0) { dst[db] = dst[0]; continue; }
 #endif
 #pragma unroll
-          for (int hh = 0; hh < 2; ++hh) dst[db].h[hh] = vt_half<HD>(Vs, (2 * c + hh) * 16, db, fr, fq);
+          for (int hh = 0; hh < 2; ++hh)
+            dst[db].h[hh] = DEADLAST && 2 * c + hh == MAXKB - 1 ? make_uint2(0, 0) : vt_half<HD>(Vs, (2 * c + hh) * 16, db, fr, fq);
         }
       };
       load_v(0, vbuf[0]);
@@ -156,7 +161,7 @@
 #pragma unroll
       for (int c = 0; c < nkc; ++c) {
         if (c + 2 < nkc) load_v(c + 2, vbuf[(c + 2) % 3]);
-        const bf16x8 pf = p_frag(st[2 * c], st[2 * c + 1]);
+        const bf16x8 pf = p_frag(st[2 * c], 2 * c + 1 < NKB ? st[2 * c + 1] : (f32x4){0.f, 0.f, 0.f, 0.f});
         __builtin_amdgcn_sched_barrier(0);
 #pragma unroll
         for (int db = 0; db < NDB; ++db) o[db] = mfma_op16(vbuf[c % 3][db].v, pf, o[db]);
@@ -172,6 +177,64 @@
     PG_T(qb >> 2, 4);
   }
   PG_T(7, 3);
+}
+
+template <int MAXKB, bool DEADLAST, int HD = 64>
+__global__ __launch_bounds__(256, attention_occupancy(MAXKB, HD)) void attention_indexed_kernel(const bf16_t* __restrict__ qkv, const bf16_t* __restrict__ q_sel,
+                                                                                                bf16_t* __restrict__ ctx_sel, int T, int H, int P, int ld_qkv_,
+                                                                                                int ld_q_, int ld_ctx_, int k_off, int v_off) {
+  constexpr int ROW = HD * 2, NKK = score_steps(HD), NDB = HD / 16, nkc = MAXKB / 2;
+  constexpr int NKB = DEADLAST ? MAXKB - 1 : MAXKB;
+  typedef kfrag_t<HD> kf_t;
+  __shared__ __attribute__((aligned(16))) char smem[2 * MAXKB * 16 * ROW];
+  char* Ks = smem;
+  char* Vs = smem + MAXKB * 16 * ROW;
+  const int tid = threadIdx.x, lane = tid & 63, wave = tid >> 6;
+  const int b = blockIdx.x / H, h = blockIdx.x % H;
+  const size_t ld_qkv = (size_t)ld_qkv_, ld_q = (size_t)ld_q_, ld_ctx = (size_t)ld_ctx_;
+  const bf16_t* base = qkv + (size_t)b * T * ld_qkv + h * HD;
+  const bf16_t* qbase = q_sel + (size_t)b * P * ld_q + h * HD;
+  stage_kv<MAXKB * 16, 256, false, HD>(Ks, Vs, tid, base, ld_qkv, k_off, v_off, 0, T, nullptr, nullptr);
+  __syncthreads();
+
+  const int fr = lane & 15, fq = lane >> 4;
+  const int nqb = (P + 15) >> 4;
+  for (int qb = wave; qb < nqb; qb += 4) {
+    int qi = qb * 16 + fr;
+    if (qi >= P) qi = P - 1;
+    kf_t qf[NKK];
+#pragma unroll
+    for (int kk = 0; kk < NKK; ++kk) qf[kk] = q_frag<HD>(qbase + (size_t)qi * ld_q, kk, fq);
+    f32x4 st[NKB];
+#pragma unroll
+    for (int kb = 0; kb < NKB; ++kb) {
+      st[kb] = (f32x4){0.f, 0.f, 0.f, 0.f};
+#pragma unroll
+      for (int kk = 0; kk < NKK; ++kk) st[kb] = score_mfma(k_frag<HD>(Ks, kb * 16 + fr, kk, fq), qf[kk], st[kb]);
+    }
+    const int tl = T - fq * 4;
+#pragma unroll
+    for (int kb = MAXKB > 6 ? MAXKB - 6 : 0; kb < NKB; ++kb)
+      if ((kb + 1) * 16 > T) st[kb] = mask_tail(st[kb], kb, tl);
+    const float inv = softmax_exact(st, lane_max(st));
+    f32x4 o[NDB];
+#pragma unroll
+    for (int db = 0; db < NDB; ++db) o[db] = (f32x4){0.f, 0.f, 0.f, 0.f};
+#pragma unroll
+    for (int c = 0; c < nkc; ++c) {
+      const bf16x8 pf = p_frag(st[2 * c], 2 * c + 1 < NKB ? st[2 * c + 1] : (f32x4){0.f, 0.f, 0.f, 0.f});
+#pragma unroll
+      for (int db = 0; db < NDB; ++db) {
+        VtFrag vf;
+#pragma unroll
+        for (int hh = 0; hh < 2; ++hh)
+          vf.h[hh] = DEADLAST && 2 * c + hh == MAXKB - 1 ? make_uint2(0, 0) : vt_half<HD>(Vs, (2 * c + hh) * 16, db, fr, fq);
+        o[db] = mfma_op16(vf.v, pf, o[db]);
+      }
+    }
+    const int q = qb * 16 + fr;
+    if (q < P) store_ctx(o, inv, ctx_sel + ((size_t)b * P + q) * ld_ctx + h * HD + fq * 4);
+  }
 }
 
 template <int MAXKB, int OCC, bool PADMASK, bool BIASKV, int HD = 64>
@@ -335,15 +398,19 @@
 }
 
 template <int KB, int HD, class... Args>
-static void launch_rung(bool pad, bool bias, bool split, dim3 grid, hipStream_t s, Args... args) {
+static void launch_rung(bool pad, bool bias, bool split, bool dead, dim3 grid, hipStream_t s, Args... args) {
   auto go = [&](auto* kernel) { hipLaunchKernelGGL(kernel, grid, dim3(256), 0, s, args...); };
   if constexpr (coarse_rung(KB) && HD == 64) {
     if (bias && pad) return go(attention_kernel<KB, true, true, false, HD>);
     if (bias) return go(attention_kernel<KB, false, true, false, HD>);
   }
   if constexpr (KB * 16 <= attention_max_keys(HD)) {
-    if (pad) go(attention_kernel<KB, true, false, false, HD>);
-    else if (split) go(attention_kernel<KB, false, false, true, HD>);
+    if (pad) return go(attention_kernel<KB, true, false, false, HD>);
+    if constexpr (dead_last_built(HD, KB)) {
+      if (dead && split) return go(attention_kernel<KB, false, false, true, HD, true>);
+      if (dead) return go(attention_kernel<KB, false, false, false, HD, true>);
+    }
+    if (split) go(attention_kernel<KB, false, false, true, HD>);
     else go(attention_kernel<KB, false, false, false, HD>);
   }
 }
@@ -358,6 +425,10 @@
   if (pad) go(attention_long_kernel<KB, 2, true, false, HD>);
   else go(attention_long_kernel<KB, 2, false, false, HD>);
 }
+
+static bool g_all_blocks = false;
+void attention_all_blocks(bool on) { g_all_blocks = on; }
+static bool dead_last_block(int T, int kb) { return !g_all_blocks && T <= 16 * (kb - 1); }
 
 int launch_attention_seq_bf16(hipStream_t s, const bf16_t* qkv, bf16_t* ctx, int64_t n_seq, int T, int H, int ld_qkv,
                               int ld_ctx, int k_off, int v_off, SeqLayout sl, const int32_t* key_tok, int pad_idx,
@@ -372,7 +443,7 @@
       return launch_long<HD>(p.pad, p.bias, dim3(p.grid), s, qkv, ctx, T, H, ld_qkv, ld_ctx, k_off, v_off, sl, p.n_qchunk, key_tok,
                              pad_idx, bias_kv);
     visit_rung(p.kb, [&](auto kb) {
-      launch_rung<decltype(kb)::value, HD>(p.pad, p.bias, p.split > 1, dim3(p.grid), s, qkv, ctx, T, H, ld_qkv, ld_ctx, k_off, v_off,
+      launch_rung<decltype(kb)::value, HD>(p.pad, p.bias, p.split > 1, dead_last_block(T, p.kb), dim3(p.grid), s, qkv, ctx, T, H, ld_qkv, ld_ctx, k_off, v_off,
                                            sl, key_tok, pad_idx, bias_kv, p.split_from, p.split);
     });
   };
@@ -387,4 +458,25 @@
   return launch_attention_seq_bf16(s, qkv, ctx, B, T, H, ld_qkv, ld_ctx, k_off, v_off, sl, key_tok, pad_idx, bias_kv, head_dim);
 }
 
+bool attention_indexed_ok(int T, int head_dim) { return head_dim == 64 && T >= 1 && T <= attention_max_keys(64); }
+int launch_attention_indexed_bf16(hipStream_t s, const bf16_t* qkv, const bf16_t* q_sel, bf16_t* ctx_sel, int B, int T, int H, int P,
+                                  int ld_qkv, int ld_q, int ld_ctx, int k_off, int v_off, int head_dim) {
+  if (!attention_indexed_ok(T, head_dim)) return fail(1, "attention: the indexed-query form is built for heads of 64 and up to 576 keys");
+  if (B < 0 || H < 1 || P < 0 || (int64_t)B * H > 0x7fffffff) return fail(1, "attention: bad indexed-query shape");
+  if (B == 0 || P == 0) return 0;
+  const int kb = attention_rung(T, true);
+  const bool dead = dead_last_block(T, kb);
+  note_kernel(("indexed kb" + std::to_string(kb) + " hd64 P" + std::to_string(P) + " " + std::to_string(B * H) + "wg").c_str());
+  visit_rung(kb, [&](auto r) {
+    constexpr int KB = decltype(r)::value;
+    auto go = [&](auto* kernel) {
+      hipLaunchKernelGGL(kernel, dim3((unsigned)(B * H)), dim3(256), 0, s, qkv, q_sel, ctx_sel, T, H, P, ld_qkv, ld_q, ld_ctx, k_off, v_off);
+    };
+    if (dead) go(attention_indexed_kernel<KB, true>);
+    else go(attention_indexed_kernel<KB, false>);
+  });
+  PG_HIP(hipGetLastError());
+  return 0;
+}
+
 PG_OPS_END
diff --git a/protein_gibbs_sampler_amd/csrc/engine.h b/protein_gibbs_sampler_amd/csrc/engine.h
--- a/protein_gibbs_sampler_amd/csrc/engine.h
+++ b/protein_gibbs_sampler_amd/csrc/engine.h
@@ -130,6 +130,7 @@
 
   DevBuf x, h, qkv, ctx, ffn, sel_h, sel_g, logits, d_tokens, d_idx, d_samp_tok, d_samp_logits, d_rowmap, scratch;
   DevBuf x_sel, ctx_sel, h_sel, ffn_sel;
+  DevBuf q_sel;
   DevBuf tmp_idx, tmp_out;
   DevBuf splitk;
   DevBuf ffn_f32, scores;
@@ -200,7 +201,10 @@
   int ffn_block(const DenseW& out, const FfnW& F, const LnW* next_ln, int Mi, int64_t M, bool folded = false);
   bool prune_last(int64_t n_draws, int64_t token_rows) const;
   int pruned_tail(const DenseW& out, const FfnW& F, const int32_t* sel_idx, const int32_t* sel_row_map, int P, int width, int64_t n_sel,
-                  const int32_t* d_iter, int Ni, bool ln_in_gemm);
+                  const int32_t* d_iter, int Ni, bool ln_in_gemm, bool ctx_ready = false);
+  static constexpr int64_t kSampledQueriesRows = 4096;
+  bool sampled_queries(int B, int T, const int32_t* sel_idx, int64_t n_sel, int P) const;
+  int last_layer_sampled(const EsmLayer& L, int B, int T, int Mi, int64_t M, const int32_t* sel_idx, int P, int64_t n_sel, const int32_t* d_iter);
   enum ChainRan { CHAIN_NOT_RUN, CHAIN_TO_LAST_ATTENTION, CHAIN_WHOLE_FORWARD };
   int chain_forward(int B, int T, int Mi, bool stop_at_last_attention, ChainRan* ran);
   int esm_trunk(const int32_t* d_tok, int B, int T, const int32_t* sel_idx, int P, int64_t n_sel, const int32_t* d_iter);
diff --git a/protein_gibbs_sampler_amd/csrc/engine.hip b/protein_gibbs_sampler_amd/csrc/engine.hip
--- a/protein_gibbs_sampler_amd/csrc/engine.hip
+++ b/protein_gibbs_sampler_amd/csrc/engine.hip
@@ -603,7 +603,7 @@
 }
 
 int Engine::pruned_tail(const DenseW& out, const FfnW& F, const int32_t* sel_idx, const int32_t* sel_row_map, int P, int width,
-                        int64_t n_sel, const int32_t* d_iter_, int Ni, bool ln_in_gemm) {
+                        int64_t n_sel, const int32_t* d_iter_, int Ni, bool ln_in_gemm, bool ctx_ready) {
   const int d = cfg.d_model, f = cfg.d_ffn;
   const int64_t Np = round_up64(n_sel, kRowPad);
   int rc;
@@ -614,7 +614,7 @@
   bf16_t* FS = ffn_sel.as<bf16_t>();
   rc = timed(PC_HEAD, [&] {
     int r2 = launch_gather_rows(stream, x.as<float>(), XS, sel_idx, sel_row_map, P, width, n_sel, d * 4, d_iter_);
-    if (r2) return r2;
+    if (r2 || ctx_ready) return r2;
     return launch_gather_rows(stream, ctx.as<bf16_t>(), ctx_sel.as<bf16_t>(), sel_idx, sel_row_map, P, width, n_sel, d * 2, d_iter_);
   });
   if (rc) return rc;
@@ -626,6 +626,36 @@
     if ((rc = dense(PC_GEMM, HS, F.fc1, FS, Ni, EPI_BF16_GELU))) return rc;
   }
   return dense(PC_GEMM, FS, F.fc2, XS, Ni, EPI_F32_RESID, 0, true);
+}
+
+bool Engine::sampled_queries(int B, int T, const int32_t* sel_idx, int64_t n_sel, int P) const {
+  return sel_idx && cfg.arch == PG_ARCH_ESM1B && !strict() && !esm_pad_in_batch && !tap && !ctap && P >= 1 && n_sel == (int64_t)B * P &&
+         batch_rows_for(B, T) > kSampledQueriesRows && OPS(attention_indexed_ok, T, head_dim);
+}
+
+int Engine::last_layer_sampled(const EsmLayer& L, int B, int T, int Mi, int64_t M, const int32_t* sel_idx, int P, int64_t n_sel,
+                               const int32_t* d_iter_) {
+  const int d = cfg.d_model;
+  const int64_t Np = round_up64(n_sel, kRowPad);
+  const int Ni = sel_gemm_rows(n_sel, Np);
+  int rc;
+  if ((rc = h_sel.ensure((size_t)Np * d * 2, stream)) || (rc = q_sel.ensure((size_t)Np * d * 2, stream)) ||
+      (rc = ctx_sel.ensure((size_t)Np * d * 2, stream))) return rc;
+  bf16_t* Hh = h.as<bf16_t>();
+  bf16_t* QKV = qkv.as<bf16_t>();
+  const DenseW& W = L.qkv;
+  rc = timed(PC_GEMM_QKV, [&] {
+    return OPS(launch_gemm_bf16, stream, Hh, W.w + (size_t)d * W.K, W.b + d, QKV + d, Mi, 2 * d, W.K, W.K, W.K, 3 * d, EPI_BF16, nullptr, 0, (int)M);
+  });
+  if (rc) return rc;
+  if ((rc = timed(PC_HEAD, [&] { return launch_gather_rows(stream, Hh, h_sel.as<bf16_t>(), sel_idx, nullptr, P, T, n_sel, d * 2, d_iter_); }))) return rc;
+  rc = timed(PC_GEMM_QKV, [&] {
+    return OPS(launch_gemm_bf16, stream, h_sel.as<bf16_t>(), W.w, W.b, q_sel.as<bf16_t>(), Ni, d, W.K, W.K, W.K, d, EPI_BF16, nullptr, 0, 0);
+  });
+  if (rc) return rc;
+  return timed(PC_ATTN, [&] {
+    return OPS(launch_attention_indexed_bf16, stream, QKV, q_sel.as<bf16_t>(), ctx_sel.as<bf16_t>(), B, T, cfg.n_heads, P, 3 * d, d, d, d, 2 * d, head_dim);
+  });
 }
 
 int Engine::trunk(const int32_t* d_tok, int B, int R, int C, const int32_t* sel_idx, const int32_t* sel_row_map, int P, int64_t n_sel,
@@ -720,8 +750,13 @@
   const EsmLayer& tail = esm_layers.back();
   auto finish_selected = [&] { return pruned_tail(tail.out, tail.ffn, sel_idx, nullptr, P, T, n_sel, d_iter_, sel_gemm_rows(n_sel, round_up64(n_sel, kRowPad)), ln_in_gemm); };
   if (ran == CHAIN_TO_LAST_ATTENTION) return finish_selected();
+  const bool sampled_last = !ln_in_gemm && sampled_queries(B, T, sel_idx, n_sel, P);
   for (int l = 0; l < cfg.n_layers; ++l) {
     const EsmLayer& L = esm_layers[l];
+    if (sampled_last && l == cfg.n_layers - 1) {
+      if ((rc = last_layer_sampled(L, B, T, Mi, M, sel_idx, P, n_sel, d_iter_))) return rc;
+      return pruned_tail(tail.out, tail.ffn, sel_idx, nullptr, P, T, n_sel, d_iter_, sel_gemm_rows(n_sel, round_up64(n_sel, kRowPad)), ln_in_gemm, true);
+    }
     if ((rc = ln_in_gemm ? dense_ln(X, L.ln1, L.qkv, QKV, Mi, EPI_BF16) : dense(PC_GEMM_QKV, Hh, L.qkv, QKV, Mi, EPI_BF16))) return rc;
     if ((rc = rope(QKV, M, T)) || (rc = tap_attention(l, QKV))) return rc;
     if ((rc = timed(PC_ATTN, [&] { return OPS(launch_attention_bf16, stream, QKV, CTX, B, T, cfg.n_heads, 3 * d, d, d, 2 * d, esm_pad_in_batch ? d_tok : nullptr, cfg.pad_idx, L.bias_kv16, head_dim); }))) return rc;
diff --git a/protein_gibbs_sampler_amd/csrc/kernels_ops.inc b/protein_gibbs_sampler_amd/csrc/kernels_ops.inc
--- a/protein_gibbs_sampler_amd/csrc/kernels_ops.inc
+++ b/protein_gibbs_sampler_amd/csrc/kernels_ops.inc
@@ -31,6 +31,10 @@
 int launch_attention_seq_bf16(hipStream_t s, const bf16_t* qkv, bf16_t* ctx, int64_t n_seq, int T, int H, int ld_qkv,
                               int ld_ctx, int k_off, int v_off, SeqLayout sl, const int32_t* key_tok = nullptr,
                               int pad_idx = -1, const bf16_t* bias_kv = nullptr, int head_dim = 64);
+bool attention_indexed_ok(int T, int head_dim);
+int launch_attention_indexed_bf16(hipStream_t s, const bf16_t* qkv, const bf16_t* q_sel, bf16_t* ctx_sel, int B, int T, int H, int P,
+                                  int ld_qkv, int ld_q, int ld_ctx, int k_off, int v_off, int head_dim = 64);
+void attention_all_blocks(bool on);
 size_t msa_row_split_scratch_bytes(int B, int R, int C, int H, int order_bh);
 void attention_plan_text(int64_t n_seq, int T, int H, int head_dim, bool has_pad, bool has_bias, int row_step, int n_cu, std::string* text);
 void attention_f32_plan_text(int64_t n_seq, int T, int H, int head_dim, bool has_pad, bool has_bias, std::string* text);
```

Measured after the change: 73110 sampled positions/s, median of 5. No clear change (+0.4%).
